# halismai/bpvo

Hardware: AMD Instinct MI355X
Metric: GN iterations/s (1241x376 bit-planes 8ch, 4 levels, Tukey; linearise + solve + update = 1, the reference's _num_fun_evals) (higher is better)
Workload: dtype f32 (+f64 projection/interpolation); 1 GPU; batch of 1024 independent 1241x376 stereo pairs (1024 per GPU), bitplanes descriptor, 4 pyramid levels, tukey loss, converge with AlgorithmParameters() tolerances; pairs_per_gpu=1024

## Files before the change

### __graft_entry__.py

```python
from __future__ import annotations

import os
import subprocess
import sys

ROOT = os.path.dirname(os.path.abspath(__file__))
CSRC = os.path.join(ROOT, "bpvo_amd", "csrc")
HIP_LIB = os.path.join(CSRC, "libbpvo_hip.so")
ORACLE_DIR = os.path.join(ROOT, "oracle")
ORACLE_LIB = os.path.join(ORACLE_DIR, "_build", "libbpvo_oracle.so")

MGPU_LIB = os.path.join(CSRC, "libbpvo_hip_mgpu.so")

HIP_SOURCES = ["context.hip", "frames.hip", "estimate.hip", "batch.hip", "vo.hip", "measure.hip", "kernels_frame.hip", "kernels_intensity_norm.hip", "kernels_planes.hip", "kernels_gn.hip", "kernels_gn_ref.hip", "kernels_gn_team.hip", "kernels_gn_rig.hip", "kernels_gn_cov.hip", "pose_cov.hip", "kernels_score.hip", "score.hip", "kernels_stereo.hip", "kernels_sgm.hip", "kernels_sgbm.hip", "kernels_rectify.hip", "rectify.hip", "stereo.hip", "kernels_disparity_fusion.hip", "disparity_fusion.hip", "kernels_disparity_variance.hip", "disparity_variance.hip", "kernels_motion_stereo.hip", "motion_stereo.hip"]
HIP_HEADERS = ["host_ctx.h", "device_owned.h", "vo_state.h", "gn_rounds.h", "frame_plan.h", "kernels.h", "types.h", "device_math.h", "gn_common.h", "gn_warp.h", "warp_rule.h", "gn_median.h", "gn_tscale.h", "tscale_math.h", "gn_irls.h", "gn_step.h", "rig_math.h", "pose_cov_math.h", "pose_score_math.h", "rectify_math.h", "intensity_norm_math.h", "disparity_fusion_math.h", "disparity_variance_math.h", "motion_stereo_math.h", "gn_cov.h", "frame_common.h", "latch_table.h", "sg_scanline.h",
               os.path.join("..", "..", "include", "bpvo_hip", "c_api.h")]
HIPCC_FLAGS = ["--offload-arch=gfx950", "-O3", "-std=c++17", "-ffp-contract=off", "-fPIC", "-Wall", "-Wno-unused-function"]
OBJ_DIR = os.path.join(CSRC, "obj")


def _newer(target, sources):
    if not os.path.exists(target):
        return True
    t = os.path.getmtime(target)
    return any(os.path.getmtime(s) > t for s in sources if os.path.exists(s))


def _hipcc():
    for cand in ("hipcc", "/opt/rocm/bin/hipcc"):
        try:
            subprocess.run([cand, "--version"], check=True, capture_output=True)
            return cand
        except Exception:
            continue
    raise RuntimeError("hipcc not found")


def build_hip(force: bool = False, extra_flags=(), out: str | None = None) -> str:
    from concurrent.futures import ThreadPoolExecutor
    out = out or HIP_LIB
    headers = [os.path.join(CSRC, h) for h in HIP_HEADERS]
    if not force and not _newer(out, [os.path.join(CSRC, s) for s in HIP_SOURCES] + headers):
        return out
    obj_dir = OBJ_DIR if out == HIP_LIB else OBJ_DIR + "_" + os.path.splitext(os.path.basename(out))[0]
    os.makedirs(obj_dir, exist_ok=True)
    hipcc = _hipcc()
    jobs = []
    for s in HIP_SOURCES:
        src = os.path.join(CSRC, s)
        obj = os.path.join(obj_dir, os.path.splitext(s)[0] + ".o")
        if force or _newer(obj, [src] + headers):
            jobs.append([hipcc, *HIPCC_FLAGS, *extra_flags, "-c", src, "-o", obj])

    def run(cmd):
        return subprocess.run(cmd, cwd=CSRC, capture_output=True, text=True)
    with ThreadPoolExecutor(max_workers=min(8, os.cpu_count() or 1)) as ex:
        for cmd, r in zip(jobs, ex.map(run, jobs)):
            if r.returncode != 0:
                raise RuntimeError("hipcc failed (%s):\n%s%s" % (cmd[-3], r.stdout, r.stderr))
    objs = [os.path.join(obj_dir, os.path.splitext(s)[0] + ".o") for s in HIP_SOURCES]
    if force or jobs or _newer(out, objs):
        r = subprocess.run([hipcc, "--offload-arch=gfx950", "-shared", "-fPIC", "-o", out, *objs], cwd=CSRC, capture_output=True, text=True)
        if r.returncode != 0:
            raise RuntimeError("hipcc link failed:\n" + r.stdout + r.stderr)
    return out


def build_mgpu(force: bool = False) -> str:
    src = os.path.join(CSRC, "multi_gpu.hip")
    deps = [src, HIP_LIB, os.path.join(ROOT, "include", "bpvo_hip", "multi_gpu.h"), os.path.join(ROOT, "include", "bpvo_hip", "c_api.h")]
    if force or _newer(MGPU_LIB, deps):
        rocm_lib = os.path.join(os.environ.get("ROCM_PATH", "/opt/rocm"), "lib")
        cmd = [_hipcc(), "--offload-arch=gfx950", "-O2", "-std=c++17", "-fPIC", "-shared", "-Wall", "-o", MGPU_LIB, src,
               "-L", CSRC, "-lbpvo_hip", "-L", rocm_lib, "-lrccl", "-lpthread", "-Wl,-rpath,$ORIGIN", f"-Wl,-rpath,{rocm_lib}"]
        r = subprocess.run(cmd, cwd=CSRC, capture_output=True, text=True)
        if r.returncode != 0:
            raise RuntimeError("hipcc (multi_gpu) failed:\n" + r.stdout + r.stderr)
    return MGPU_LIB


def build_oracle(force: bool = False) -> str:
    if force:
        subprocess.run(["make", "-C", ORACLE_DIR, "clean"], check=True, capture_output=True)
    r = subprocess.run(["make", "-C", ORACLE_DIR], capture_output=True, text=True)
    if r.returncode != 0:
        raise RuntimeError("oracle build failed:\n" + r.stdout + r.stderr)
    return ORACLE_LIB


def build_reference_pins() -> str | None:
    if not os.path.isdir("/root/reference/bpvo"):
        return None
    r = subprocess.run(["make", "-C", ORACLE_DIR, "ref"], capture_output=True, text=True)
    if r.returncode != 0:
        raise RuntimeError("oracle/_ref build failed:\n" + r.stdout + r.stderr)
    return os.path.join(ORACLE_DIR, "_ref", "libbpvo_ref.so")


# ... 65 lines not shown
```

### bpvo_amd/csrc/batch.hip

```cpp
#include "host_ctx.h"

using namespace bpvo_hip;
using namespace bpvo_hip_host;

namespace {

constexpr int kUploadChunkPairs = 16;
constexpr int kUploadGroup = 4;
struct UploadRun {
  bpvo_hip_ctx* c = nullptr;
  int n_pairs = 0;
  std::vector<std::pair<int, int>> chunks;
  std::vector<int> recorded;
  std::mutex mu;
  std::condition_variable cv;
  std::vector<std::thread> workers;
  std::string err;
  ~UploadRun() { for(auto& t : workers) if(t.joinable()) t.join(); }
};

int upload_prepare(bpvo_hip_ctx* c, int n_pairs)
{
  const size_t npix = c->geom[0].npix;
  c->up_slot_bytes = (size_t) kUploadChunkPairs * npix * (2 + 4);
// ... 107 lines not shown
      }
      FR_CK(c, fr_lane, hipStreamWaitEvent(fr_lane.stream, c->up_chunk_done[k], 0));
    }
    const int p0 = u.chunks[mine[i]].first;
    int np = 0;
    for(size_t q = i; q < i + take; ++q) np += u.chunks[mine[q]].second;
    FrameRun fr = fr_lane;
    fr.tab = 2 * p0;
    fr.selected_ev = nullptr; fr.on_selected = nullptr;
    int rc = frames_set_data_slots(c, strided_slots(2 * p0, 1, 2 * np).data(), 2 * np, c->up_d_img + (size_t) 2 * p0 * npix, c->up_d_disp + (size_t) p0 * npix, true, fr, 2);
    if(rc) return rc;
    i += take;
  }
  return BPVO_OK;
}

int batch_run_staggered(bpvo_hip_ctx* c, int n_pairs, int nl, const uint8_t* images, const float* disparities, bool on_device, float* poses,
                        bpvo_hip_stats* stats, UploadRun* pipe, const std::vector<std::pair<int, int>>* host_group_list)
{
  HIP_CK(c, hipStreamSynchronize(c->stream));
  c->frac_valid = false;
  const size_t npix = c->geom[0].npix;
  std::vector<int> rcs(nl, BPVO_OK);
  std::mutex mu;
  std::condition_variable cv;
  std::vector<int> selected(nl, 0);
  std::vector<std::pair<int, int>> groups;
  if(host_group_list) groups = *host_group_list;
  else host_groups(n_pairs, nl, 1, groups);
  const int nsub = (int) groups.size() / nl;
  auto run = [&](int k) {
    Lane* ln = &c->lanes[k];
    (void) hipSetDevice(c->device);
    auto release_next = [&mu, &cv, &selected, k] { { std::lock_guard<std::mutex> lk(mu); selected[k] = 1; } cv.notify_all(); };
    struct Release { std::function<void()> f; ~Release() { f(); } } always{release_next};
    if(k > 0 && !pipe) {
      { std::unique_lock<std::mutex> lk(mu); cv.wait(lk, [&] { return selected[k - 1] != 0; }); }
      if(hipStreamWaitEvent(ln->stream, c->lanes[k - 1].selected_ev, 0) != hipSuccess) { ln->err = "hipStreamWaitEvent"; rcs[k] = BPVO_ERR_DEVICE; return; }
    }
    for(int sub = 0; sub < nsub; ++sub) {
      const int lo = groups[(size_t) sub * nl + k].first, hi = groups[(size_t) sub * nl + k].second, n = hi - lo;
      if(n <= 0) continue;
      FrameRun fr{ln->stream, ln, 2 * lo, true, nullptr, nullptr};
      int rc = pipe ? upload_consume(c, *pipe, lo, hi, fr)
                    : frames_set_data_slots(c, strided_slots(2 * lo, 1, 2 * n).data(), 2 * n, images + (size_t) 2 * lo * npix, disparities + (size_t) 2 * lo * npix, on_device, fr,
                                            c->keep_current_disparity ? 0 : 1);
      if(rc) { rcs[k] = rc; return; }
      if(sub == 0) {
        fr.selected_ev = ln->selected_ev;
        fr.on_selected = release_next;
      }
      rc = frames_set_template_slots(c, strided_slots(2 * lo, 2, n).data(), n, fr);
      if(rc) { rcs[k] = rc; return; }
      std::vector<int> wss(n), refs(n), curs(n);
      for(int i = 0; i < n; ++i) { wss[i] = lo + i; refs[i] = 2 * (lo + i); curs[i] = 2 * (lo + i) + 1; }
      rc = estimate_group(c, ln, n, wss.data(), refs.data(), curs.data(), nullptr, poses ? poses + 16 * (size_t) lo : nullptr,
                          stats ? stats + (size_t) lo * c->L : nullptr, c->d_records + (size_t) kRecordFloats * lo, false);
      if(rc) { rcs[k] = rc; return; }
    }
  };
  {
    std::vector<std::thread> th;
    for(int k = 1; k < nl; ++k) th.emplace_back(run, k);
    run(0);
    for(auto& t : th) t.join();
  }
  for(int k = 0; k < nl; ++k)
    if(rcs[k]) { c->err = c->lanes[k].err; return rcs[k]; }
  resolve_events(c);
  for(int i = 0; i < n_pairs; ++i) {
    Workspace& w = c->ws[i];
    w.last_ref = 2 * i;
    w.last_cur = 2 * i + 1;
    w.last_level = c->params.maxTestLevel;
    w.has_estimate = true;
  }
  return BPVO_OK;
}

}

extern "C" {

int bpvo_hip_batch_run(bpvo_hip_ctx* c, int n_pairs, const uint8_t* images, const float* disparities, int on_device,
                       float* poses, bpvo_hip_stats* stats)
{
  CHECK_CTX(c);
  if(n_pairs < 0 || 2 * n_pairs > c->n_frames || n_pairs > c->n_pairs) return fail(c, BPVO_ERR_INVALID_ARG, "batch exceeds ctx capacity");
  for(int i = 0; i < 2 * n_pairs; ++i)
    if(c->frames[i].own_geom) return fail(c, BPVO_ERR_UNSUPPORTED, "pair batches run the context's camera: its slots carry per-sequence cameras (bpvo_hip_seq_set_camera)");
  (void) hipSetDevice(c->device);
  if(n_pairs > 0 && (!images || !disparities)) return fail(c, BPVO_ERR_INVALID_ARG, "nullptr image/disparity");
  const bool use_pipe = !on_device && c->up_workers > 0 && !c->keep_current_disparity && n_pairs >= 2 * kUploadChunkPairs;
  int nl = lanes_for(c, n_pairs, use_pipe ? 2 : 8);
  if(nl < 0) return nl;
  if(team_serves(c, n_pairs)) nl = 1;
  if(c->stagger && n_pairs >= c->stagger_min_pairs && nl > 1 && !c->profile_all) {
    if(!use_pipe) return batch_run_staggered(c, n_pairs, nl, images, disparities, on_device != 0, poses, stats, nullptr, nullptr);
    std::vector<std::pair<int, int>> groups;
    const int nsub = 1;
    const bool plan = nl == 2 && nsub == 1 && c->up_plan[0] > 0.0 && n_pairs >= 32 * kUploadChunkPairs;
    if(plan) host_groups_plan(c, n_pairs, groups);
    else host_groups(n_pairs, nl, nsub, groups);
    UploadRun pipe;
    int rcp = upload_start(c, pipe, n_pairs, groups, images, disparities);
    if(rcp) return rcp;
    c->ctl_by_kernel = true;
    rcp = batch_run_staggered(c, n_pairs, nl, images, disparities, false, poses, stats, &pipe, &groups);
    c->ctl_by_kernel = false;
    return rcp;
  }
  int rc;
  if(use_pipe) {
    UploadRun pipe;
    std::vector<std::pair<int, int>> groups;
    host_groups(n_pairs, 1, 1, groups);
    rc = upload_start(c, pipe, n_pairs, groups, images, disparities);
    if(rc) return rc;
    rc = upload_consume(c, pipe, 0, n_pairs, ctx_run(c));
  } else {
    rc = frames_set_data(c, 0, 1, 2 * n_pairs, images, disparities, on_device != 0, c->keep_current_disparity ? 0 : 1);
  }
  if(rc) return rc;
  FrameRun fr = ctx_run(c);
  fr.no_final_sync = !c->profiling;
  fr.defer_finest_nrm = !team_serves(c, n_pairs) || n_pairs <= c->team_split_max_pairs || templates_may_be_dense(c);
  rc = frames_set_template_slots(c, strided_slots(0, 2, n_pairs).data(), n_pairs, fr);
  if(rc == BPVO_OK) rc = bpvo_hip_batch_estimate(c, n_pairs, nullptr, poses, stats);
  if(c->nrm_pending) { (void) hipEventSynchronize(c->nrm_pending); c->nrm_pending = nullptr; }
  if(c->nrm_pending_finest) { (void) hipEventSynchronize(c->nrm_pending_finest); c->nrm_pending_finest = nullptr; }
  return rc;
}
int bpvo_hip_batch_result_records_device(bpvo_hip_ctx* c, const float** d_records, int* floats_per_pair)
{
  CHECK_CTX(c);
  *d_records = c->d_records;
  *floats_per_pair = kRecordFloats;
  return BPVO_OK;
}

int bpvo_hip_batch_copy_records_device(bpvo_hip_ctx* c, float* d_dst, int n_pairs)
{
  CHECK_CTX(c);
  if(!d_dst || n_pairs < 0 || n_pairs > c->n_pairs) return fail(c, BPVO_ERR_INVALID_ARG, "bad record copy");
  (void) hipSetDevice(c->device);
  HIP_CK(c, hipMemcpyAsync(d_dst, c->d_records, sizeof(float) * kRecordFloats * (size_t) n_pairs, hipMemcpyDeviceToDevice, c->stream));
  HIP_CK(c, hipStreamSynchronize(c->stream));
  return BPVO_OK;
}

}
```

### bpvo_amd/csrc/context.hip

```cpp
#include "host_ctx.h"

using namespace bpvo_hip;
using namespace bpvo_hip_host;

namespace bpvo_hip_host {

std::atomic<int> g_live_ctx[64];
thread_local std::string g_create_error;

int fail(bpvo_hip_ctx* c, int code, const char* msg)
{
  c->err = msg;
  return code;
}


void gaussian_kernel5(double sigma, float k[3])
{
  float kk[5];
  const double sigmaX = sigma > 0 ? sigma : ((5 - 1) * 0.5 - 1) * 0.3 + 0.8;
  const double scale2X = -0.5 / (sigmaX * sigmaX);
  double sum = 0;
  for(int i = 0; i < 5; ++i) {
    const double x = i - 2.0;
// ... 42 lines not shown
{
  Carver cv{base};
  for(int l = 0; l < c->L; ++l) {
    const LevelGeom& g = c->geom[l];
    f.sal[l] = cv.take<float>(g.npix);
    const size_t nwords = (size_t) g.rows * ((g.cols + 63) / 64);
    f.flag[l] = (uint8_t*) cv.take<unsigned long long>((std::max(g.npix, nwords * 8) + 7) / 8);
    f.blk_count[l] = cv.take<int>(std::max((size_t) g.nblk, nwords));
    f.pts[l] = cv.take<float4>(g.cap);
    f.ptc[l] = cv.take<float2>(g.cap);
    f.inds[l] = cv.take<int>(g.cap);
    f.pix[l] = cv.take<float>((size_t) g.cap * c->C);
    f.grad[l] = cv.take<float>((size_t) g.cap * c->C * 2);
  }
  f.nrm = cv.take<float>(4 * kMaxLevels);
  f.n_dev = cv.take<int>(kMaxLevels);
  f.sel_info = cv.take<int>(4 * kMaxLevels);
  if(total) *total = cv.off;
}

hipError_t ensure_template_storage(bpvo_hip_ctx* c, FrameSlot& f, hipStream_t stream)
{
  if(f.tmpl_slab) return hipSuccess;
  size_t total = 0;
  FrameSlot tmp;
  carve_frame_tmpl(c, tmp, nullptr, &total);
  if(hipError_t e = f.tmpl_slab.alloc(total)) return e;
  if(hipError_t e = hipMemsetAsync(f.tmpl_slab, 0, total, stream)) return e;
  carve_frame_tmpl(c, f, f.tmpl_slab, nullptr);
  return hipSuccess;
}

FrameJob make_frame_job(bpvo_hip_ctx* c, FrameSlot& f, int l)
{
  const LevelGeom& g = slot_geom(c, f, l);
  FrameJob j;
  std::memset(&j, 0, sizeof(j));
  j.img = f.img[l];
  j.cen = f.cen[l];
  j.ch0 = (f.ch0_valid && f.lazy[l] != 2) ? f.ch0[l] : nullptr;
  j.scratch = f.scratch;
  j.inorm = c->d_inorm ? c->d_inorm + ((size_t) (&f - c->frames.data()) * c->L + l) : nullptr;
  j.desc = f.desc[l];
  j.sal = f.sal_state[l] == FrameSlot::SAL_STORED ? f.sal[l] : nullptr;
  j.flag = f.flag[l];
  j.words = reinterpret_cast<unsigned long long*>(f.flag[l]);
  j.blk_count = f.blk_count[l];
  j.n_out = f.n_dev ? f.n_dev + l : nullptr;
  j.disp = f.disp;
  j.pts = f.pts[l];
  j.ptc = f.ptc[l];
  j.inds = f.inds[l];
  j.pix = f.pix[l];
  j.grad = f.grad[l];
  j.nrm = f.nrm ? f.nrm + 4 * l : nullptr;
  j.rows = g.rows; j.cols = g.cols; j.level = l; j.disp_cols = slot_geom(c, f, 0).cols;
  j.cap = g.cap;
  j.nms_radius = g.nms_radius;
  std::memcpy(j.K, g.K, sizeof(j.K));
  j.b = g.b;
  j.dspace = c->dspace;
  j.lazy = f.lazy[l];
  const bpvo_hip_params& sp = f.seq_params ? *f.seq_params : c->params;
  j.min_saliency = sp.minSaliency; j.min_disp = sp.minValidDisparity; j.max_disp = sp.maxValidDisparity;
  j.max_points = slot_budget(c, f, l);
  j.sel_info = f.sel_info ? f.sel_info + 4 * l : nullptr;
  return j;
}

PairJob make_pair_job(bpvo_hip_ctx* c, int ws, int ref, int cur, int l)
{
  FrameSlot& fr = c->frames[ref];
  FrameSlot& fc = c->frames[cur];
  const LevelGeom& g = slot_geom(c, fr, l);
  PairJob j;
  std::memset(&j, 0, sizeof(j));
  j.pts = fr.pts[l];
  j.ptc = fr.ptc[l];
  j.pix = fr.pix[l];
  j.grad = fr.grad[l];
  j.nrm = fr.nrm + 4 * l;
  j.n = fr.n_host[l];
  j.desc = fc.desc[l];
  j.rows = g.rows; j.cols = g.cols;
  std::memcpy(j.K, g.K, sizeof(j.K));
  j.b = g.b;
  j.f_inv[0] = 1.0f / g.K[0]; j.f_inv[1] = 1.0f / g.K[4];
  j.dspace = c->dspace;
  j.r = c->ws[ws].r;
  j.valid = c->ws[ws].valid;
  j.cand = c->ws[ws].cand;
  j.tapkey = c->ws[ws].tapkey;
  j.tapcache_on = c->ws[ws].tapkey != nullptr;
  j.tapcache = c->ws[ws].tapcache;
  j.med_blk = c->ws[ws].med_blk;
  j.partials = c->ws[ws].partials;
  j.st = c->d_states + ws;
  j.cnt = c->d_counters + kWsCounters * (size_t) ws;
  j.ticket = c->d_tickets + ws;
  if(ws == c->trace_ws) { j.trace = c->d_trace; j.trace_cap = (int) (c->d_trace.size() / kTraceFloats); }
  j.pitch = c->C;
  j.n_groups = c->G;
  j.med_tot = (int) med_totals_at(c);
  pair_job_set_params(j, c->params);
  return j;
}
void pair_job_set_params(PairJob& j, const bpvo_hip_params& p)
{
  j.prm = GNParams{p.maxIterations, kMaxFunEvals, p.parameterTolerance, p.functionTolerance, p.gradientTolerance};
  j.loss = p.lossFunction;
  j.good_thr = p.goodPointThreshold;
}

PairJob group_pair_job(const bpvo_hip_ctx* c, const PairJob& whole, int k)
{
  PairJob j = whole;
  const size_t off = (size_t) k * c->Cg;
  const size_t nblk = (size_t) ((whole.n + kChunkPoints - 1) / kChunkPoints);
  const size_t ntiles = (size_t) std::max(1, (whole.n + gn_pts_per_block(c->Cg) - 1) / gn_pts_per_block(c->Cg));
  j.desc = whole.desc.get() + off;
  j.pix = whole.pix.get() + off;
  j.grad = whole.grad.get() + off;
  j.r = whole.r.get() + off;
  j.cand = whole.cand.get() + (size_t) k * nblk * kChunkPoints * c->Cg;
  j.med_blk = whole.med_blk.get() + (size_t) k * nblk * 4;
  j.partials = whole.partials.get() + (size_t) k * ntiles * kPartialStride;
  j.n_groups = 1;
  return j;
}

Event take_event(Lane* ln)
{
  Event e;
  if(!ln->ev_pool.empty()) {
    e = std::move(ln->ev_pool.back());
    ln->ev_pool.pop_back();
  }
  else (void) e.create(0);
  return e;
}
void resolve_events(bpvo_hip_ctx* c)
{
  for(auto& ln : c->lanes) {
    for(auto& ep : ln.ev_pending) {
      float ms = 0.0f;
      if(hipEventElapsedTime(&ms, ep.a, ep.b) == hipSuccess) {
        c->kc_ms[ep.kc] += ms;
        c->kc_units[ep.kc] += ep.units;
        c->kc_launches[ep.kc] += 1;
      }
      ln.ev_pool.push_back(std::move(ep.a));
      ln.ev_pool.push_back(std::move(ep.b));
    }
    ln.ev_pending.clear();
  }
}

int lanes_for(bpvo_hip_ctx* c, int n, int cap)
{
  if(g_live_ctx[c->device & 63].load() > 1) return 1;
  const int want = std::max(1, std::min(std::min(c->max_lanes_now, cap), n / kMinPairsPerLane));
  if(want > (int) c->lanes.size()) {
    const int rc = ensure_lanes(c, want);
    if(rc) return rc;
  }
  return want;
// ... 21 lines not shown
    HIP_CK(c, ln.h_pk_ctl.alloc(kPkCtlWords * kMaxLevels));
    if(first) {
      HIP_CK(c, ln.d_team_ctl.alloc((size_t) gn_team_ctl_words(kMaxTeams)));
      HIP_CK(c, ln.h_team_ctl.alloc(64));
      std::memset(ln.h_team_ctl, 0, sizeof(unsigned) * 64);
    }
    HIP_CK(c, ln.h_states.alloc((size_t) n_pairs + n_pairs));
  }
  return BPVO_OK;
}

const std::vector<OptionDef>& option_table()
{
#define OPT_INT(key_, field_, lo_, hi_) OptionDef{key_, lo_, hi_, [](bpvo_hip_ctx* c) { return (double) c->field_; }, \
                                                  [](bpvo_hip_ctx* c, double v) { c->field_ = (decltype(c->field_)) v; return BPVO_OK; }}
  static const std::vector<OptionDef> t = {
    OptionDef{"lanes", 1, 8, [](bpvo_hip_ctx* c) { return (double) std::max(1, std::min(c->max_lanes_now, std::max(1, c->n_pairs / kMinPairsPerLane))); },
              [](bpvo_hip_ctx* c, double v) {
                const int n = std::max(1, std::min((int) v, std::max(1, c->n_pairs / kMinPairsPerLane)));
                const int rc = ensure_lanes(c, n);
                if(rc == BPVO_OK) c->max_lanes_now = (int) v;
                return rc;
              }},
    OptionDef{"persistent", 0, 1, [](bpvo_hip_ctx* c) { return (double) c->persistent; },
              [](bpvo_hip_ctx* c, double v) { c->persistent = (int) v; if(c->persistent) c->persistent_failed.store(false); return BPVO_OK; }},
    OPT_INT("persist_max_ws", persist_max_ws, 1, kPersistMaxWs),
    OPT_INT("persist_grid", persist_grid, 1, 128),
    OPT_INT("persist_max_points", persist_max_points, 0, 1 << 30),
    OPT_INT("dense_candidates_from", dense_candidates_from, 0, 1 << 30),
    OPT_INT("persist_timeout_ticks", persist_timeout, 1, 1e15),
    OPT_INT("team", team_mode, 0, 1),
    OPT_INT("team_max_pairs", team_max_pairs, 0, 1 << 20),
    OPT_INT("team_full_pairs", team_full_pairs, 0, 1 << 20),
    OPT_INT("team_size", team_size_env, 0, 256),
    OptionDef{"team_cus", 1, 1 << 16, [](bpvo_hip_ctx* c) { return (double) c->num_cus; },
              [](bpvo_hip_ctx* c, double v) {
                if(c->device_cus > 0 && (int) v > c->device_cus) { c->err = "option team_cus: more CUs than the device has"; return BPVO_ERR_INVALID_ARG; }
                c->num_cus = (int) v;
                return BPVO_OK;
              }},
    OPT_INT("team_local_barriers", team_local_barriers, 0, 1),
    OPT_INT("team_join", team_join, 0, 2),
    OptionDef{"team_joins_seen", 0, 0, [](bpvo_hip_ctx* c) { return (double) c->team_joins.load(); },
              [](bpvo_hip_ctx* c, double) { c->team_joins.store(0); return BPVO_OK; }},
    OPT_INT("team_join_from_pairs", team_join_from_pairs, 0, 1 << 20),
    OPT_INT("team_spares", team_spares, 0, 1),
    OPT_INT("vo_disparity_late", vo_disparity_late, 0, 1),
    OPT_INT("stereo_frames_per_launch", stereo_frames_per_launch, 0, 65535),
    OptionDef{"stereo_frames_per_launch_seen", 0, 0, [](bpvo_hip_ctx* c) { return (double) c->st_frames_per_launch_seen; }, [](bpvo_hip_ctx*, double) { return BPVO_OK; }},
    OptionDef{"stereo_free_mib_seen", 0, 0, [](bpvo_hip_ctx* c) { return (double) (c->st_free_seen >> 20); }, [](bpvo_hip_ctx*, double) { return BPVO_OK; }},
    OptionDef{"rectify_last_kernel_ms", 0, 0, [](bpvo_hip_ctx* c) {
                float ms = -1.0f;
                if(!c->rect.timed || hipEventSynchronize(c->rect.t1) != hipSuccess || hipEventElapsedTime(&ms, c->rect.t0, c->rect.t1) != hipSuccess) return -1.0;
                return (double) ms;
              }, [](bpvo_hip_ctx*, double) { return BPVO_OK; }},
    OptionDef{"fusion_last_splat_ms", 0, 0, [](bpvo_hip_ctx* c) { return fusion_last_ms(c, 0); }, [](bpvo_hip_ctx*, double) { return BPVO_OK; }},
    OptionDef{"fusion_last_update_ms", 0, 0, [](bpvo_hip_ctx* c) { return fusion_last_ms(c, 1); }, [](bpvo_hip_ctx*, double) { return BPVO_OK; }},
    OptionDef{"variance_last_kernel_ms", 0, 0, [](bpvo_hip_ctx* c) { return variance_last_ms(c); }, [](bpvo_hip_ctx*, double) { return BPVO_OK; }},
    OptionDef{"motion_stereo_last_kernel_ms", 0, 0, [](bpvo_hip_ctx* c) { return motion_stereo_last_ms(c); }, [](bpvo_hip_ctx*, double) { return BPVO_OK; }},
    OPT_INT("normalization_side_stream", nrm_side_stream, 0, 1),
    OPT_INT("normalization_form", nrm_dpp_asm, 0, 4),
    OPT_INT("small_batch_fused", small_batch_fused, 0, 1),
    OPT_INT("levels_in_one_launch_max_frames", merge_levels_max_frames, 0, 1 << 20),
    OPT_INT("normalization_deferred", nrm_defer, 0, 1),
    OPT_INT("team_split_max_pairs", team_split_max_pairs, 0, 1 << 20),
    OPT_INT("fuse_frozen", fuse_frozen, 0, 1),
    OPT_INT("reference_reduction", reference_reduction, 0, 1),
    OPT_INT("step_in_reduce_max_pairs", step_in_reduce_max, 0, 1 << 20),
    OPT_INT("stagger", stagger, 0, 1),
    OPT_INT("stagger_min_pairs", stagger_min_pairs, 0, 1 << 20),
    OPT_INT("upload_workers", up_workers, 0, 32),
    OPT_INT("keep_current_disparity", keep_current_disparity, 0, 1),
    OptionDef{"pose_covariance", 0, 1, [](bpvo_hip_ctx* c) { return (double) c->pose_covariance; },
              [](bpvo_hip_ctx* c, double v) -> int {
                if((int) v) {
                  const int rc = pose_cov_ensure_scratch(c);
                  if(rc) return rc;
                }
                c->pose_covariance = (int) v;
                return BPVO_OK;
              }},
    OPT_INT("lazy_template_descriptor", lazy_template, 0, 1),
    OPT_INT("lazy_template_saliency", lazy_saliency, 0, 1),
    OPT_INT("points_from_compact_stream", points_from_compact, 0, 1),
    OptionDef{"tapcache_max_density", 0.0, 1e9, [](bpvo_hip_ctx* c) { return c->tapcache_max_density; },
              [](bpvo_hip_ctx* c, double v) { c->tapcache_max_density = v; return BPVO_OK; }},
    OptionDef{"upload_plan_first", 0.0, 0.9, [](bpvo_hip_ctx* c) { return c->up_plan[0]; },
              [](bpvo_hip_ctx* c, double v) { if(v + c->up_plan[1] >= 1.0) return BPVO_ERR_INVALID_ARG; c->up_plan[0] = v; return BPVO_OK; }},
    OptionDef{"upload_plan_second", 0.01, 0.99, [](bpvo_hip_ctx* c) { return c->up_plan[1]; },
              [](bpvo_hip_ctx* c, double v) { if(v + c->up_plan[0] >= 1.0) return BPVO_ERR_INVALID_ARG; c->up_plan[1] = v; return BPVO_OK; }},
  };
#undef OPT_INT
  return t;
}
int set_option(bpvo_hip_ctx* c, const std::string& key, double v)
{
  for(const OptionDef& o : option_table())
    if(key == o.key) {
      if(!(v >= o.lo && v <= o.hi)) { c->err = "option " + key + ": value out of range"; return BPVO_ERR_INVALID_ARG; }
      const int rc = o.set(c, v);
      if(rc == BPVO_ERR_INVALID_ARG) c->err = "option " + key + ": invalid value";
      return rc;
    }
  c->err = "unknown option: " + key;
  return BPVO_ERR_INVALID_ARG;
}
int apply_options_string(bpvo_hip_ctx* c, const char* str)
{
  std::string s(str);
  size_t i = 0;
  while(i < s.size()) {
    size_t j = s.find(',', i);
    if(j == std::string::npos) j = s.size();
    const std::string kv = s.substr(i, j - i);
    i = j + 1;
    if(kv.empty()) continue;
    const size_t eq = kv.find('=');
    if(eq == std::string::npos) { c->err = "expected key=value: " + kv; return BPVO_ERR_INVALID_ARG; }
    char* end = nullptr;
    const double v = std::strtod(kv.c_str() + eq + 1, &end);
    if(end == kv.c_str() + eq + 1) { c->err = "not a number: " + kv; return BPVO_ERR_INVALID_ARG; }
    const int rc = set_option(c, kv.substr(0, eq), v);
    if(rc) return rc;
  }
  return BPVO_OK;
}

}

extern "C" {

void bpvo_hip_default_params(bpvo_hip_params* p)
{
  p->numPyramidLevels = -1;
  p->minImageDimensionForPyramid = 40;
  p->sigmaPriorToCensusTransform = -1.0f;
  p->sigmaBitPlanes = 0.5f;
  p->dfSigma1 = 0.75f;
  p->dfSigma2 = 1.75f;
  p->latchNumBytes = 1;
  p->latchRotationInvariance = 0;
  p->latchHalfSsdSize = 1;
  p->centralDifferenceRadius = 3;
  p->centralDifferenceSigmaBefore = 0.75f;
  p->centralDifferenceSigmaAfter = 1.75f;
  p->laplacianKernelSize = 1;
  p->maxIterations = 50;
  p->parameterTolerance = 1e-7f;
  p->functionTolerance = 1e-6f;
  p->gradientTolerance = 1e-8f;
  p->relaxTolerancesForCoarseLevels = 1;
  p->gradientEstimation = BPVO_GRAD_CD3;
  p->interp = BPVO_INTERP_LINEAR;
  p->lossFunction = BPVO_LOSS_TUKEY;
  p->descriptor = BPVO_DESC_INTENSITY;
  p->verbosity = BPVO_VERB_ITERATION;
  p->minTranslationMagToKeyFrame = 0.15f;
  p->minRotationMagToKeyFrame = 5.0f;
  p->maxFractionOfGoodPointsToKeyFrame = 0.6f;
  p->goodPointThreshold = 0.85f;
  p->minNumPixelsForNonMaximaSuppression = 320 * 240;
  p->nonMaxSuppRadius = 1;
  p->minNumPixelsToWork = 256;
  p->minSaliency = 0.1f;
  p->minValidDisparity = 0.001f;
  p->maxValidDisparity = 512.0f;
// ... 314 lines not shown
```

### bpvo_amd/csrc/estimate.hip

```cpp
#include "host_ctx.h"

using namespace bpvo_hip;
using namespace bpvo_hip_host;

namespace bpvo_hip_host {


struct TeamPlan { int team_size, n_teams, join_mode, spare_workgroups; };
static TeamPlan team_plan(const bpvo_hip_ctx* c, int n)
{
  TeamPlan t;
  const int slots = std::max(1, c->num_cus);
  int ts = c->team_size_env > 0 ? c->team_size_env : std::max(1, std::min(std::max(1, c->device_cus > 0 ? c->device_cus / 8 : 32), slots / std::max(1, n)));
  ts = std::max(1, std::min(ts, slots));
  t.team_size = ts;
  t.n_teams = std::max(1, std::min(std::min(n, slots / ts), kMaxTeams));
  t.join_mode = (t.team_size < gn_team_max_size() && t.n_teams > 1 && n >= c->team_join_from_pairs) ? c->team_join : 0;
  t.spare_workgroups = (t.join_mode && c->team_spares) ? std::max(0, slots - t.team_size * t.n_teams) : 0;
  return t;
}

bool team_serves(const bpvo_hip_ctx* c, int n)
{
  bool size_ok = n >= 2 && n > c->persist_max_ws && n <= c->team_max_pairs;
// ... 10 lines not shown
static bool templates_suit_teams(const bpvo_hip_ctx* c, int n, const int* refs)
{
  for(int i = 0; i < n; ++i)
    for(int l = c->params.maxTestLevel; l < c->L; ++l)
      if(c->frames[refs[i]].n_host[l] > c->persist_max_points) return false;
  return true;
}

template <class PrmOf>
static void fill_job_tables(bpvo_hip_ctx* c, Lane* ln, int first, int n, const int* wss, const int* refs, const int* curs, PrmOf&& prm_of, int* max_pts)
{
  const int NP = c->n_pairs;
  const size_t table = (size_t) c->L * NP;
  for(int l = 0; l < c->L; ++l)
    for(int i = 0; i < n; ++i) {
      PairJob& pj = ln->h_pjobs[(size_t) l * NP + first + i];
      pj = make_pair_job(c, wss[i], refs[i], curs[i], l);
      if(const bpvo_hip_params* prm = prm_of(i)) pair_job_set_params(pj, *prm);
      for(int k = 0; k < c->G && c->G > 1; ++k) ln->h_pjobs[(size_t) (1 + k) * table + (size_t) l * NP + first + i] = group_pair_job(c, pj, k);
      max_pts[l] = std::max(max_pts[l], pj.n);
    }
}
template <class LossOf, class Run>
static int for_each_loss(int n, LossOf&& loss_of, Run&& run)
{
  std::vector<char> done((size_t) n, 0);
  for(int i = 0; i < n; ++i) {
    if(done[i]) continue;
    std::vector<int> at;
    for(int k = i; k < n; ++k)
      if(!done[k] && loss_of(k) == loss_of(i)) { done[k] = 1; at.push_back(k); }
    if(int rc = run(at)) return rc;
  }
  return BPVO_OK;
}

void linearize_launches(bpvo_hip_ctx* c, Lane* ln, const GNLaunch& g, size_t stride, const LinearizeFlags& f)
{
  constexpr unsigned kProfileEvery = 5;
  const bool all = f.timers == TIMERS_ALWAYS || (f.timers != TIMERS_OFF && c->profile_all);
  if(f.warp) {
    const bool sampled = all || (f.timers == TIMERS_ESTIMATE && (c->profile_k6_all || (ln->k6_seq++ % kProfileEvery) == 0));
    ScopedTimer t(c, KC_WARP_RESIDUAL, 0.0, ln, sampled);
    for_each_group(c, g, stride, [&](const GNLaunch& gg) { launch_warp_residual(ln->stream, gg); });
  }
  { ScopedTimer t(c, KC_MEDIAN, 0.0, ln, all && f.median); if(f.median) launch_median(ln->stream, median_launch(c, g)); }
  if(f.reduce) {
    ScopedTimer t(c, KC_IRLS_REDUCE, 0.0, ln, all || (f.timers == TIMERS_ESTIMATE && c->profile_k6_all));
    if(g.reference_reduction) launch_irls_reduce(ln->stream, g);
    else for_each_group(c, g, stride, [&](const GNLaunch& gg) { launch_irls_reduce(ln->stream, gg); });
  }
  if(f.step && !g.step_in_reduce) {
    ScopedTimer t(c, KC_GN_STEP, 0.0, ln, all);
    launch_gn_step(ln->stream, g, f.step_mode);
  }
}

template <class QueueIterations, class QueueFlags, class Read>
static int lane_rounds(Lane* ln, int max_iterations, QueueIterations&& queue_iterations, QueueFlags&& queue_flags, Read&& read)
{
  return run_rounds(max_iterations, queue_iterations,
                    [&](int slot) -> int {
                      if(int rc = queue_flags(slot)) return rc;
                      LANE_CK(ln, hipEventRecord(ln->round_ev[slot], ln->stream));
                      return BPVO_OK;
                    },
                    [&](int slot) -> int {
                      LANE_CK(ln, hipEventSynchronize(ln->round_ev[slot]));
                      return BPVO_OK;
                    },
                    read);
}

struct GroupRun {
  bpvo_hip_ctx* c;
  Lane* ln;
  int n;
  const int* wss; const int* refs; const int* curs;
  const float* T_init;
  const bpvo_hip_params* const* prms;
  float* d_records_out;
  int loss, max_iterations;
  std::vector<int> max_pts;
  bool ref_mode;
  int fuse_frozen;
  bool allow_persistent;
  bool pk_group;
  bool small_ctx;
  bool l2_moot;
  bool team_ran, team_split, frac_queued;
};
static void group_modes(GroupRun& r, bool allow_persistent)
{
  const bpvo_hip_ctx* c = r.c;
  r.ref_mode = c->reference_reduction != 0;
  r.fuse_frozen = r.ref_mode ? 0 : c->fuse_frozen;
  r.allow_persistent = allow_persistent;
  r.pk_group = allow_persistent && c->persistent && !c->persistent_failed.load() && r.n <= c->persist_max_ws && !c->profile_all && !r.ref_mode &&
               !loss_is_chain_only(r.loss);
  r.small_ctx = (size_t) c->L * c->n_pairs <= 64 && r.n <= 8 && c->small_batch_fused && c->G == 1;
  r.l2_moot = r.loss == BPVO_LOSS_L2 && c->C == 8 && r.fuse_frozen && !c->fast_warp && c->params.interp == BPVO_INTERP_LINEAR;
  r.team_ran = r.team_split = r.frac_queued = false;
}

static int group_upload(GroupRun& r)
{
  bpvo_hip_ctx* c = r.c;
  Lane* ln = r.ln;
  const int n = r.n, NP = c->n_pairs;
  const int* refs = r.refs;
  const float* T_init = r.T_init;
  const bool persistent = r.pk_group;
  std::fill(r.max_pts.begin(), r.max_pts.end(), 0);
  const size_t table = (size_t) c->L * NP;
  fill_job_tables(c, ln, 0, n, r.wss, refs, r.curs, [&](int i) { return r.prms ? r.prms[i] : nullptr; }, r.max_pts.data());
  if((c->C == 8 || c->C == 1) && n > c->persist_max_ws)
    for(int l = 0; l < c->L; ++l)
      for(int i = 0; i < n; ++i) {
        PairJob& pj = ln->h_pjobs[(size_t) l * NP + i];
        if((double) pj.n > c->tapcache_max_density * (double) slot_geom(c, c->frames[refs[i]], l).npix) pj.tapcache_on = 0;
      }
  if(r.small_ctx) {
    if(T_init) std::memcpy(ln->h_T, T_init, sizeof(float) * 16 * n);
    launch_set_pose_upload(ln->stream, ln->d_pjobs, ln->h_pjobs, (size_t) c->L * NP, ln->h_pjobs + (size_t) (c->L - 1) * NP, T_init ? ln->h_T : nullptr, n,
                           persistent ? ln->d_pk_ctl : nullptr, persistent ? kPkCtlWords * kMaxLevels : 0);
  } else {
    const size_t table_bytes = sizeof(PairJob) * table * (size_t) job_tables(c);
    if(c->ctl_by_kernel.load()) launch_copy_rows(ln->stream, ln->d_pjobs, ln->h_pjobs, table_bytes, table_bytes, 1);
    else LANE_CK(ln, hipMemcpyAsync(ln->d_pjobs, ln->h_pjobs, table_bytes, hipMemcpyHostToDevice, ln->stream));
    const float* dT = nullptr;
    if(T_init) {
      std::memcpy(ln->h_T, T_init, sizeof(float) * 16 * n);
      if(c->ctl_by_kernel.load()) launch_copy_rows(ln->stream, ln->d_Tinit, ln->h_T, sizeof(float) * 16 * n, sizeof(float) * 16 * n, 1);
      else LANE_CK(ln, hipMemcpyAsync(ln->d_Tinit, ln->h_T, sizeof(float) * 16 * n, hipMemcpyHostToDevice, ln->stream));
      dT = ln->d_Tinit;
    }
    launch_set_pose(ln->stream, ln->d_pjobs + (size_t) (c->L - 1) * NP, dT, n, persistent ? ln->d_pk_ctl : nullptr, persistent ? kPkCtlWords * kMaxLevels : 0);
  }
  return BPVO_OK;
}

static int run_team(GroupRun& r)
{
  bpvo_hip_ctx* c = r.c;
  Lane* ln = r.ln;
  const bpvo_hip_params& p = c->params;
  const int n = r.n;
  r.team_split = (c->nrm_pending != nullptr || c->nrm_pending_finest != nullptr) && n <= c->team_split_max_pairs && c->L - 1 > p.maxTestLevel;
  if(!r.team_split) LANE_CK(ln, join_pending_normalization(c, ln->stream));
  GNTeamLaunch t;
  t.jobs_all = ln->d_pjobs; t.job_pitch = c->n_pairs; t.n_pairs = n; t.level_hi = c->L - 1; t.level_lo = p.maxTestLevel;
  t.C = c->C; t.loss = r.loss; t.fuse_frozen = c->fuse_frozen;
  t.scale_is_moot = (r.loss == BPVO_LOSS_L2 && c->C == 8 && c->fuse_frozen) ? 1 : 0;
  const TeamPlan plan = team_plan(c, n);
  t.team_size = plan.team_size;
  t.n_teams = plan.n_teams;
  t.ctl = ln->d_team_ctl;
  t.timeout_ticks = c->persist_timeout;
  t.local_barriers = c->team_local_barriers;
  t.join_mode = plan.join_mode;
  t.spare_workgroups = plan.spare_workgroups;
  LANE_CK(ln, hipMemsetAsync(ln->d_team_ctl, 0, sizeof(unsigned) * (size_t) gn_team_ctl_words(t.n_teams), ln->stream));
  hipError_t te;
  if(r.team_split) {
    t.level_lo = c->L - 1;
    te = launch_gn_team(ln->stream, t);
    if(te == hipSuccess) {
      LANE_CK(ln, hipMemcpyAsync(ln->h_team_ctl + 32, ln->d_team_ctl, sizeof(unsigned) * 32, hipMemcpyDeviceToHost, ln->stream));
      launch_team_ctl_reset_keep_abort(ln->stream, ln->d_team_ctl, t.n_teams);
    }
    LANE_CK(ln, join_pending_normalization(c, ln->stream));
    t.level_hi = c->L - 2; t.level_lo = p.maxTestLevel;
    if(te == hipSuccess) te = launch_gn_team(ln->stream, t);
  } else {
    te = launch_gn_team(ln->stream, t);
  }
  if(te == hipSuccess) {
    r.team_ran = true;
    c->team_launches.fetch_add(1);
    LANE_CK(ln, hipMemcpyAsync(ln->h_team_ctl, ln->d_team_ctl, sizeof(unsigned) * 32, hipMemcpyDeviceToHost, ln->stream));
  } else {
    (void) hipGetLastError();
    c->persistent_failed.store(true);
  }
  return BPVO_OK;
}

static GNLaunch group_level_launch(const GroupRun& r, int l)
{
  const bpvo_hip_ctx* c = r.c;
  GNLaunch g = level_launch(c, r.ln->d_pjobs + (size_t) l * c->n_pairs, r.n, r.max_pts[l], r.loss);
  g.fuse_frozen = r.fuse_frozen;
  g.step_in_reduce = (r.n <= c->step_in_reduce_max && !r.ref_mode && c->G == 1) ? 1 : 0;
  return g;
}
static bool persistent_serves_level(const GroupRun& r, int l)
{
  return r.max_pts[l] > 0 && gn_persistent_serves(group_level_launch(r, l)) && r.max_pts[l] <= r.c->persist_max_points;
}

struct PersistentLevel { bool served, began_next; };
static PersistentLevel run_level_persistent(GroupRun& r, GNLaunch g, int l, bool was_begun)
{
  bpvo_hip_ctx* c = r.c;
  Lane* ln = r.ln;
  const bool next_too = l - 1 >= c->params.maxTestLevel && persistent_serves_level(r, l - 1);
  g.begin_level = was_begun ? l : -1;
  g.begin_moot = r.l2_moot ? 1 : 0;
  g.next_jobs = next_too ? ln->d_pjobs + (size_t) (l - 1) * c->n_pairs : nullptr;
  const hipError_t pe = launch_gn_persistent(ln->stream, g, ln->d_pk_ctl + (size_t) l * kPkCtlWords, gn_persistent_grid(g, c->persist_grid), c->persist_timeout);
  if(pe == hipSuccess) {
    c->persistent_levels.fetch_add(1);
    return {true, next_too};
  }
  (void) hipGetLastError();
  c->persistent_failed.store(true);
  if(was_begun) launch_level_begin(ln->stream, g.jobs, r.n, g.max_points, l, r.l2_moot ? 1 : 0);
  return {false, false};
}

static int run_level_chain(GroupRun& r, GNLaunch g)
{
  bpvo_hip_ctx* c = r.c;
  Lane* ln = r.ln;
  const int NP = c->n_pairs;
  const size_t table = (size_t) c->L * NP;
  int* const lists[3] = {ln->d_list, ln->d_list + NP, ln->d_list + 2 * (size_t) NP};
  int n_cur = r.n;
  g.active.list = nullptr;
  const bool fused_path = c->C == 8 && r.fuse_frozen && !c->fast_warp && c->params.interp == BPVO_INTERP_LINEAR;
  bool none_moving = r.l2_moot;
  LinearizeFlags f;
  f.timers = TIMERS_ESTIMATE;
  return lane_rounds(ln, r.max_iterations,
                     [&](int) -> int {
                       g.npairs = n_cur;
                       f.median = !none_moving;
                       f.warp = !(none_moving && fused_path);
                       for(int k = 0; k < kItersPerSync; ++k) linearize_launches(c, ln, g, table, f);
                       return BPVO_OK;
                     },
                     [&](int slot) -> int {
                       launch_compact_active(ln->stream, g.jobs, g.active, n_cur, lists[slot], ln->d_active + 2 * slot);
                       LANE_CK(ln, hipMemcpyAsync(ln->h_active + 2 * slot, ln->d_active + 2 * slot, 2 * sizeof(int), hipMemcpyDeviceToHost, ln->stream));
                       return BPVO_OK;
                     },
                     [&](int slot) {
                       const int n_left = ln->h_active[2 * slot];
                       if(n_left <= 0) return false;
                       n_cur = n_left;
                       none_moving = none_moving || ln->h_active[2 * slot + 1] == 0;
                       g.active.list = lists[slot];
                       return true;
                     });
}

static int run_levels(GroupRun& r)
{
  bpvo_hip_ctx* c = r.c;
  Lane* ln = r.ln;
  bool persistent = r.pk_group;
  bool begun = false;
  for(int l = c->L - 1; l >= c->params.maxTestLevel; --l) {
    const GNLaunch g = group_level_launch(r, l);
    if(l < c->L - 1) LANE_CK(ln, join_pending_normalization(c, ln->stream, l));
    const bool was_begun = begun;
    begun = false;
    if(!was_begun) launch_level_begin(ln->stream, g.jobs, r.n, g.max_points, l, r.l2_moot ? 1 : 0);
    if(g.max_points <= 0) continue;
    if(persistent && persistent_serves_level(r, l)) {
      const PersistentLevel pk = run_level_persistent(r, g, l, was_begun);
      begun = pk.began_next;
      if(pk.served) continue;
    }
    persistent = false;
    if(int rc = run_level_chain(r, g)) return rc;
  }
  return BPVO_OK;
}

static int queue_fraction_good(GroupRun& r)
{
  bpvo_hip_ctx* c = r.c;
  Lane* ln = r.ln;
  const bpvo_hip_params& p = c->params;
  const int NP = c->n_pairs;
  const PairJob* coarsest = ln->d_pjobs + (size_t) (c->L - 1) * NP;
  const bool want_frac = r.n == 1 && c->prefetch_frac_thr >= 0.0f && ln == &c->lanes[0];
  if(r.small_ctx) launch_pack_records(ln->stream, coarsest, r.n, c->L, r.d_records_out, c->d_states, ln->h_states, r.pk_group ? ln->d_pk_ctl : nullptr,
                                      r.pk_group ? ln->h_pk_ctl : nullptr, kPkCtlWords * kMaxLevels, want_frac ? c->d_count : nullptr);
  else launch_pack_records(ln->stream, coarsest, r.n, c->L, r.d_records_out);
  const int npts = ln->h_pjobs[(size_t) p.maxTestLevel * NP].n;
  if(!want_frac || npts <= 0) return BPVO_OK;
  const PairJob* job = ln->d_pjobs + (size_t) p.maxTestLevel * NP;
  launch_refresh_residuals(ln->stream, level_launch(c, job, 1, npts, p.lossFunction));
  if(!r.small_ctx) LANE_CK(ln, hipMemsetAsync(c->d_count, 0, sizeof(unsigned int), ln->stream));
  launch_count_good(ln->stream, job, npts, c->C, p.lossFunction, c->prefetch_frac_thr, c->d_count);
  LANE_CK(ln, hipMemcpyAsync(c->h_ints, c->d_count, sizeof(unsigned int), hipMemcpyDeviceToHost, ln->stream));
  r.frac_queued = true;
  c->frac_n = npts;
  return BPVO_OK;
}

#ifdef BPVO_PK_TIMING
static void print_pk_timing(const GroupRun& r)
{
  const bpvo_hip_ctx* c = r.c;
  const Lane* ln = r.ln;
  static const char* names[6] = {"warp", "barrier1", "median", "irls", "barrier2", "step"};
  if(r.pk_group) {
    for(int l = c->L - 1; l >= 0; --l) {
      const unsigned* t = ln->h_pk_ctl + (size_t) l * kPkCtlWords;
      if(!t[15]) continue;
      std::fprintf(stderr, "pk level %d: %u iterations;", l, t[15]);
      for(int k = 0; k < 6; ++k) std::fprintf(stderr, " %s %.2f", names[k], 0.01 * t[8 + k] / t[15]);
      std::fprintf(stderr, " | step: sum_partials %.2f unpack %.2f solve %.2f pose %.2f tests %.2f", 0.01 * t[20] / t[15], 0.01 * t[16] / t[15], 0.01 * t[17] / t[15],
                   0.01 * t[18] / t[15], 0.01 * t[19] / t[15]);
      std::fprintf(stderr, " us per iteration\n");
    }
  }
  if(r.team_ran) {
    for(int l = c->L - 1; l >= 0 && l < 4; --l) {
      const unsigned* t = ln->h_team_ctl + 4 + 7 * l;
      if(!t[6]) continue;
      std::fprintf(stderr, "team level %d: %u iterations;", l, t[6]);
      for(int k = 0; k < 6; ++k) std::fprintf(stderr, " %s %.2f", names[k], 0.01 * t[k] / t[6]);
      std::fprintf(stderr, " us per iteration\n");
    }
  }
}
#endif

static int group_collect(GroupRun& r, bool* gave_up)
{
  bpvo_hip_ctx* c = r.c;
  Lane* ln = r.ln;
  int ws_lo = r.wss[0], ws_hi = r.wss[0];
  for(int i = 1; i < r.n; ++i) { ws_lo = std::min(ws_lo, r.wss[i]); ws_hi = std::max(ws_hi, r.wss[i]); }
  if(!r.small_ctx) {
    LANE_CK(ln, hipMemcpyAsync(ln->h_states + ws_lo, c->d_states + ws_lo, sizeof(GNState) * (size_t) (ws_hi - ws_lo + 1), hipMemcpyDeviceToHost, ln->stream));
    if(r.pk_group)
      LANE_CK(ln, hipMemcpyAsync(ln->h_pk_ctl, ln->d_pk_ctl, sizeof(unsigned) * kPkCtlWords * kMaxLevels, hipMemcpyDeviceToHost, ln->stream));
  }
  if(c->before_final_sync && ln == &c->lanes[0]) {
    const std::function<int()> f = std::move(c->before_final_sync);
    c->before_final_sync = nullptr;
    if(const int rcf = f()) return rcf;
  }
  LANE_CK(ln, hipStreamSynchronize(ln->stream));
  LANE_CK(ln, hipGetLastError());
  if(r.frac_queued) { c->frac_valid = true; c->frac_ws = r.wss[0]; c->frac_thr = c->prefetch_frac_thr; c->frac_cnt = (unsigned) c->h_ints[0]; }
#ifdef BPVO_PK_TIMING
  print_pk_timing(r);
#endif
  if(r.team_ran) {
    c->team_joins.fetch_add(ln->h_team_ctl[3] + (r.team_split ? ln->h_team_ctl[32 + 3] : 0u));
    *gave_up = ln->h_team_ctl[1] != 0 || (r.team_split && ln->h_team_ctl[32 + 1] != 0);
  }
  if(r.pk_group)
    for(int l = 0; l < c->L; ++l) *gave_up = *gave_up || ln->h_pk_ctl[(size_t) l * kPkCtlWords + 1] != 0;
  return BPVO_OK;
}

static void group_outputs(const GroupRun& r, float* poses, bpvo_hip_stats* stats)
{
  const int L = r.c->L;
  for(int i = 0; i < r.n; ++i) {
    const GNState& st = r.ln->h_states[r.wss[i]];
    if(poses) std::memcpy(poses + 16 * (size_t) i, st.T_out, 16 * sizeof(float));
    if(stats)
      for(int l = 0; l < L; ++l) stats[(size_t) i * L + l] = st.stats[l];
  }
}

int estimate_group(bpvo_hip_ctx* c, Lane* ln, int n, const int* wss, const int* refs, const int* curs, const float* T_init,
                   float* poses, bpvo_hip_stats* stats, float* d_records_out, bool allow_persistent, const bpvo_hip_params* const* prms)
{
  if(n <= 0) return BPVO_OK;
  (void) hipSetDevice(c->device);
  GroupRun r{c, ln, n, wss, refs, curs, T_init, prms, d_records_out};
  r.loss = prms ? prms[0]->lossFunction : c->params.lossFunction;
  r.max_iterations = c->params.maxIterations;
  if(prms) {
    r.max_iterations = prms[0]->maxIterations;
    for(int i = 1; i < n; ++i) r.max_iterations = std::max(r.max_iterations, prms[i]->maxIterations);
  }
  r.max_pts.assign((size_t) c->L, 0);
  for(const bool persistent_forms : {allow_persistent, false}) {
    group_modes(r, persistent_forms);
    if(int rc = group_upload(r)) return rc;
    if(persistent_forms && ln == &c->lanes[0] && !loss_is_chain_only(r.loss) && team_serves(c, n) && templates_suit_teams(c, n, refs))
      if(int rc = run_team(r)) return rc;
    if(!r.team_ran)
      if(int rc = run_levels(r)) return rc;
    if(int rc = queue_fraction_good(r)) return rc;
    bool gave_up = false;
    if(int rc = group_collect(r, &gave_up)) return rc;
    if(!gave_up) break;
    c->persistent_failed.store(true);
  }
  group_outputs(r, poses, stats);
  return BPVO_OK;
}

int check_pairs(bpvo_hip_ctx* c, int n, const int* wss, const int* refs, const int* curs, int level_lo, int level_hi)
{
  for(int i = 0; i < n; ++i) {
    CHECK_WS(c, wss[i]); CHECK_SLOT(c, refs[i]); CHECK_SLOT(c, curs[i]);
  }
  for(int i = 0; i < n; ++i) {
    if(!c->frames[refs[i]].has_template) return fail(c, BPVO_ERR_NO_TEMPLATE, "reference frame has no template");
    if(!c->frames[curs[i]].has_data) return fail(c, BPVO_ERR_NO_DATA, "no data in frame");
    for(int l = level_lo; l <= level_hi; ++l)
      if(c->frames[refs[i]].n_host[l] <= 0) return fail(c, BPVO_ERR_NO_TEMPLATE, "you should call setData before calling computeResiduals");
  }
  for(int i = 0; i < n; ++i)
    if(int rc = ensure_dense_descriptor(c, curs[i])) return rc;
  return BPVO_OK;
}

static int estimate_one_loss(bpvo_hip_ctx* c, int n, const int* wss, const int* refs, const int* curs, const float* T_init, float* poses, bpvo_hip_stats* stats,
                             const bpvo_hip_params* const* prms);
int estimate_batch(bpvo_hip_ctx* c, int n, const int* wss, const int* refs, const int* curs, const float* T_init, float* poses, bpvo_hip_stats* stats,
                   const bpvo_hip_params* const* prms)
{
  if(!prms) return estimate_one_loss(c, n, wss, refs, curs, T_init, poses, stats, prms);
  return for_each_loss(n, [&](int i) { return prms[i]->lossFunction; }, [&](const std::vector<int>& at) {
    const int m = (int) at.size();
    if(m == n) return estimate_one_loss(c, n, wss, refs, curs, T_init, poses, stats, prms);
    std::vector<int> w(m), r(m), cu(m);
    std::vector<const bpvo_hip_params*> pp(m);
    std::vector<float> Ti, To((size_t) m * 16);
    std::vector<bpvo_hip_stats> st((size_t) m * c->L);
    if(T_init) Ti.resize((size_t) m * 16);
    for(int k = 0; k < m; ++k) {
      w[k] = wss[at[k]]; r[k] = refs[at[k]]; cu[k] = curs[at[k]]; pp[k] = prms[at[k]];
      if(T_init) std::memcpy(&Ti[(size_t) k * 16], T_init + 16 * (size_t) at[k], 64);
    }
    const int rc = estimate_one_loss(c, m, w.data(), r.data(), cu.data(), T_init ? Ti.data() : nullptr, To.data(), st.data(), pp.data());
    if(rc) return rc;
    for(int k = 0; k < m; ++k) {
      if(poses) std::memcpy(poses + 16 * (size_t) at[k], &To[(size_t) k * 16], 64);
      if(stats) std::memcpy(stats + (size_t) at[k] * c->L, &st[(size_t) k * c->L], sizeof(bpvo_hip_stats) * (size_t) c->L);
    }
    return (int) BPVO_OK;
  });
}
static int estimate_one_loss(bpvo_hip_ctx* c, int n, const int* wss, const int* refs, const int* curs, const float* T_init, float* poses, bpvo_hip_stats* stats,
                             const bpvo_hip_params* const* prms)
{
  if(n <= 0) return BPVO_OK;
  if(n > c->n_pairs) return fail(c, BPVO_ERR_INVALID_ARG, "more pairs than workspaces");
  const bpvo_hip_params& p = c->params;
  if(int rc = check_pairs(c, n, wss, refs, curs, 0, -1)) return rc;
  int nl = lanes_for(c, n, 8);
  if(nl < 0) return nl;
  const int loss = prms ? prms[0]->lossFunction : p.lossFunction;
  if(!loss_is_chain_only(loss) && team_serves(c, n) && templates_suit_teams(c, n, refs)) nl = 1;
  if(nl > 1) {
    HIP_CK(c, join_pending_normalization(c, c->stream));
    HIP_CK(c, hipStreamSynchronize(c->stream));
  }
  std::vector<int> rcs(nl, BPVO_OK);
  c->frac_valid = false;
  auto run = [&](int k) {
    const int lo = (int) ((long long) n * k / nl), hi = (int) ((long long) n * (k + 1) / nl);
    rcs[k] = estimate_group(c, &c->lanes[k], hi - lo, wss + lo, refs + lo, curs + lo, T_init ? T_init + 16 * (size_t) lo : nullptr,
                            poses ? poses + 16 * (size_t) lo : nullptr, stats ? stats + (size_t) lo * c->L : nullptr,
                            c->d_records + (size_t) kRecordFloats * lo, nl == 1, prms ? prms + lo : nullptr);
  };
  if(nl == 1) {
    run(0);
  } else {
    std::vector<std::thread> th;
    for(int k = 1; k < nl; ++k) th.emplace_back(run, k);
    run(0);
    for(auto& t : th) t.join();
  }
  for(int k = 0; k < nl; ++k)
    if(rcs[k]) { c->err = c->lanes[k].err; return rcs[k]; }
  resolve_events(c);
  for(int i = 0; i < n; ++i) {
    Workspace& w = c->ws[wss[i]];
    w.last_ref = refs[i];
    w.last_cur = curs[i];
    w.last_level = p.maxTestLevel;
    w.has_estimate = true;
  }
  return BPVO_OK;
}

void detile_to_channel_major(const float* src, int n, int C, int E, int V, float* out)
{
  const int W = C * E, pieces = W / V;
  for(int i = 0; i < n; ++i)
    for(int w = 0; w < W; ++w) {
      const int piece = w / V, within = w - piece * V;
      const float v = src[(((size_t) (i / kTile) * pieces + piece) * kTile + (size_t) (i % kTile)) * V + within];
      const int ch = w / E, e = w - ch * E;
      out[((size_t) ch * n + i) * E + e] = v;
    }
}
size_t tiled_floats(int n, int floats_per_point) { return (size_t) ((n + kTile - 1) / kTile) * kTile * floats_per_point; }

int refresh_counters(bpvo_hip_ctx* c)
{
  std::vector<unsigned long long> all(kWsCounters * (size_t) c->n_pairs);
  HIP_CK(c, hipMemcpy(all.data(), c->d_counters, all.size() * sizeof(unsigned long long), hipMemcpyDeviceToHost));
  unsigned long long h[kWsCounters] = {};
  for(int w = 0; w < c->n_pairs; ++w)
    for(int k = 0; k < kWsCounters; ++k) h[k] += all[kWsCounters * (size_t) w + k];
  c->median_bracketed = h[2];
  c->median_full = h[3];
  c->tscale_passes = h[9]; c->tscale_stages = h[11];
  for(int k = 0; k < 4; ++k) c->tap_counts[k] = h[5 + k];
  c->total_lin = h[1];
  double all_k6 = 0;
  for(const auto& ln : c->lanes) all_k6 += ln.k6_seq;
  const bool sampled = c->profiling && !c->profile_all && !c->profile_k6_all && all_k6 > 0;
  c->kc_units[KC_WARP_RESIDUAL] = sampled ? (double) h[4] * (double) c->kc_launches[KC_WARP_RESIDUAL] / all_k6 : (double) h[4];
  c->points_fused = (double) h[10];
  c->kc_units[KC_IRLS_REDUCE] = (double) h[0];
  c->kc_units[KC_MEDIAN] = (double) h[0];
  c->kc_units[KC_GN_STEP] = (double) h[1];
  return BPVO_OK;
}

int upload_single_job(bpvo_hip_ctx* c, int ws, int ref, int cur, int level)
{
  PairJob* h = c->lanes[0].h_pjobs;
  h[0] = make_pair_job(c, ws, ref, cur, level);
  for(int k = 0; k < c->G && c->G > 1; ++k) h[1 + k] = group_pair_job(c, h[0], k);
  HIP_CK(c, hipMemcpyAsync(c->d_job1, h, sizeof(PairJob) * (size_t) job_tables(c), hipMemcpyHostToDevice, c->stream));
  HIP_CK(c, hipStreamSynchronize(c->stream));
  return BPVO_OK;
}

int ensure_residuals(bpvo_hip_ctx* c, int ws)
{
  Workspace& w = c->ws[ws];
  if(w.last_ref < 0 || c->C != 8) return BPVO_OK;
  int rc = upload_single_job(c, ws, w.last_ref, w.last_cur, w.last_level);
  if(rc) return rc;
  launch_refresh_residuals(c->stream, level_launch(c, c->d_job1, 1, c->frames[w.last_ref].n_host[w.last_level], c->params.lossFunction));
  return BPVO_OK;
}

int fraction_good(bpvo_hip_ctx* c, int ws, float thr, float* frac)
{
  Workspace& w = c->ws[ws];
  if(w.last_ref < 0) return fail(c, BPVO_ERR_NO_DATA, "no linearisation has run on this workspace");
  const int n = c->frames[w.last_ref].n_host[w.last_level];
  if(c->frac_valid && c->frac_ws == ws && c->frac_thr == thr && c->frac_n == n) {
    *frac = vo_fraction_good(c->frac_cnt, n, c->C);
    return BPVO_OK;
  }
  int rc = ensure_residuals(c, ws);
  if(rc) return rc;
  rc = upload_single_job(c, ws, w.last_ref, w.last_cur, w.last_level);
  if(rc) return rc;
  HIP_CK(c, hipMemsetAsync(c->d_count, 0, sizeof(unsigned int), c->stream));
  launch_count_good(c->stream, c->d_job1, n, c->C, c->params.lossFunction, thr, c->d_count);
  unsigned int cnt = 0;
  HIP_CK(c, hipMemcpyAsync(c->h_ints, c->d_count, sizeof(unsigned int), hipMemcpyDeviceToHost, c->stream));
  HIP_CK(c, hipStreamSynchronize(c->stream));
  cnt = (unsigned int) c->h_ints[0];
  *frac = vo_fraction_good(cnt, n, c->C);
  return BPVO_OK;
}

int get_weights_host(bpvo_hip_ctx* c, int ws, std::vector<float>& w_cm, int* n_out)
{
  Workspace& w = c->ws[ws];
  if(w.last_ref < 0) return fail(c, BPVO_ERR_NO_DATA, "no linearisation has run on this workspace");
  const int n = c->frames[w.last_ref].n_host[w.last_level];
  const int C = c->C;
  int rc = ensure_residuals(c, ws);
  if(rc) return rc;
  rc = upload_single_job(c, ws, w.last_ref, w.last_cur, w.last_level);
  if(rc) return rc;
  launch_weights(c->stream, c->d_job1, n, C, c->params.lossFunction, c->d_wtmp);
  std::vector<float> pm((size_t) n * C);
  HIP_CK(c, hipMemcpyAsync(pm.data(), c->d_wtmp, pm.size() * sizeof(float), hipMemcpyDeviceToHost, c->stream));
  HIP_CK(c, hipStreamSynchronize(c->stream));
  w_cm.resize(pm.size());
  for(int i = 0; i < n; ++i)
    for(int ch = 0; ch < C; ++ch) w_cm[(size_t) ch * n + i] = pm[(size_t) i * C + ch];
  *n_out = n;
  return BPVO_OK;
}

static int lane_error(bpvo_hip_ctx* c, const Lane* ln, int rc)
{
  if(rc) c->err = ln->err;
  return rc;
}
static int rig_check(bpvo_hip_ctx* c, int n, const int* wss, const int* refs, const int* curs, const float* X, int level_lo, int level_hi)
{
  if(n < 1 || n > c->n_pairs) return fail(c, BPVO_ERR_INVALID_ARG, "rig: n must be within 1 .. the context's workspaces");
  if(!wss || !refs || !curs || !X) return fail(c, BPVO_ERR_INVALID_ARG, "rig: nullptr members / extrinsics");
  if(c->dspace) return fail(c, BPVO_ERR_UNSUPPORTED, "rig mode does not serve BPVO_WARP_DISPARITY_SPACE_F32");
  for(int i = 0; i < n; ++i) {
    for(int k = 0; k < i; ++k)
      if(wss[k] == wss[i]) return fail(c, BPVO_ERR_INVALID_ARG, "rig: a workspace appears twice");
    if(!rig_extrinsic_ok(X + 16 * (size_t) i)) return fail(c, BPVO_ERR_INVALID_ARG, "rig: an extrinsic is not a rigid transform (finite, last row 0 0 0 1, R^T R = I within 1e-4)");
  }
  return check_pairs(c, n, wss, refs, curs, level_lo, level_hi);
}
static int rig_upload(bpvo_hip_ctx* c, Lane* ln, int n, const int* wss, const int* refs, const int* curs, const float* X, std::vector<int>& max_pts)
{
  const int NP = c->n_pairs;
  const size_t table = (size_t) c->L * NP;
// ... 392 lines not shown
```

### bpvo_amd/csrc/frame_common.h

```cpp
#pragma once
#include "kernels.h"

namespace bpvo_hip {

__device__ __forceinline__ int reflect101(int p, int len)
{
  if(p < 0) p = -p;
  if(p >= len) p = 2 * len - 2 - p;
  if(p < 0) p = 0;
  return p;
}

__device__ __forceinline__ int reflect101_wide(int p, int len)
{
  if(len == 1) return 0;
  while(p < 0 || p >= len) p = p < 0 ? -p : 2 * len - 2 - p;
  return p;
}

__device__ __forceinline__ uint2 spread_planes(unsigned c)
{
  unsigned lo = c & 0xFu, hi = (c >> 4) & 0xFu;
  lo = (lo | (lo << 14)) & 0x00030003u; lo = (lo | (lo << 7)) & 0x01010101u;
  hi = (hi | (hi << 14)) & 0x00030003u; hi = (hi | (hi << 7)) & 0x01010101u;
  return make_uint2(lo, hi);
}
__device__ __forceinline__ unsigned bp_row_index(unsigned cm2, unsigned cm1, unsigned c0, unsigned cp1, unsigned cp2)
{
  return (cm1 + cp1) + 3u * (cm2 + cp2) + 9u * c0;
}
__device__ __forceinline__ float bp_row_entry(int e, float k0, float k1, float k2)
{
  const float S0 = (float) (e / 9), A = (float) (e % 3), B = (float) ((e / 3) % 3);
  return S0 * k0 + A * k1 + B * k2;
}
__device__ __forceinline__ float bp_col(float Tm2, float Tm1, float T0, float Tp1, float Tp2, float k0, float k1, float k2)
{
  float o = k0 * T0;
  o += k1 * (Tp1 + Tm1);
  o += k2 * (Tp2 + Tm2);
  return o;
}
__device__ __forceinline__ int bp_census_coord(int p, int len) { return reflect101(min(p, len + 1), len); }

__host__ __device__ __forceinline__ bool bp_tile_column_is_lazy(int x0, int W)
{
  return x0 + 64 + 8 <= (W & ~3) && !(x0 == 0 && (W & 3) == 0);
}

static inline dim3 grid2d(int W, int R, int nz) { return dim3((W + 63) / 64, (R + 3) / 4, nz); }

}
```

### bpvo_amd/csrc/frames.hip

```cpp
#include "host_ctx.h"
#include "intensity_norm_math.h"

using namespace bpvo_hip;
using namespace bpvo_hip_host;

namespace bpvo_hip_host {

FrameRun ctx_run(bpvo_hip_ctx* c) { return FrameRun{c->stream, &c->lanes[0], 0, false, nullptr, nullptr}; }

int upload_frame_jobs(bpvo_hip_ctx* c, const int* slots, int count, const FrameRun& fr, int which, const FrameJob** tab)
{
  const size_t table = (size_t) which * c->L * c->n_frames;
  FR_CK(c, fr, hipEventSynchronize(fr.ln->staging_ev[which]));
  for(int l = 0; l < c->L; ++l) {
    FrameJob* row = c->h_fjobs + table + (size_t) l * c->n_frames + fr.tab;
    for(int i = 0; i < count; ++i) row[i] = make_frame_job(c, c->frames[slots[i]], l);
  }
  const size_t pitch = sizeof(FrameJob) * (size_t) c->n_frames;
  static_assert(sizeof(FrameJob) % 8 == 0 && sizeof(PairJob) % 8 == 0, "copy_rows_kernel moves 8-byte words");
  if(c->ctl_by_kernel.load() || count <= 512)
    launch_copy_rows(fr.stream, c->d_fjobs + table + fr.tab, c->h_fjobs + table + fr.tab, pitch, sizeof(FrameJob) * (size_t) count, c->L);
  else
    FR_CK(c, fr, hipMemcpy2DAsync(c->d_fjobs + table + fr.tab, pitch, c->h_fjobs + table + fr.tab, pitch, sizeof(FrameJob) * (size_t) count, (size_t) c->L,
                                  hipMemcpyHostToDevice, fr.stream));
  FR_CK(c, fr, hipEventRecord(fr.ln->staging_ev[which], fr.stream));
  *tab = c->d_fjobs + table + fr.tab;
  return BPVO_OK;
}
std::vector<int> strided_slots(int first, int stride, int count)
{
  std::vector<int> v((size_t) std::max(count, 0));
  for(int i = 0; i < count; ++i) v[i] = first + i * stride;
  return v;
}
static const LevelGeom* stage_geom(bpvo_hip_ctx* c, const int* slots, int count)
{
  const LevelGeom* geom = c->frames[slots[0]].own_geom ? c->frames[slots[0]].geom : c->geom;
  for(int i = 1; i < count; ++i)
    if(slot_geom(c, c->frames[slots[i]], 0).rows != geom[0].rows || slot_geom(c, c->frames[slots[i]], 0).cols != geom[0].cols) {
      fail(c, BPVO_ERR_INVALID_ARG, "frame stage over slots of different sizes");
      return nullptr;
    }
  return geom;
}

int frames_set_data_slots(bpvo_hip_ctx* c, const int* slots, int count, const uint8_t* images, const float* disps, bool on_device,
                          const FrameRun& fr, int skip_odd_disp, const size_t* offsets)
{
  if(count <= 0) return BPVO_OK;
  const LevelGeom* geom = stage_geom(c, slots, count);
  if(!geom) return BPVO_ERR_INVALID_ARG;
  const size_t npix = geom[0].npix;
  const bpvo_hip_params& p = c->params;
  const DescriptorForm form = descriptor_form(p, c->C, c->inorm_radius);
  hipStream_t s = fr.stream;
  if(!on_device) {
    for(int i = 0; i < count; ++i) {
      FrameSlot& f = c->frames[slots[i]];
      const size_t at = offsets ? offsets[i] : (size_t) i * npix;
      FR_CK(c, fr, hipMemcpyAsync(f.img[0], images + at, npix, hipMemcpyHostToDevice, s));
      if(!(skip_odd_disp && (i & 1)) && !fr.skip_disparity_upload)
        FR_CK(c, fr, hipMemcpyAsync(f.disp, disps + at, npix * sizeof(float), hipMemcpyHostToDevice, s));
    }
  }
  const bool lazy_ok = skip_odd_disp != 0 && c->lazy_template && form == DF_BITPLANES_FUSED && p.gradientEstimation == BPVO_GRAD_CD3;
  const bool census_only_ok = lazy_ok && c->lazy_saliency;
  bool census_only[kMaxLevels] = {};
  bool any_census_only = false;
  for(int l = p.maxTestLevel; l < c->L; ++l) any_census_only |= census_only[l] = census_only_ok && geom[l].nms_radius == 1;
  for(int i = 0; i < count; ++i) {
    FrameSlot& f = c->frames[slots[i]];
    f.ch0_valid = !(skip_odd_disp && (i & 1));
    for(int l = 0; l < c->L; ++l) {
      f.lazy[l] = (lazy_ok && !(i & 1) && geom[l].nms_radius > 0) ? (census_only[l] ? 2 : 1) : 0;
      if(f.sal_state[l] == FrameSlot::SAL_ON_DEMAND) f.sal_state[l] = FrameSlot::SAL_GONE;
    }
  }
  const FrameJob* tab = nullptr;
  int rc = upload_frame_jobs(c, slots, count, fr, 0, &tab);
  if(rc) return rc;
  const int NF = c->n_frames;
  if(on_device && offsets) {
    size_t* h_off = c->h_seq_off + fr.tab;
    for(int i = 0; i < count; ++i) h_off[i] = offsets[i];
    FR_CK(c, fr, hipMemcpyAsync(c->d_seq_off + fr.tab, h_off, sizeof(size_t) * (size_t) count, hipMemcpyHostToDevice, s));
    launch_ingest_at(s, tab, images, disps, c->d_seq_off + fr.tab, npix, count);
  } else if(on_device) {
    launch_ingest(s, tab, images, disps, npix, count, skip_odd_disp);
  }
  {
    double px = 0;
    for(int l = 1; l < c->L; ++l) px += (double) geom[l].npix * count;
    ScopedTimer t(c, KC_PYRAMID, px, fr.ln);
    bool grouped = count <= c->merge_levels_max_frames;
    for(int l = 0; l < c->L; ++l) grouped = grouped && geom[l].cols >= 8 && geom[l].rows >= 8;
    for(int l = 1; l < c->L;) {
      const int steps = grouped ? std::min(3, c->L - l) : 0;
      if(steps >= 2) {
        launch_pyramid_levels(s, tab + (size_t) (l - 1) * NF, NF, steps, geom[l + steps - 1].cols, geom[l + steps - 1].rows, count);
        l += steps;
      } else {
        launch_pyrdown(s, tab + (size_t) (l - 1) * NF, tab + (size_t) l * NF, geom[l].cols, geom[l].rows, count);
        l += 1;
      }
    }
  }
  {
    const int tested = c->L - p.maxTestLevel;
    double px = 0;
    for(int l = p.maxTestLevel; l < c->L; ++l) px += (double) geom[l].npix * count;
    ScopedTimer t(c, KC_DESCRIPTOR, px, fr.ln);
    for(const LevelSpan& sp : level_spans(c->L, p.maxTestLevel, merge_descriptor_levels(count, c->merge_levels_max_frames, tested, form))) {
      const FrameLaunch f = frame_launch(c, tab, geom, sp, count);
      switch(form) {
        case DF_BITPLANES_FUSED:
          if(sp.count > 1 ? any_census_only : census_only[sp.first]) launch_census_templates(s, f);
          if(sp.count == 1 && census_only[sp.first]) launch_bitplanes_pairs(s, f, c->gauss_k);
          else launch_bitplanes(s, f, p.sigmaBitPlanes, c->gauss_k, 1);
          break;
        case DF_BITPLANES_SMOOTHED_CENSUS:
        case DF_BITPLANES_UNSMOOTHED:
          launch_census(s, f, p.sigmaPriorToCensusTransform > 0.0f ? c->census_taps : nullptr);
          launch_bitplanes(s, f, p.sigmaBitPlanes, c->gauss_k, 0);
          break;
        case DF_INTENSITY: launch_intensity(s, f); break;
        case DF_INTENSITY_NORM: launch_intensity_norm(s, f, c->inorm_radius); break;
        case DF_LAPLACIAN: launch_laplacian(s, f.jobs, f.W, f.R, count, p.laplacianKernelSize); break;
        case DF_GRADIENT: launch_gradient_descriptor(s, f.jobs, f.W, f.R, count, c->grad_pre); break;
        case DF_FIELDS_1ST:
        case DF_FIELDS_2ND: launch_descriptor_fields(s, f.jobs, f.W, f.R, count, form == DF_FIELDS_2ND, c->df_g1, c->df_g2); break;
        case DF_CENTRAL_DIFFERENCE: launch_central_difference(s, f.jobs, f.W, f.R, count, p.centralDifferenceRadius, c->cd_before, c->cd_after); break;
        case DF_LATCH:
          launch_latch(s, f.jobs, f.W, f.R, count, p.latchNumBytes, p.latchHalfSsdSize, c->d_latch_off, c->latch_taps[0], c->latch_taps[1], c->latch_after);
          break;
      }
    }
  }
  FR_CK(c, fr, hipGetLastError());
  for(int i = 0; i < count; ++i) {
    FrameSlot& f = c->frames[slots[i]];
    f.has_data = true;
    f.has_disp = !(skip_odd_disp && (i & 1));
  }
  return BPVO_OK;
}
int upload_disparity(bpvo_hip_ctx* c, int slot, const float* disparity)
{
  if(!c->copy_stream) {
    HIP_CK(c, c->copy_stream.create());
    HIP_CK(c, c->copy_ev.create(hipEventDisableTiming));
  }
  HIP_CK(c, hipMemcpyAsync(c->frames[slot].disp, disparity, slot_geom(c, c->frames[slot], 0).npix * sizeof(float), hipMemcpyHostToDevice, c->copy_stream));
  HIP_CK(c, hipEventRecord(c->copy_ev, c->copy_stream));
  HIP_CK(c, hipStreamWaitEvent(c->stream, c->copy_ev, 0));
  return BPVO_OK;
}
int frames_set_data(bpvo_hip_ctx* c, int first, int stride, int count, const uint8_t* images, const float* disps, bool on_device, int skip_odd_disp)
{
  if(count <= 0) return BPVO_OK;
  if(first < 0 || stride < 1 || first + (count - 1) * stride >= c->n_frames) return fail(c, BPVO_ERR_INVALID_ARG, "bad frame slot range");
  if(!images || !disps) return fail(c, BPVO_ERR_INVALID_ARG, "nullptr image/disparity");
  return frames_set_data_slots(c, strided_slots(first, stride, count).data(), count, images, disps, on_device, ctx_run(c), skip_odd_disp);
}

int frames_set_template_slots(bpvo_hip_ctx* c, const int* slots, int count, const FrameRun& fr)
{
  if(count <= 0) return BPVO_OK;
  const LevelGeom* geom = stage_geom(c, slots, count);
  if(!geom) return BPVO_ERR_INVALID_ARG;
  hipStream_t s = fr.stream;
  for(int i = 0; i < count; ++i) FR_CK(c, fr, ensure_template_storage(c, c->frames[slots[i]], s));
  bool budget_at[kMaxLevels] = {};
  for(int i = 0; i < count; ++i) {
    FrameSlot& f = c->frames[slots[i]];
    f.min_saliency_used = (f.seq_params ? f.seq_params : &c->params)->minSaliency;
    for(int l = 0; l < c->L; ++l) {
      f.budget_used[l] = l >= c->params.maxTestLevel ? slot_budget(c, f, l) : 0;
      if(f.budget_used[l] > 0) budget_at[l] = true;
      f.sal_state[l] = (f.lazy[l] == 2 && slot_budget(c, f, l) <= 0) ? FrameSlot::SAL_ON_DEMAND : FrameSlot::SAL_STORED;
    }
  }
  const FrameJob* tab = nullptr;
  int rc = upload_frame_jobs(c, slots, count, fr, 1, &tab);
  if(rc) return rc;
  const int NF = c->n_frames;
  int* const h_ints = c->h_ints + (size_t) fr.tab * kMaxLevels;
  int* const d_ints = c->d_ints + (size_t) fr.tab * kMaxLevels;
  const bpvo_hip_params& p = c->params;
  const int border = std::max(p.nonMaxSuppRadius, 3);
  const int tested = c->L - p.maxTestLevel;
  bool tiled = true;
  for(int l = p.maxTestLevel; l < c->L; ++l) tiled = tiled && geom[l].nms_radius <= 1;
  hipEvent_t counts_ev = fr.ln ? fr.ln->round_ev[0] : nullptr;
  const bool side = c->nrm_side_stream && !fr.own_thread && fr.ln == &c->lanes[0] && counts_ev;
  if(side && !c->side_stream) {
    FR_CK(c, fr, c->side_stream.create());
    FR_CK(c, fr, c->side_stream2.create());
    for(auto& e : c->side_ev) FR_CK(c, fr, e.create(hipEventDisableTiming));
  }
  const int with_nrm = c->dspace ? 0 : p.withNormalization;
  const bool defer = fr.defer_finest_nrm && c->nrm_defer && !c->nrm_pending && !c->nrm_pending_finest;
// ... 3 lines not shown
    for(int k = 0; k < nrm.n; ++k) {
      const NrmPart& q = nrm.part[k];
      hipStream_t on = q.stream == NRM_INLINE ? s : (q.stream == NRM_SIDE ? c->side_stream : c->side_stream2);
      if(on != s && (k == 0 || q.stream != nrm.part[k - 1].stream)) FR_CK(c, fr, hipStreamWaitEvent(on, c->side_ev[0], 0));
      { ScopedTimer t(c, KC_NORMALIZATION, 0.0, fr.ln, true, on == s ? nullptr : on); launch_normalization(on, tab, NF, count, q.first_level, q.end_level, with_nrm, c->nrm_dpp_asm); }
      if(q.event >= 0) FR_CK(c, fr, hipEventRecord(c->side_ev[q.event], on));
    }
    if(nrm.pending_finest_event >= 0) c->nrm_pending_finest = c->side_ev[nrm.pending_finest_event];
    if(nrm.pending_event >= 0) c->nrm_pending = c->side_ev[nrm.pending_event];
    return BPVO_OK;
  };
  for(const LevelSpan& sp : level_spans(c->L, p.maxTestLevel, merge_selection_levels(count, c->merge_levels_max_frames, tested, tiled))) {
    const FrameLaunch f = frame_launch(c, tab, geom, sp, count);
    const int radius = geom[sp.first].nms_radius;
    double px = 0, budget_px = 0;
    for(int l = sp.first; l < sp.first + sp.count; ++l) {
      px += (double) geom[l].npix * count;
      if(budget_at[l]) budget_px += (double) geom[l].npix * count;
    }
    const bool budget = budget_px > 0;
    {
      ScopedTimer t(c, KC_SALIENCY_SELECT, px, fr.ln);
      launch_saliency_select(s, f, c->C, radius, border, c->gauss_k, budget ? SELECT_CANDIDATES : SELECT_ALL);
    }
    if(!budget) continue;
    {
      ScopedTimer t(c, KC_POINT_BUDGET, budget_px, fr.ln);
      launch_point_budget(s, f, radius);
    }
    ScopedTimer t(c, KC_SALIENCY_SELECT, 0.0, fr.ln);
    launch_saliency_select(s, f, c->C, radius, border, c->gauss_k, SELECT_COMPACT);
  }
  if(!nrm.behind_readback)
    if(int rcn = run_normalization()) return rcn;
  launch_gather_counts(s, tab, NF, count, p.maxTestLevel, c->L, d_ints);
  FR_CK(c, fr, hipMemcpyAsync(h_ints, d_ints, sizeof(int) * kMaxLevels * (size_t) count, hipMemcpyDeviceToHost, s));
  if(counts_ev) FR_CK(c, fr, hipEventRecord(counts_ev, s));
  if(fr.selected_ev) FR_CK(c, fr, hipEventRecord(fr.selected_ev, s));
  if(fr.on_selected) fr.on_selected();
  if(nrm.behind_readback)
    if(int rcn = run_normalization()) return rcn;
  if(counts_ev) FR_CK(c, fr, hipEventSynchronize(counts_ev));
  else FR_CK(c, fr, hipStreamSynchronize(s));
  int max_n[kMaxLevels] = {};
  double pts = 0;
  for(int i = 0; i < count; ++i) {
    FrameSlot& f = c->frames[slots[i]];
    for(int l = 0; l < c->L; ++l) {
      f.n_host[l] = (l >= p.maxTestLevel) ? h_ints[(size_t) i * kMaxLevels + l] : 0;
      max_n[l] = std::max(max_n[l], f.n_host[l]);
      pts += f.n_host[l];
    }
  }
  if(c->profiling) {
    std::lock_guard<std::mutex> lk(c->units_mu);
    c->kc_units[KC_TEMPLATE] += pts;
    c->kc_units[KC_NORMALIZATION] += pts;
  }
  for(const LevelSpan& sp : level_spans(c->L, p.maxTestLevel, merge_template_levels(count, c->merge_levels_max_frames, tested))) {
    ScopedTimer t(c, KC_TEMPLATE, 0.0, fr.ln);
    const int most = *std::max_element(max_n + sp.first, max_n + sp.first + sp.count);
    launch_template_build(s, frame_launch(c, tab, geom, sp, count), c->C, most, p.gradientEstimation == BPVO_GRAD_CD5, c->gauss_k);
  }
  if(nrm.join_event >= 0) FR_CK(c, fr, hipStreamWaitEvent(s, c->side_ev[nrm.join_event], 0));
  if(!fr.own_thread && !fr.no_final_sync) {
    FR_CK(c, fr, hipStreamSynchronize(s));
    FR_CK(c, fr, hipGetLastError());
    resolve_events(c);
  }
  for(int i = 0; i < count; ++i) c->frames[slots[i]].has_template = true;
  return BPVO_OK;
}
int frames_set_template(bpvo_hip_ctx* c, int first, int stride, int count)
{
  if(count <= 0) return BPVO_OK;
  if(first < 0 || stride < 1 || first + (count - 1) * stride >= c->n_frames) return fail(c, BPVO_ERR_INVALID_ARG, "bad frame slot range");
  for(int i = 0; i < count; ++i) {
    if(!c->frames[first + i * stride].has_data) return fail(c, BPVO_ERR_NO_DATA, "no data in frame");
    if(!c->frames[first + i * stride].has_disp) return fail(c, BPVO_ERR_NO_DATA, "no disparity in frame (the current frame of a pair batch)");
  }
  return frames_set_template_slots(c, strided_slots(first, stride, count).data(), count, ctx_run(c));
}

int ensure_dense_descriptor(bpvo_hip_ctx* c, int slot)
{
  FrameSlot& f = c->frames[slot];
  bool any = false;
  for(int l = 0; l < c->L; ++l) any = any || f.lazy[l];
  if(!any) return BPVO_OK;
  uint8_t was[kMaxLevels];
  for(int l = 0; l < c->L; ++l) { was[l] = f.lazy[l]; f.lazy[l] = 0; }
  auto restore = [&]() { for(int l = 0; l < c->L; ++l) f.lazy[l] = was[l]; };
  const FrameRun fr = ctx_run(c);
  const FrameJob* tab = nullptr;
  const int rc = upload_frame_jobs(c, &slot, 1, fr, 0, &tab);
  if(rc) { restore(); return rc; }
  for(const LevelSpan& sp : level_spans(c->L, c->params.maxTestLevel, false))
    launch_bitplanes(c->stream, frame_launch(c, tab, c->geom, sp, 1), c->params.sigmaBitPlanes, c->gauss_k, 1);
  if(hipGetLastError() != hipSuccess || hipStreamSynchronize(c->stream) != hipSuccess) {
    restore();
    return fail(c, BPVO_ERR_DEVICE, "ensure_dense_descriptor: descriptor kernels failed");
  }
  return BPVO_OK;
}


int ensure_saliency(bpvo_hip_ctx* c, int slot, int level)
{
  FrameSlot& f = c->frames[slot];
  if(f.sal_state[level] == FrameSlot::SAL_STORED) return BPVO_OK;
  if(f.sal_state[level] == FrameSlot::SAL_GONE)
    return fail(c, BPVO_ERR_NO_DATA, "the saliency map of a pair batch's template frame is formed on demand from the frame's data, which has been replaced");
  if(int rc = ensure_dense_descriptor(c, slot)) return rc;
  f.sal_state[level] = FrameSlot::SAL_STORED;
  const FrameRun fr = ctx_run(c);
  const FrameJob* tab = nullptr;
  int rc = upload_frame_jobs(c, &slot, 1, fr, 1, &tab);
  if(rc == BPVO_OK) {
    launch_saliency(c->stream, frame_launch(c, tab, &slot_geom(c, f, 0), LevelSpan{level, 1}, 1), c->C);
    if(hipGetLastError() != hipSuccess || hipStreamSynchronize(c->stream) != hipSuccess) rc = fail(c, BPVO_ERR_DEVICE, "ensure_saliency: saliency kernel failed");
  }
  if(rc) f.sal_state[level] = FrameSlot::SAL_ON_DEMAND;
  return rc;
}

int check_point_budget(bpvo_hip_ctx* c, const int* max_points, int n_levels)
{
  if(n_levels < 0 || n_levels > c->L) return fail(c, BPVO_ERR_INVALID_ARG, "point budget: more levels than the context has");
  if(n_levels > 0 && !max_points) return fail(c, BPVO_ERR_INVALID_ARG, "point budget: nullptr");
  for(int l = 0; l < n_levels; ++l) {
    if(max_points[l] < 0) return fail(c, BPVO_ERR_INVALID_ARG, "point budget: negative");
    if(max_points[l] > 0 && max_points[l] < 16) return fail(c, BPVO_ERR_INVALID_ARG, "point budget: 1 .. 15 points would always give an empty template (templates are cut to a multiple of 16)");
  }
  return BPVO_OK;
}

}

extern "C" {

int bpvo_hip_set_intensity_normalization(bpvo_hip_ctx* c, int radius)
{
  CHECK_CTX(c);
  if(descriptor_form(c->params, c->C) != DF_INTENSITY)
    return fail(c, BPVO_ERR_UNSUPPORTED, "intensity normalization: a mode of the Intensity descriptor, this context has another");
  if(radius < kInormOff || radius > kInormMaxRadius)
    return fail(c, BPVO_ERR_INVALID_ARG, "intensity normalization: radius -1 (off), 0 (whole image) or 1 .. 15 (local)");
  for(const FrameSlot& f : c->frames)
    if(f.has_data || f.has_template)
      return fail(c, BPVO_ERR_INVALID_ARG, "intensity normalization: a frame slot holds data; set it before the first frame or once every slot is cleared");
  (void) hipSetDevice(c->device);
  if(radius == 0 && !c->d_inorm) {
    const size_t n = (size_t) c->n_frames * c->L;
    HIP_CK(c, c->d_inorm.alloc(n));
    HIP_CK(c, hipMemsetAsync(c->d_inorm, 0, n * sizeof(InormScratch), c->stream));
    HIP_CK(c, hipStreamSynchronize(c->stream));
  } else if(radius != 0 && c->d_inorm) {
    HIP_CK(c, hipStreamSynchronize(c->stream));
    c->d_inorm.reset();
  }
  c->inorm_radius = radius;
  return BPVO_OK;
}
int bpvo_hip_get_intensity_normalization(const bpvo_hip_ctx* c, int* radius)
{
  if(!c || !radius) return BPVO_ERR_INVALID_ARG;
  *radius = c->inorm_radius;
  return BPVO_OK;
}

int bpvo_hip_set_point_budget(bpvo_hip_ctx* c, const int* max_points, int n_levels)
{
  CHECK_CTX(c);
  if(int rc = check_point_budget(c, max_points, n_levels)) return rc;
  for(int l = 0; l < kMaxLevels; ++l) c->point_budget[l] = l < n_levels ? max_points[l] : 0;
  return BPVO_OK;
}
int bpvo_hip_get_point_budget(const bpvo_hip_ctx* c, int* max_points)
{
  if(!c || !max_points) return BPVO_ERR_INVALID_ARG;
  for(int l = 0; l < kMaxLevels; ++l) max_points[l] = c->point_budget[l];
  return BPVO_OK;
}
int bpvo_hip_get_selection_info(bpvo_hip_ctx* c, int slot, int level, int* n_candidates, float* threshold, int* n_ties_kept)
{
// ... 190 lines not shown
```

### bpvo_amd/csrc/gn_warp.h

```cpp
#pragma once
#include "gn_common.h"
#include "warp_rule.h"

namespace bpvo_hip {

__device__ __forceinline__ void projection_matrix(const PairJob& j, const float* __restrict__ T, float (&P)[12])
{
#pragma unroll
  for(int r = 0; r < 3; ++r)
#pragma unroll
    for(int c = 0; c < 4; ++c) {
      float s = j.K[r * 3 + 0] * T[0 * 4 + c];
      s += j.K[r * 3 + 1] * T[1 * 4 + c];
      s += j.K[r * 3 + 2] * T[2 * 4 + c];
      P[r * 4 + c] = s;
    }
}

__device__ __forceinline__ void dspace_matrix(const PairJob& j, const float* __restrict__ T, float (&P)[12])
{
  const float fx = j.K[0], fy = j.K[4];
  M44 G, Gi, Tm;
  for(int i = 0; i < 16; ++i) { G.m[i] = 0.0f; Gi.m[i] = 0.0f; Tm.m[i] = T[i]; }
  G.m[0] = fx; G.m[5] = fy; G.m[11] = fx * j.b; G.m[14] = 1.0f;
  Gi.m[0] = (float) (1.0 / (double) fx); Gi.m[5] = (float) (1.0 / (double) fy); Gi.m[11] = 1.0f;
  Gi.m[14] = (float) (1.0 / (double) (fx * j.b));
  const M44 H = m44_mul(m44_mul(G, Tm), Gi);
#pragma unroll
  for(int c = 0; c < 4; ++c) { P[c] = H.m[c]; P[4 + c] = H.m[4 + c]; P[8 + c] = H.m[12 + c]; }
}

__device__ __forceinline__ float bilinear_res(float i00, float i01, float i10, float i11, float i0, double xf, double yf, double wx, double wy)
{
  const double Iw = wy * ((double) i00 * wx + (double) i01 * xf) + yf * ((double) i10 * wx + (double) i11 * xf);
  return (float) (Iw - (double) i0);
}
__device__ __forceinline__ float bilinear_res_f32(float i00, float i01, float i10, float i11, float i0, const float (&cf)[4])
{
  const float Iw = (cf[0] * i00 + cf[1] * i01) + (cf[2] * i10 + cf[3] * i11);
  return Iw - i0;
}

__device__ __forceinline__ unsigned tap_key(int xi, int yi) { return ((unsigned) yi << 16) | (unsigned) xi; }
__device__ __forceinline__ void taps8_gather(const PairJob& j, int xi, int yi, int W, float4 (&t)[8])
{
  const float4* q0 = reinterpret_cast<const float4*>(j.desc + ((size_t) yi * W + xi) * 8);
  const float4* q1 = q0 + (size_t) W * 2;
  t[0] = q0[0]; t[1] = q0[1]; t[2] = q0[2]; t[3] = q0[3];
  t[4] = q1[0]; t[5] = q1[1]; t[6] = q1[2]; t[7] = q1[3];
}
template <bool NT>
__device__ __forceinline__ void taps8_cache_store(const PairJob& j, int i, unsigned key, const float4 (&t)[8])
{
  float4* tc = reinterpret_cast<float4*>(j.tapcache.get());
#pragma unroll
  for(int k = 0; k < 8; ++k) store_v4<NT>(tc + tile_index<8>(i, k), t[k]);
  j.tapkey[i] = key;
}
__device__ __forceinline__ void taps8_unpack(const float4 (&t)[8], const float4 px0, const float4 px1, float (&i00)[8], float (&i01)[8],
                                             float (&i10)[8], float (&i11)[8], float (&i0)[8])
{
#pragma unroll
  for(int h = 0; h < 2; ++h) {
    i00[4 * h] = t[h].x; i00[4 * h + 1] = t[h].y; i00[4 * h + 2] = t[h].z; i00[4 * h + 3] = t[h].w;
    i01[4 * h] = t[2 + h].x; i01[4 * h + 1] = t[2 + h].y; i01[4 * h + 2] = t[2 + h].z; i01[4 * h + 3] = t[2 + h].w;
    i10[4 * h] = t[4 + h].x; i10[4 * h + 1] = t[4 + h].y; i10[4 * h + 2] = t[4 + h].z; i10[4 * h + 3] = t[4 + h].w;
    i11[4 * h] = t[6 + h].x; i11[4 * h + 1] = t[6 + h].y; i11[4 * h + 2] = t[6 + h].z; i11[4 * h + 3] = t[6 + h].w;
  }
  i0[0] = px0.x; i0[1] = px0.y; i0[2] = px0.z; i0[3] = px0.w; i0[4] = px1.x; i0[5] = px1.y; i0[6] = px1.z; i0[7] = px1.w;
}
__device__ __forceinline__ void taps8_residuals(const float4 (&t)[8], const float4 px0, const float4 px1, double xf, double yf, float (&res)[8])
{
  const double wx = 1.0 - xf, wy = 1.0 - yf;
  float i00[8], i01[8], i10[8], i11[8], i0[8];
  taps8_unpack(t, px0, px1, i00, i01, i10, i11, i0);
#pragma unroll
  for(int c = 0; c < 8; ++c) res[c] = bilinear_res(i00[c], i01[c], i10[c], i11[c], i0[c], xf, yf, wx, wy);
}

template <int C, bool FAST, bool HALF = false, bool NT = true>
__device__ __forceinline__ bool warp_point(const PairJob& j, const float (&P)[12], int i, bool in_block, float (&res)[C], bool& cache_hit,
                                           float4* X_out = nullptr)
{
  cache_hit = false;
  const int W = j.cols, R = j.rows;
  const float4 X = load_point<NT>(j, i);
  if(X_out) *X_out = X;
  unsigned spec_key = 0; float4 spec_taps = make_float4(0.0f, 0.0f, 0.0f, 0.0f); float spec_pix = 0.0f;
  if constexpr(C == 1) {
    if(j.tapcache_on) {
      spec_key = j.tapkey[i];
      spec_taps = load_v4<NT>(reinterpret_cast<const float4*>(j.tapcache.get()) + i);
    }
    spec_pix = j.pix[i];
  }
  int xi = 0, yi = 0;
  bool valid;
  double xf = 0.0, yf = 0.0;
  float cf[4] = {0, 0, 0, 0};
  if constexpr(!FAST) {
    const WarpFoot f = warp_foot(P, X.x, X.y, X.z, X.w, W, R);
    xi = f.xi; yi = f.yi; valid = f.valid; xf = f.xf; yf = f.yf;
  } else {
    const WarpFootF32 f = warp_foot_f32(P, X.x, X.y, X.z, X.w, j.dspace != 0, j.K[2], j.K[5], W, R);
    xi = f.xi; yi = f.yi; valid = f.valid;
#pragma unroll
    for(int k = 0; k < 4; ++k) cf[k] = f.cf[k];
  }

  if constexpr(HALF && C == 8 && !FAST) {
    if(valid) {
      const double wx = 1.0 - xf, wy = 1.0 - yf;
      const float4* q0 = reinterpret_cast<const float4*>(j.desc + ((size_t) yi * W + xi) * 8);
      const float4* q1 = q0 + (size_t) W * 2;
      const unsigned key = tap_key(xi, yi);
      const bool cached = j.tapcache_on != 0;
      const bool hit = cached && j.tapkey[i] == key;
      cache_hit = hit;
      float4* tc = reinterpret_cast<float4*>(j.tapcache.get());
      const float4* p0 = reinterpret_cast<const float4*>(j.pix.get());
#pragma unroll
      for(int h = 0; h < 2; ++h) {
        float4 a, b, c, d;
        if(hit) {
          a = load_v4<NT>(tc + tile_index<8>(i, h)); b = load_v4<NT>(tc + tile_index<8>(i, 2 + h));
          c = load_v4<NT>(tc + tile_index<8>(i, 4 + h)); d = load_v4<NT>(tc + tile_index<8>(i, 6 + h));
        } else {
          a = q0[h]; b = q0[2 + h]; c = q1[h]; d = q1[2 + h];
          if(in_block && cached) {
            store_v4<NT>(tc + tile_index<8>(i, h), a); store_v4<NT>(tc + tile_index<8>(i, 2 + h), b);
            store_v4<NT>(tc + tile_index<8>(i, 4 + h), c); store_v4<NT>(tc + tile_index<8>(i, 6 + h), d);
          }
        }
        const float4 t = load_v4<NT>(p0 + tile_index<2>(i, h));
        const float i00[4] = {a.x, a.y, a.z, a.w}, i01[4] = {b.x, b.y, b.z, b.w}, i10[4] = {c.x, c.y, c.z, c.w},
                    i11[4] = {d.x, d.y, d.z, d.w}, i0[4] = {t.x, t.y, t.z, t.w};
#pragma unroll
        for(int k = 0; k < 4; ++k) res[4 * h + k] = bilinear_res(i00[k], i01[k], i10[k], i11[k], i0[k], xf, yf, wx, wy);
        if(h == 0) __builtin_amdgcn_sched_barrier(0);
      }
      if(!hit && in_block && cached) j.tapkey[i] = key;
    } else {
#pragma unroll
      for(int c = 0; c < 8; ++c) res[c] = 0.0f;
    }
    return valid;
  }

  const int PT = (C == 8 || C == 1) ? C : j.pitch;
  if(valid) {
    const double wx = 1.0 - xf, wy = 1.0 - yf;
    const float* __restrict__ d0 = j.desc + ((size_t) yi * W + xi) * PT;
    const float* __restrict__ d1 = d0 + (size_t) W * PT;
    float I00[C], I01[C], I10[C], I11[C], I0[C];
    if constexpr(C == 8) {
      const unsigned key = tap_key(xi, yi);
      const bool cached = j.tapcache_on != 0;
      const bool hit = cached && j.tapkey[i] == key;
      cache_hit = hit;
      float4 t[8];
      if(hit) {
        const float4* tc = reinterpret_cast<const float4*>(j.tapcache.get());
#pragma unroll
        for(int k = 0; k < 8; ++k) t[k] = load_v4<NT>(tc + tile_index<8>(i, k));
      } else {
        taps8_gather(j, xi, yi, W, t);
        if(in_block && cached) taps8_cache_store<NT>(j, i, key, t);
      }
      const float4* p0 = reinterpret_cast<const float4*>(j.pix.get());
      const float4 t0 = load_v4<NT>(p0 + tile_index<2>(i, 0)), t1 = load_v4<NT>(p0 + tile_index<2>(i, 1));
      taps8_unpack(t, t0, t1, I00, I01, I10, I11, I0);
    } else if constexpr(C == 1) {
      const unsigned key = tap_key(xi, yi);
      float4* tc = reinterpret_cast<float4*>(j.tapcache.get());
      float4 t = spec_taps;
      const bool cached = j.tapcache_on != 0;
      cache_hit = cached && spec_key == key;
      if(!cache_hit) {
        t = make_float4(d0[0], d0[1], d1[0], d1[1]);
        if(in_block && cached) { store_v4<NT>(tc + i, t); j.tapkey[i] = key; }
      }
      I00[0] = t.x; I01[0] = t.y; I10[0] = t.z; I11[0] = t.w;
      I0[0] = spec_pix;
    } else {
#pragma unroll
      for(int c = 0; c < C; ++c) {
        I00[c] = d0[c]; I01[c] = d0[PT + c]; I10[c] = d1[c]; I11[c] = d1[PT + c];
        I0[c] = j.pix[(size_t) i * PT + c];
      }
    }
#pragma unroll
    for(int c = 0; c < C; ++c) {
      if constexpr(!FAST) {
        res[c] = bilinear_res(I00[c], I01[c], I10[c], I11[c], I0[c], xf, yf, wx, wy);
      } else {
        res[c] = bilinear_res_f32(I00[c], I01[c], I10[c], I11[c], I0[c], cf);
      }
    }
  } else {
    if constexpr(!FAST) {
#pragma unroll
      for(int c = 0; c < C; ++c) res[c] = 0.0f;
    } else {
      if constexpr(C == 8) {
        const float4* p0 = reinterpret_cast<const float4*>(j.pix.get());
        const float4 t0 = p0[tile_index<2>(i, 0)], t1 = p0[tile_index<2>(i, 1)];
        res[0] = 0.0f - t0.x; res[1] = 0.0f - t0.y; res[2] = 0.0f - t0.z; res[3] = 0.0f - t0.w;
        res[4] = 0.0f - t1.x; res[5] = 0.0f - t1.y; res[6] = 0.0f - t1.z; res[7] = 0.0f - t1.w;
      } else {
#pragma unroll
        for(int c = 0; c < C; ++c) res[c] = 0.0f - j.pix[(size_t) i * PT + c];
      }
    }
  }
  return valid;
}

template <int C, bool FAST>
__device__ __forceinline__ void warp_chunk(const PairJob& j, int mode, unsigned chunk, BracketLds& s, bool dense = false)
{
  const GNState* __restrict__ st = j.st;
  if(mode == 2) { if(!st->r_stale) return; }
  else {
    if(!st->active) return;
    if(mode == 1 && !(st->delta_scale > 1e-6f)) return;
  }
  const int n = j.n;
  if((int) (chunk * K6_BLOCK) >= n) return;

  if(mode != 2 && chunk == 0 && threadIdx.x == 0) j.cnt[4] += (unsigned long long) n;

  float P[12];
  if(FAST && j.dspace) dspace_matrix(j, mode == 2 ? st->T_lin : st->T, P);
  else projection_matrix(j, mode == 2 ? st->T_lin : st->T, P);

  const int i_raw = chunk * K6_BLOCK + threadIdx.x;
  const bool in_block = i_raw < n;
  const int i = in_block ? i_raw : n - 1;
  float res[C];
  bool hit;
  const bool valid = warp_point<C, FAST>(j, P, i, in_block, res, hit);
  if(in_block) j.valid[i] = valid ? 1 : 0;
  if(in_block) {
    if constexpr(C == 8) {
      float4* o = reinterpret_cast<float4*>(j.r.get());
      store_stream(o + tile_index<2>(i, 0), make_float4(res[0], res[1], res[2], res[3]));
      store_stream(o + tile_index<2>(i, 1), make_float4(res[4], res[5], res[6], res[7]));
    } else {
#pragma unroll
      for(int c = 0; c < C; ++c) j.r[(size_t) i * j.pitch + c] = res[c];
    }
  }
  if(mode != 2 && (st->delta_scale > 1e-6f) && st->median_valid) {
    if(dense) bracket_chunk<C, true>(j, st->lo_key, st->hi_key, valid && in_block, hit && valid && in_block, res, chunk, (int) (threadIdx.x >> 6), s, true);
    else bracket_chunk<C, false>(j, st->lo_key, st->hi_key, valid && in_block, hit && valid && in_block, res, chunk, (int) (threadIdx.x >> 6), s, true);
  }
}

}
```

### bpvo_amd/csrc/host_ctx.h

```cpp
#pragma once
#include <hip/hip_runtime.h>

#include <algorithm>
#include <atomic>
#include <chrono>
#include <cmath>
#include <cstdio>
#include <cstdlib>
#include <cstring>
#include <functional>
#include <condition_variable>
#include <memory>
#include <mutex>
#include <string>
#include <thread>
#include <vector>

#include "device_owned.h"
#include "frame_plan.h"
#include "gn_rounds.h"
#include "kernels.h"
#include "latch_table.h"
#include "rig_math.h"
#include "vo_state.h"

using namespace bpvo_hip;
#include "latch_table.h"

namespace bpvo_hip_host {

using namespace bpvo_hip;


extern std::atomic<int> g_live_ctx[64];
extern thread_local std::string g_create_error;

struct LevelGeom {
  int rows, cols;
  size_t npix;
  int nblk;
  int cap;
  int nms_radius;
  float K[9];
  float b;
};

struct FrameSlot {
  bool has_data = false, has_template = false;
  bool has_disp = false;
  DeviceBuf<unsigned char> data_slab, tmpl_slab;
  uint8_t* img[kMaxLevels] = {};
  uint8_t* cen[kMaxLevels] = {};
  float* ch0[kMaxLevels] = {};
  uint8_t lazy[kMaxLevels] = {};
  enum : uint8_t { SAL_STORED = 0, SAL_ON_DEMAND = 1, SAL_GONE = 2 };
  uint8_t sal_state[kMaxLevels] = {};
  bool ch0_valid = true;
  float* desc[kMaxLevels] = {};
  float* disp = nullptr;
  float* scratch = nullptr;
  float* sal[kMaxLevels] = {};
  uint8_t* flag[kMaxLevels] = {};
  int* blk_count[kMaxLevels] = {};
  float4* pts[kMaxLevels] = {};
  float2* ptc[kMaxLevels] = {};
  int* inds[kMaxLevels] = {};
  float* pix[kMaxLevels] = {};
  float* grad[kMaxLevels] = {};
  float* nrm = nullptr;
  int* n_dev = nullptr;
  int n_host[kMaxLevels] = {};
  bool own_geom = false;
  LevelGeom geom[kMaxLevels];
  const bpvo_hip_params* seq_params = nullptr;
  bool own_budget = false;
  int budget[kMaxLevels] = {};
  int budget_used[kMaxLevels] = {};
  float min_saliency_used = 0.0f;
  int* sel_info = nullptr;
};

struct Workspace {
  DeviceBuf<float> r;
  DeviceBuf<uint8_t> valid;
  DeviceBuf<uint32_t> cand, med_blk, tapkey;
  DeviceBuf<float> tapcache, partials;
  int last_ref = -1, last_cur = -1, last_level = -1;
  bool has_estimate = false;
};

struct CovScratch {
  int group = 0;
  DeviceBuf<unsigned char> d_slab;
  float* d_r = nullptr; size_t r_floats = 0;
  uint8_t* d_valid = nullptr; size_t valid_bytes = 0;
  float* d_partials = nullptr; size_t partial_floats = 0;
  unsigned long long* d_cnt = nullptr;
  GNState* d_states = nullptr;
  unsigned char* d_tables = nullptr;
  PinnedBuf<unsigned char> h_tables;
  size_t tables_bytes = 0, off_members = 0, off_T = 0, off_sigma = 0, off_X = 0;
  bpvo_hip_pose_covariance* d_out = nullptr;
  PinnedBuf<bpvo_hip_pose_covariance> h_out;
  float* d_sums = nullptr;
};

struct ScoreScratch {
  DeviceBuf<PairJob> d_jobs;
  DeviceBuf<float> d_T;
  DeviceBuf<ScorePartial> d_partials;
  DeviceBuf<bpvo_hip_pose_score> d_out;
};

struct RectMap {
  DeviceBuf<int2> d_map;
  int rows = 0, cols = 0;
  int raw_rows = 0, raw_cols = 0;
  uint64_t outside = 0;
};
struct RectState {
  RectMap own[2];
  std::vector<RectMap> seq;
  DeviceBuf<uint8_t> raw[2];
  DeviceBuf<uint8_t> out;
  PinnedBuf<RectifyFrame> h_tab; DeviceBuf<RectifyFrame> d_tab;
  Event tab_ev;
  uint64_t launches = 0, pixels = 0;
  Event t0, t1; bool timed = false;
};

struct FusionSeq {
  bpvo_hip_disparity_fusion prm = {0, 0.0f, 0.0f, 0.0f, 0.0f};
  bool own = false;
  DeviceBuf<unsigned char> slab;
  size_t npix = 0;
  float* Dc = nullptr; float* Vc = nullptr; unsigned long long* zbuf = nullptr;
  bool carried = false;
  bpvo_hip_disparity_fusion_info info = {};
};
// ... 135 lines not shown
  std::vector<SeqState> seqs;
  DeviceBuf<bpvo_hip_point_with_info> d_seq_cloud;
  PinnedBuf<PairJob> h_seq_jobs;
  DeviceBuf<PairJob> d_seq_jobs;
  PinnedBuf<CloudJob> h_cloud_jobs;
  DeviceBuf<CloudJob> d_cloud_jobs;
  PinnedBuf<unsigned> h_seq_cnt;
  DeviceBuf<unsigned> d_seq_cnt;
  PinnedBuf<size_t> h_seq_off;
  DeviceBuf<size_t> d_seq_off;
  std::vector<RigState> rigs;
  DeviceBuf<float> d_rig_X;
  DeviceBuf<char> d_rig_stage; PinnedBuf<char> h_rig_stage;
  DeviceBuf<int> d_rig_active; PinnedBuf<int> h_rig_active;
  int pose_covariance = 0;
  CovScratch cov;
  bpvo_hip_pose_covariance vo_cov;
  std::vector<bpvo_hip_pose_covariance> seq_cov;
  ScoreScratch score;
  double points_fused = 0;
  int fast_warp = 0;
  int dspace = 0;
  int fuse_frozen = 1;
  int G = 1, Cg = 0;
  int reference_reduction = 0;
  int step_in_reduce_max = 128;
  int persistent = 1, persist_max_ws = 1, persist_grid = 64;
  int persist_max_points = 32768;
  int dense_candidates_from = 32768;
  long long persist_timeout = 50000000ll;
  int team_mode = 1, team_max_pairs = 128, team_full_pairs = 80, team_size_env = 0, num_cus = 0, device_cus = 0;
  int team_join = 2;
  int merge_levels_max_frames = 8;
  int small_batch_fused = 1;
  int nrm_dpp_asm = 4;
  int nrm_side_stream = 1;
  int nrm_defer = 1;
  int team_split_max_pairs = 4;
  Stream side_stream, side_stream2;
  Stream copy_stream;
  Event copy_ev;
  std::function<int()> before_final_sync;
  int vo_disparity_late = 1;
  Event side_ev[4];
  hipEvent_t nrm_pending = nullptr;
  hipEvent_t nrm_pending_finest = nullptr;
  int team_spares = 1;
  int team_join_from_pairs = 48;
  int team_local_barriers = 1;
  std::atomic<uint64_t> team_launches{0};
  std::atomic<uint64_t> team_joins{0};
  std::atomic<bool> persistent_failed{false};
  std::atomic<uint64_t> persistent_levels{0};
  DeviceBuf<float> d_trace;
  int trace_ws = -1;
  int max_lanes_now = 1 << 30;
  DeviceBuf<uint8_t> st_left, st_right, st_left_pre, st_right_pre;
  DeviceBuf<float> st_disp;
  DeviceBuf<float> st_var;
  size_t st_pixels = 0;
  DeviceBuf<unsigned char> st_sgm;
  PinnedBuf<StereoFrame> h_st_frames; DeviceBuf<StereoFrame> d_st_frames;
  Event st_tab_ev;
  int stereo_frames_per_launch = 0;
  size_t st_sgm_budget = 0, st_free_seen = 0;
  int st_frames_per_launch_seen = 0;
  RectState rect;
  FusionState fusion;
  VarianceState variance;
  MotionStereoState motion_stereo;
  int up_workers = 6;
  std::atomic<bool> ctl_by_kernel{false};
  Stream up_stream;
  std::vector<PinnedBuf<uint8_t>> up_pinned;
  std::vector<Event> up_slot_free;
  std::vector<Event> up_chunk_done;
  size_t up_slot_bytes = 0;
  DeviceBuf<uint8_t> up_d_img;
  DeviceBuf<float> up_d_disp;
  double up_plan[2] = {0.19, 0.50};
  int points_from_compact = 0;
  int lazy_template = 1;
  int lazy_saliency = 1;
  int keep_current_disparity = 0;
  double up_last_seconds = 0.0;
  size_t up_last_bytes = 0;
  bool counted_live = false;
  float prefetch_frac_thr = -1.0f;
  bool frac_valid = false; int frac_ws = -1; float frac_thr = 0.0f; unsigned frac_cnt = 0; int frac_n = 0;
  double tapcache_max_density = 0.5;
  bool stagger = true;
  int stagger_min_pairs = 192;
  int census_taps[2] = {0, 0};
  bool profiling = false;
  bool profile_all = false;
  bool profile_k6_all = false;
  double kc_ms[KC_COUNT] = {};
  double kc_units[KC_COUNT] = {};
  uint64_t kc_launches[KC_COUNT] = {};
  uint64_t total_lin = 0, median_bracketed = 0, median_full = 0;
  uint64_t tscale_stages = 0, tscale_passes = 0;
  uint64_t tap_counts[4] = {};
  std::mutex units_mu;
  std::string err;
};

namespace bpvo_hip_host {

#define HIP_CK(ctx_, expr)                                                                  \
  do {                                                                                      \
    hipError_t e_ = (expr);                                                                 \
    if(e_ != hipSuccess) {                                                                  \
      (ctx_)->err = std::string(#expr) + ": " + hipGetErrorString(e_);                      \
      return BPVO_ERR_DEVICE;                                                               \
    }                                                                                       \
  } while(0)

#define LANE_CK(ln_, expr)                                                                  \
  do {                                                                                      \
    hipError_t e_ = (expr);                                                                 \
    if(e_ != hipSuccess) {                                                                  \
      (ln_)->err = std::string(#expr) + ": " + hipGetErrorString(e_);                       \
      (void) hipStreamSynchronize((ln_)->stream);                                           \
      return BPVO_ERR_DEVICE;                                                               \
    }                                                                                       \
  } while(0)

inline int auto_pyramid_levels(int rows, int cols, int minImageDimensionForPyramid)
{
  return 1 + (int) std::round(std::log2(std::min(rows, cols) / (double) minImageDimensionForPyramid));
}

Event take_event(Lane* ln);
struct ScopedTimer {
  Lane* ln;
  EventPair ep;
  bool on;
  hipStream_t st;
  ScopedTimer(bpvo_hip_ctx* c_, int kc, double units, Lane* lane = nullptr, bool sampled = true, hipStream_t stream = nullptr)
      : ln(lane ? lane : &c_->lanes[0]), on(c_->profiling && sampled), st(stream ? stream : (lane ? lane : &c_->lanes[0])->stream)
  {
    if(!on) return;
    ep.kc = kc; ep.units = units;
    ep.a = take_event(ln); ep.b = take_event(ln);
    (void) hipEventRecord(ep.a, st);
  }
  ~ScopedTimer()
  {
    if(!on) return;
    (void) hipEventRecord(ep.b, st);
    ln->ev_pending.push_back(std::move(ep));
  }
};

struct FrameRun {
  hipStream_t stream;
  Lane* ln;
  int tab;
  bool own_thread;
  hipEvent_t selected_ev;
  std::function<void()> on_selected;
  bool defer_finest_nrm = false;
  bool no_final_sync = false;
  bool skip_disparity_upload = false;
};
#define FR_CK(c_, fr_, expr)                                                                \
// ... 13 lines not shown
int check_point_budget(bpvo_hip_ctx* c, const int* max_points, int n_levels);

int fail(bpvo_hip_ctx* c, int code, const char* msg);
void gaussian_kernel5(double sigma, float k[3]);
void gaussian_taps(int n, double sigma, GaussTaps* g);
int imsmooth_taps(float sigma);
int auto_gauss_taps_f32(float sigma);
void carve_frame_data(bpvo_hip_ctx* c, FrameSlot& f, unsigned char* base, size_t* total);
void carve_frame_tmpl(bpvo_hip_ctx* c, FrameSlot& f, unsigned char* base, size_t* total);
hipError_t ensure_template_storage(bpvo_hip_ctx* c, FrameSlot& f, hipStream_t stream);
FrameJob make_frame_job(bpvo_hip_ctx* c, FrameSlot& f, int l);
PairJob make_pair_job(bpvo_hip_ctx* c, int ws, int ref, int cur, int l);
void pair_job_set_params(PairJob& j, const bpvo_hip_params& p);
void resolve_events(bpvo_hip_ctx* c);
FrameRun ctx_run(bpvo_hip_ctx* c);
std::vector<int> strided_slots(int first, int stride, int count);
int upload_frame_jobs(bpvo_hip_ctx* c, const int* slots, int count, const FrameRun& fr, int which, const FrameJob** tab);
inline bpvo_hip::FrameLaunch frame_launch(const bpvo_hip_ctx* c, const FrameJob* tab, const LevelGeom* geom, LevelSpan span, int count)
{
  return bpvo_hip::FrameLaunch{tab + (size_t) span.first * c->n_frames, geom[span.first].cols, geom[span.first].rows, count, span.count, c->n_frames};
}
int frames_set_data_slots(bpvo_hip_ctx* c, const int* slots, int count, const uint8_t* images, const float* disps, bool on_device, const FrameRun& fr,
                          int skip_odd_disp = 0, const size_t* offsets = nullptr);
int frames_set_template_slots(bpvo_hip_ctx* c, const int* slots, int count, const FrameRun& fr);
int frames_set_data(bpvo_hip_ctx* c, int first, int stride, int count, const uint8_t* images, const float* disps, bool on_device, int skip_odd_disp = 0);
int frames_set_template(bpvo_hip_ctx* c, int first, int stride, int count);
int upload_disparity(bpvo_hip_ctx* c, int slot, const float* disparity);
bool team_serves(const bpvo_hip_ctx* c, int n);
PairJob group_pair_job(const bpvo_hip_ctx* c, const PairJob& whole, int k);
inline int job_tables(const bpvo_hip_ctx* c) { return c->G > 1 ? 1 + c->G : 1; }
template <class F>
inline void for_each_group(const bpvo_hip_ctx* c, const bpvo_hip::GNLaunch& g, size_t stride, F&& f)
{
  if(c->G <= 1) { f(g); return; }
  for(int k = 0; k < c->G; ++k) {
    bpvo_hip::GNLaunch gg = g;
    gg.jobs = g.jobs + (size_t) (1 + k) * stride;
    gg.C = c->Cg;
    f(gg);
  }
}
inline size_t med_totals_at(const bpvo_hip_ctx* c) { return (((size_t) ((c->cap_max + bpvo_hip::kChunkPoints - 1) / bpvo_hip::kChunkPoints) * (size_t) c->G) + 7) / 8 * 8; }
inline hipError_t join_pending_normalization(bpvo_hip_ctx* c, hipStream_t s, int level = -1)
{
  hipError_t e = hipSuccess;
  if(c->nrm_pending) { e = hipStreamWaitEvent(s, c->nrm_pending, 0); c->nrm_pending = nullptr; }
  if(c->nrm_pending_finest && (level < 0 || level <= c->params.maxTestLevel)) {
    const hipError_t e2 = hipStreamWaitEvent(s, c->nrm_pending_finest, 0);
    c->nrm_pending_finest = nullptr;
    if(e == hipSuccess) e = e2;
  }
  return e;
}
inline bool templates_may_be_dense(const bpvo_hip_ctx* c)
{
  for(int l = c->params.maxTestLevel; l < c->L; ++l)
    if(c->geom[l].nms_radius <= 0 && c->geom[l].npix > (size_t) std::max(0, c->persist_max_points)) return true;
  return false;
}
inline bool loss_is_chain_only(int loss) { return loss == BPVO_LOSS_STUDENT_T; }
inline bool single_pair_is_queued_at_once(const bpvo_hip_ctx* c)
{
  return c->persistent && !c->persistent_failed.load() && !c->profile_all && !c->reference_reduction && !loss_is_chain_only(c->params.lossFunction) &&
         (c->C == 8 || c->C == 1) && c->params.interp == BPVO_INTERP_LINEAR && !c->fast_warp && !templates_may_be_dense(c);
}
inline int dense_candidates(const bpvo_hip_ctx* c, int max_points) { return (c->G == 1 && max_points >= c->dense_candidates_from) ? 1 : 0; }
inline bpvo_hip::GNLaunch median_launch(const bpvo_hip_ctx* c, bpvo_hip::GNLaunch g) { if(c->G > 1) g.C = c->Cg; return g; }
inline bpvo_hip::GNLaunch level_launch(const bpvo_hip_ctx* c, const bpvo_hip::PairJob* jobs, int npairs, int max_points, int loss)
{
  bpvo_hip::GNLaunch g;
  g.jobs = jobs; g.npairs = npairs; g.max_points = max_points; g.C = c->C; g.loss = loss;
  g.fast_warp = c->fast_warp; g.interp = c->params.interp;
  g.reference_reduction = c->reference_reduction ? 1 : 0;
  g.dense_candidates = dense_candidates(c, max_points);
  return g;
}
enum LinearizeTimers { TIMERS_OFF, TIMERS_ESTIMATE, TIMERS_LEVEL2, TIMERS_ALWAYS };
struct LinearizeFlags {
  bool warp = true, median = true, reduce = true, step = true;
  int step_mode = 0;
  LinearizeTimers timers = TIMERS_OFF;
};
void linearize_launches(bpvo_hip_ctx* c, Lane* ln, const bpvo_hip::GNLaunch& g, size_t stride, const LinearizeFlags& f);
int check_pairs(bpvo_hip_ctx* c, int n, const int* wss, const int* refs, const int* curs, int level_lo, int level_hi);
int estimate_group(bpvo_hip_ctx* c, Lane* ln, int n, const int* wss, const int* refs, const int* curs, const float* T_init, float* poses,
                   bpvo_hip_stats* stats, float* d_records_out, bool allow_persistent, const bpvo_hip_params* const* prms = nullptr);
int estimate_batch(bpvo_hip_ctx* c, int n, const int* wss, const int* refs, const int* curs, const float* T_init, float* poses, bpvo_hip_stats* stats,
                   const bpvo_hip_params* const* prms = nullptr);
int estimate_rig(bpvo_hip_ctx* c, int n, const int* wss, const int* refs, const int* curs, const float* X, const float* T_init, float* T_est, bpvo_hip_stats* stats);
struct RigProblem {
  int n;
  const int* wss; const int* refs; const int* curs;
  const float* X;
  const float* T_init;
  float* T_est;
  bpvo_hip_stats* stats;
  const bpvo_hip_params* prm;
};
int estimate_rigs(bpvo_hip_ctx* c, int R, const RigProblem* rigs);
inline size_t rig_stage_X_at(const bpvo_hip_ctx* c) { return (sizeof(bpvo_hip::RigEntry) * (size_t) c->n_pairs + 63) / 64 * 64; }
inline size_t rig_stage_bytes(const bpvo_hip_ctx* c) { return rig_stage_X_at(c) + 2 * sizeof(float) * 16 * (size_t) c->n_pairs; }
void detile_to_channel_major(const float* src, int n, int C, int E, int V, float* out);
size_t tiled_floats(int n, int floats_per_point);
int refresh_counters(bpvo_hip_ctx* c);
int upload_single_job(bpvo_hip_ctx* c, int ws, int ref, int cur, int level);
int ensure_residuals(bpvo_hip_ctx* c, int ws);
int fraction_good(bpvo_hip_ctx* c, int ws, float thr, float* frac);
int get_weights_host(bpvo_hip_ctx* c, int ws, std::vector<float>& w_cm, int* n_out);
int check_template_not_empty(bpvo_hip_ctx* c, int ref_slot);
int ensure_lanes(bpvo_hip_ctx* c, int n);
int lanes_for(bpvo_hip_ctx* c, int n, int cap);
int ensure_saliency(bpvo_hip_ctx* c, int slot, int level);
int ensure_dense_descriptor(bpvo_hip_ctx* c, int slot);
int pose_cov_pass(bpvo_hip_ctx* c, int n_records, int members, const int* wss, const int* refs, const int* curs, const float* X, int level,
                  const float* T, const float* sigma, const bpvo_hip_params* const* prms, bpvo_hip_pose_covariance* out);
int pose_cov_ensure_scratch(bpvo_hip_ctx* c);
void pose_cov_none(bpvo_hip_pose_covariance* r);
int pose_score_served(bpvo_hip_ctx* c);
int score_pairs(bpvo_hip_ctx* c, int n_pairs, const int* refs, const int* curs, int level, int n_poses, const float* T, float tau,
                bpvo_hip_pose_score* out);
inline int seq_capacity(const bpvo_hip_ctx* c) { return std::max(0, std::min(c->n_frames / 3, c->n_pairs)); }
const RectMap* rect_map_of(const bpvo_hip_ctx* c, int seq, int side);
struct RectSide { int side; const uint8_t* raw; uint8_t* dst; };
int rectify_queue(bpvo_hip_ctx* c, int n, const int* seq , int n_sides, const RectSide* sides, bool on_device);
int rect_clear(bpvo_hip_ctx* c, int seq);
struct FusionItem { int seq; int slot; const float* P; const float* R = nullptr; int view_slot = -1; const float* T_view = nullptr; };
bool fusion_on(const bpvo_hip_ctx* c, int seq);
int fusion_stage(bpvo_hip_ctx* c, int n, const FusionItem* items);
void fusion_seq_reset(bpvo_hip_ctx* c, int seq);
double fusion_last_ms(bpvo_hip_ctx* c, int which);
struct StereoSize;
int variance_front(bpvo_hip_ctx* c, int n, const StereoSize* sz, const int* ids, const uint8_t* d_left, const uint8_t* d_right);
const float* variance_map_of(const bpvo_hip_ctx* c, int seq);
inline void variance_call_done(bpvo_hip_ctx* c) { c->variance.live = false; }
void variance_seq_reset(bpvo_hip_ctx* c, int seq);
int variance_scratch_moved(bpvo_hip_ctx* c, size_t npix);
int stereo_reserve(bpvo_hip_ctx* c, size_t npix);
double variance_last_ms(bpvo_hip_ctx* c);
struct MotionStereoView { int seq; int slot; int view_slot; const float* T; unsigned long long* zbuf; };
bool motion_stereo_on(const bpvo_hip_ctx* c, int seq);
int motion_stereo_stage(bpvo_hip_ctx* c, int n, const MotionStereoView* views, bool* launched);
void motion_stereo_seq_reset(bpvo_hip_ctx* c, int seq);
double motion_stereo_last_ms(bpvo_hip_ctx* c);
int fuse_disparities_impl(bpvo_hip_ctx* c, int n, const int* seq, const float* disparities, const float* variances, int on_device, const float* poses);
struct StereoSize { int rows, cols; };
int stereo_front(bpvo_hip_ctx* c, int n, const StereoSize* sz, const int* ids, const uint8_t* left, const uint8_t* right, bool raw, bool on_device,
                 const bpvo_hip_stereo_params* sp, const uint8_t** d_left);
int seq_fail(bpvo_hip_ctx* c, int code, int seq, const char* what);
int camera_too_large(bpvo_hip_ctx* c, int seq, int rows, int cols);
int set_option(bpvo_hip_ctx* c, const std::string& key, double v);
int apply_options_string(bpvo_hip_ctx* c, const char* str);
struct OptionDef { const char* key; double lo, hi; std::function<double(bpvo_hip_ctx*)> get; std::function<int(bpvo_hip_ctx*, double)> set; };
const std::vector<OptionDef>& option_table();

}

#define CHECK_CTX(c) if(!(c)) return BPVO_ERR_INVALID_ARG
#define CHECK_SLOT(c, s) if((s) < 0 || (s) >= (c)->n_frames) return fail(c, BPVO_ERR_INVALID_ARG, "bad frame slot")
#define CHECK_WS(c, w) if((w) < 0 || (w) >= (c)->n_pairs) return fail(c, BPVO_ERR_INVALID_ARG, "bad workspace")
#define CHECK_LEVEL(c, l) if((l) < (c)->params.maxTestLevel || (l) >= (c)->L) return fail(c, BPVO_ERR_INVALID_ARG, "bad level")
```

### bpvo_amd/csrc/kernels.h

```cpp
#pragma once

#include <hip/hip_runtime.h>

#include "types.h"

#include <type_traits>

template <class F>
static inline void dispatch_channels(int C, F&& f)
{
  switch(C) {
    case 1: f(std::integral_constant<int, 1>()); break;
    case 3: f(std::integral_constant<int, 3>()); break;
    case 5: f(std::integral_constant<int, 5>()); break;
    case 10: f(std::integral_constant<int, 10>()); break;
    case 16: f(std::integral_constant<int, 16>()); break;
    case 32: f(std::integral_constant<int, 32>()); break;
    case 24: f(std::integral_constant<int, 24>()); break;
    case 48: f(std::integral_constant<int, 48>()); break;
    default: f(std::integral_constant<int, 8>()); break;
  }
}

template <class F>
static inline bool dispatch_wide_channels(int C, F&& f)
{
  switch(C) {
    case 64: f(std::integral_constant<int, 64>()); return true;
    case 80: f(std::integral_constant<int, 80>()); return true;
    case 120: f(std::integral_constant<int, 120>()); return true;
    case 128: f(std::integral_constant<int, 128>()); return true;
    case 168: f(std::integral_constant<int, 168>()); return true;
    case 224: f(std::integral_constant<int, 224>()); return true;
    case 256: f(std::integral_constant<int, 256>()); return true;
    case 288: f(std::integral_constant<int, 288>()); return true;
    case 360: f(std::integral_constant<int, 360>()); return true;
    case 512: f(std::integral_constant<int, 512>()); return true;
    default: return false;
  }
}

namespace bpvo_hip {

inline size_t align_up(size_t v, size_t a = 256) { return (v + a - 1) / a * a; }
struct Carver {
  unsigned char* base;
  size_t off = 0;
  template <typename T>
  T* take(size_t count)
  {
    T* p = base ? reinterpret_cast<T*>(base + off) : nullptr;
    off += align_up(count * sizeof(T));
    return p;
  }
};

constexpr int kMaxGaussTaps = 31;
struct GaussTaps { int n = 0; float k[kMaxGaussTaps] = {}; int ki[kMaxGaussTaps] = {}; };

void launch_ingest(hipStream_t s, const FrameJob* jobs_level0, const uint8_t* d_images, const float* d_disps, size_t npix, int nframes, int skip_odd_disp = 0);
void launch_ingest_at(hipStream_t s, const FrameJob* jobs_level0, const uint8_t* d_images, const float* d_disps, const size_t* d_offsets, size_t npix, int nframes);
void launch_pyrdown(hipStream_t s, const FrameJob* src, const FrameJob* dst, int dW, int dR, int nframes);
void launch_pyramid_levels(hipStream_t s, const FrameJob* src_row, int job_pitch, int steps, int dW, int dR, int nframes);
struct FrameLaunch { const FrameJob* jobs; int W, R, nframes, nlevels, job_pitch; };
void launch_intensity(hipStream_t s, const FrameLaunch& f);
void launch_intensity_norm(hipStream_t s, const FrameLaunch& f, int radius);
void launch_gradient_descriptor(hipStream_t s, const FrameJob* jobs, int W, int R, int nframes, const GaussTaps& pre);
void launch_descriptor_fields(hipStream_t s, const FrameJob* jobs, int W, int R, int nframes, int second_order, const GaussTaps& g1,
                              const GaussTaps& g2);
void launch_central_difference(hipStream_t s, const FrameJob* jobs, int W, int R, int nframes, int radius, const GaussTaps& before,
                               const GaussTaps& after);
void launch_latch(hipStream_t s, const FrameJob* jobs, int W, int R, int nframes, int bytes, int half_ssd, const signed char* d_offsets, int kc, int ks,
                  const GaussTaps& after);
void launch_laplacian(hipStream_t s, const FrameJob* jobs, int W, int R, int nframes, int ksize );
void launch_census(hipStream_t s, const FrameLaunch& f, const int* blur_taps );
void launch_bitplanes_pairs(hipStream_t s, const FrameLaunch& f, const float k[3]);
void launch_census_templates(hipStream_t s, const FrameLaunch& f);
void launch_bitplanes(hipStream_t s, const FrameLaunch& f, float sigma, const float k[3], int from_image);
enum { SELECT_ALL = 0, SELECT_CANDIDATES = 1, SELECT_COMPACT = 2 };
void launch_saliency_select(hipStream_t s, const FrameLaunch& f, int C, int nms_radius, int border, const float gauss_k[3], int part);
void launch_point_budget(hipStream_t s, const FrameLaunch& f, int nms_radius);
void launch_saliency(hipStream_t s, const FrameLaunch& f, int C);
void launch_copy_rows(hipStream_t s, void* dst, const void* src_host_pinned, size_t pitch_bytes, size_t width_bytes, int rows);
void launch_gather_counts(hipStream_t s, const FrameJob* jobs , int job_pitch, int nframes, int first_level, int num_levels,
                          int* out );
void launch_normalization(hipStream_t s, const FrameJob* jobs , int job_pitch, int nframes, int first_level,
                          int num_levels, int with_normalization, int form = 1);
void launch_export_jacobians(hipStream_t s, const FrameJob* job , int C, int n, float* out );
void launch_template_build(hipStream_t s, const FrameLaunch& f, int C, int max_points, int grad_cd5, const float gauss_k[3]);

struct StereoFrame { int rows, cols; size_t offset; };
struct StereoLaunch {
  const uint8_t* left_pre;
  const uint8_t* right_pre;
  float* disp;
  int rows, cols, nframes;
  const StereoFrame* frames = nullptr;
  size_t total_pixels = 0;
  int wsz, ndisp, mindisp, cap, texture_threshold, uniqueness_ratio;
};
void launch_stereo_prefilter(hipStream_t s, const uint8_t* src, uint8_t* dst, int rows, int cols, int cap, int nframes);
void launch_stereo_prefilter_frames(hipStream_t s, const uint8_t* src, uint8_t* dst, const StereoFrame* frames , int max_rows, int max_cols,
                                    int cap, int nframes);
bool launch_stereo_bm(hipStream_t s, const StereoLaunch& g);
struct RectifyFrame { int rows, cols, raw_rows, raw_cols; const int2* map; const uint8_t* src; uint8_t* dst; };
void launch_rectify_frames(hipStream_t s, const RectifyFrame* frames , int nframes, int max_rows, int max_cols);
struct FusionJob {
  int rows, cols, predict, pad_;
  float fx, fy, cx, cy, b, lo, hi;
  float r2, q2, gate, fill2;
  float P[12];
  float* slot;
  float* Dc;
  float* Vc;
  unsigned long long* zbuf;
  unsigned* counts;
  const float* R;
};
void launch_fusion_splat(hipStream_t s, const FusionJob* jobs , int njobs, size_t max_pixels);
void launch_fusion_update(hipStream_t s, const FusionJob* jobs , int njobs, size_t max_pixels);
struct VarianceJob {
  const uint8_t* L;
  const uint8_t* R;
  const float* M;
  float* out;
  unsigned* counts;
  int rows, cols, radius, pad_;
  float lo, hi, noise2, min2, max2;
};
constexpr int kVarianceCounters = 6 + 3;
void launch_disparity_variance(hipStream_t s, const VarianceJob* jobs , int njobs, int max_tiles);
int disparity_variance_tiles(int rows, int cols);
struct MotionStereoJob {
  const uint8_t* C;
  const uint8_t* K;
  unsigned long long* zbuf;
  const float* pd;
  const float* pv;
  float* out_d;
  float* out_v;
  uint8_t* out_c;
  unsigned* counts;
  double fx, fy, cx, cy, R[9], e[3];
  int rows, cols, radius, steps;
  float lo, hi, min_gain, noise2, min2, max2, gate, pad_;
};
constexpr int kMotionStereoCounters = 7 + 3;
void launch_motion_stereo(hipStream_t s, const MotionStereoJob* jobs , int njobs, int max_tiles);
int motion_stereo_tiles(int rows, int cols);

struct SgmLaunch {
  const uint8_t* left;
  const uint8_t* right;
  float* disp;
  void* scratch;
  int rows, cols, nframes;
  int frames_per_launch = 1;
  int ndisp, sobel_cap, census_radius, window_radius, P1, P2, consistency_threshold;
  double disparity_factor, census_weight;
};
// ... 153 lines not shown
```

### bpvo_amd/csrc/kernels_frame.hip

```cpp
#include <algorithm>
#include <cstdlib>

#include "frame_common.h"

namespace bpvo_hip {

__device__ __forceinline__ const FrameJob& level_job(const FrameJob* jobs, unsigned z, int nframes, int job_pitch, int job_step = 1)
{
  const unsigned lvl = z / (unsigned) nframes;
  return jobs[(size_t) lvl * job_pitch + (size_t) (z - lvl * (unsigned) nframes) * job_step];
}

template <bool AT>
__global__ __launch_bounds__(256) void ingest_kernel(const FrameJob* jobs, const uint8_t* images, const float* disps, size_t npix, int skip_odd_disp,
                                                     const size_t* __restrict__ offs)
{
  const FrameJob& j = jobs[blockIdx.z];
  const uint8_t* __restrict__ si = images + (AT ? offs[blockIdx.z] : (size_t) blockIdx.z * npix);
  const float* __restrict__ sd = disps + (AT ? offs[blockIdx.z] : (size_t) (skip_odd_disp == 2 ? blockIdx.z / 2 : blockIdx.z) * npix);
  uint8_t* __restrict__ di = const_cast<uint8_t*>(j.img.get());
  float* __restrict__ dd = const_cast<float*>(j.disp.get());
  const size_t t = (size_t) blockIdx.x * 256 + threadIdx.x, stride = (size_t) gridDim.x * 256;
  const bool w4 = (npix % 4 == 0) && (((uintptr_t) si | (uintptr_t) di) % 4 == 0);
  if(w4) {
// ... 153 lines not shown
      const int x2 = 2 * (xlo[k + 1] + c);
      const uint8_t* row = cur + r * pc - xlo[k];
      const unsigned a0 = row[reflect101(x2 - 2, W[k])], a1 = row[reflect101(x2 - 1, W[k])], a2 = row[x2], a3 = row[reflect101(x2 + 1, W[k])],
                     a4 = row[reflect101(x2 + 2, W[k])];
      s_h[r * E1 + c] = (uint16_t) (a0 + 4u * a1 + 6u * a2 + 4u * a3 + a4);
    }
    __syncthreads();
    const int sh = NL - (k + 1);
    const int ox0 = (blockIdx.x * PA_T) << sh, ox1 = min(((blockIdx.x + 1) * PA_T) << sh, W[k + 1]);
    const int oy0 = (blockIdx.y * PA_T) << sh, oy1 = min(((blockIdx.y + 1) * PA_T) << sh, H[k + 1]);
    uint8_t* __restrict__ dst = const_cast<uint8_t*>(jobs[(size_t) (k + 1) * job_pitch + blockIdx.z].img.get());
    for(int i = tid; i < dny * dnx; i += 256) {
      const int r = i / dnx, c = i - r * dnx;
      const int y = ylo[k + 1] + r, x = xlo[k + 1] + c, y2 = 2 * y;
      const uint16_t* col = s_h + c - ylo[k] * E1;
      const unsigned b0 = col[reflect101(y2 - 2, H[k]) * E1], b1 = col[reflect101(y2 - 1, H[k]) * E1], b2 = col[y2 * E1],
                     b3 = col[reflect101(y2 + 1, H[k]) * E1], b4 = col[reflect101(y2 + 2, H[k]) * E1];
      const uint8_t v = (uint8_t) ((b0 + 4u * b1 + 6u * b2 + 4u * b3 + b4 + 128u) >> 8);
      nxt[r * pn + c] = v;
      if(x >= ox0 && x < ox1 && y >= oy0 && y < oy1) dst[(size_t) y * W[k + 1] + x] = v;
    }
    __syncthreads();
    { uint8_t* t = cur; cur = nxt; nxt = t; }
    { const int t = pc; pc = pn; pn = t; }
  }
}
void launch_pyramid_levels(hipStream_t s, const FrameJob* src_row, int job_pitch, int steps, int dW, int dR, int nframes)
{
  const dim3 grid((dW + PA_T - 1) / PA_T, (dR + PA_T - 1) / PA_T, nframes);
  if(steps == 3) hipLaunchKernelGGL(pyramid_levels_kernel<3>, grid, dim3(256), 0, s, src_row, job_pitch);
  else if(steps == 2) hipLaunchKernelGGL(pyramid_levels_kernel<2>, grid, dim3(256), 0, s, src_row, job_pitch);
  else hipLaunchKernelGGL(pyramid_levels_kernel<1>, grid, dim3(256), 0, s, src_row, job_pitch);
}

__global__ __launch_bounds__(256) void intensity_kernel(const FrameJob* jobs, int nframes, int job_pitch)
{
  const FrameJob& j = level_job(jobs, blockIdx.z, nframes, job_pitch);
  const int n = j.rows * j.cols;
  const int i = (blockIdx.x * 256 + threadIdx.x) * 4;
  if(i >= n) return;
  if(i + 3 < n && ((uintptr_t) (j.img + i) & 3) == 0) {
    const uchar4 v = *reinterpret_cast<const uchar4*>(j.img + i);
    *reinterpret_cast<float4*>(j.desc + i) = make_float4((float) v.x, (float) v.y, (float) v.z, (float) v.w);
  } else {
    for(int k = i; k < n && k < i + 4; ++k) j.desc[k] = (float) j.img[k];
  }
}

constexpr int ROWS_PER_THREAD = 4;
constexpr int CENSUS_ROWS = 8;
__global__ __launch_bounds__(256) void census_kernel(const FrameJob* jobs)
{
  const FrameJob& j = jobs[blockIdx.z];
  const int x = blockIdx.x * 64 + (threadIdx.x & 63);
  const int y0 = (blockIdx.y * 4 + (threadIdx.x >> 6)) * CENSUS_ROWS;
  const int W = j.cols, R = j.rows;
  if(x >= W || y0 >= R) return;
  const bool xin = x > 0 && x < W - 1;
  const int xm = max(x - 1, 0), xp = min(x + 1, W - 1);
  uint8_t w[CENSUS_ROWS + 2][3];
#pragma unroll
  for(int k = 0; k < CENSUS_ROWS + 2; ++k) {
    const uint8_t* p = j.img + (size_t) min(max(y0 - 1 + k, 0), R - 1) * W;
    w[k][0] = p[xm]; w[k][1] = p[x]; w[k][2] = p[xp];
  }
#pragma unroll
  for(int k = 0; k < CENSUS_ROWS; ++k) {
    const int y = y0 + k;
    if(y < R) {
      uint8_t out = 0;
      if(xin && y > 0 && y < R - 1) {
        const uint8_t ctr = w[k + 1][1];
        out = (uint8_t) (((w[k][0] >= ctr) << 0) | ((w[k][1] >= ctr) << 1) | ((w[k][2] >= ctr) << 2) | ((w[k + 1][0] >= ctr) << 3) |
                         ((w[k + 1][2] >= ctr) << 4) | ((w[k + 2][0] >= ctr) << 5) | ((w[k + 2][1] >= ctr) << 6) | ((w[k + 2][2] >= ctr) << 7));
      }
      j.cen[(size_t) y * W + x] = out;
    }
  }
}

typedef unsigned int u32_unaligned __attribute__((aligned(1)));
typedef unsigned short u16_unaligned __attribute__((aligned(1)));
constexpr int CT_ROWS = 8, CT_PX = 4;
__global__ __launch_bounds__(256) void census_templates_kernel(const FrameJob* jobs, int nframes, int job_pitch)
{
  const FrameJob& j = level_job(jobs, blockIdx.z, nframes, job_pitch, 2);
  if(j.lazy != 2) return;
  const int W = j.cols, R = j.rows;
  const int x = (blockIdx.x * 64 + (threadIdx.x & 63)) * CT_PX;
  const int y0 = (blockIdx.y * 4 + (threadIdx.x >> 6)) * CT_ROWS;
  if(x >= W || y0 >= R) return;
  const uint8_t* __restrict__ img = j.img;
  uint8_t* __restrict__ cen = j.cen;
  const bool inner = x >= 1 && x + CT_PX < W;
  unsigned long long w[CT_ROWS + 2];
#pragma unroll
  for(int k = 0; k < CT_ROWS + 2; ++k) {
    const uint8_t* p = img + (size_t) min(max(y0 - 1 + k, 0), R - 1) * W;
    if(inner) {
      w[k] = (unsigned long long) *reinterpret_cast<const u32_unaligned*>(p + x - 1) |
             ((unsigned long long) *reinterpret_cast<const u16_unaligned*>(p + x + 3) << 32);
    } else {
      unsigned long long v = 0;
#pragma unroll
      for(int q = 0; q < CT_PX + 2; ++q) v |= (unsigned long long) p[min(max(x - 1 + q, 0), W - 1)] << (8 * q);
      w[k] = v;
    }
  }
#pragma unroll
  for(int k = 0; k < CT_ROWS; ++k) {
    const int y = y0 + k;
    if(y >= R) break;
    const bool yin = y > 0 && y < R - 1;
    unsigned out4 = 0;
#pragma unroll
    for(int q = 0; q < CT_PX; ++q) {
      const unsigned a = (unsigned) (w[k] >> (8 * q)), b = (unsigned) (w[k + 1] >> (8 * q)), c = (unsigned) (w[k + 2] >> (8 * q));
      const unsigned ctr = (b >> 8) & 0xffu;
      unsigned out = (((a & 0xffu) >= ctr) << 0) | ((((a >> 8) & 0xffu) >= ctr) << 1) | ((((a >> 16) & 0xffu) >= ctr) << 2) | (((b & 0xffu) >= ctr) << 3) |
                     ((((b >> 16) & 0xffu) >= ctr) << 4) | (((c & 0xffu) >= ctr) << 5) | ((((c >> 8) & 0xffu) >= ctr) << 6) | ((((c >> 16) & 0xffu) >= ctr) << 7);
      if(!(yin && x + q > 0 && x + q < W - 1)) out = 0;
      out4 |= out << (8 * q);
    }
    uint8_t* o = cen + (size_t) y * W + x;
    if(x + CT_PX <= W) *reinterpret_cast<u32_unaligned*>(o) = out4;
    else
      for(int q = 0; q < W - x; ++q) o[q] = (uint8_t) (out4 >> (8 * q));
  }
}

constexpr int CB_TW = 64, CB_TH = 4;
__global__ __launch_bounds__(256) void census_blur_kernel(const FrameJob* jobs, int kc, int ks, int nframes, int job_pitch)
{
  __shared__ uint8_t s_src[(CB_TH + 4) * (CB_TW + 4)];
  __shared__ int s_tmp[(CB_TH + 4) * (CB_TW + 2)];
  __shared__ uint8_t s_b[(CB_TH + 2) * (CB_TW + 2)];
  const FrameJob& j = level_job(jobs, blockIdx.z, nframes, job_pitch);
  const int W = j.cols, R = j.rows;
  const int x0 = blockIdx.x * CB_TW, y0 = blockIdx.y * CB_TH;
  if(x0 >= W || y0 >= R) return;
  const int tid = threadIdx.x;
  for(int i = tid; i < (CB_TH + 4) * (CB_TW + 4); i += 256) {
    const int ly = i / (CB_TW + 4), lx = i - ly * (CB_TW + 4);
    const int gy = reflect101(min(y0 + ly - 2, R + 1), R), gx = reflect101(min(x0 + lx - 2, W + 1), W);
    s_src[i] = j.img[(size_t) gy * W + gx];
  }
  __syncthreads();
  for(int i = tid; i < (CB_TH + 4) * (CB_TW + 2); i += 256) {
    const int ly = i / (CB_TW + 2), lx = i - ly * (CB_TW + 2);
    const uint8_t* p = s_src + ly * (CB_TW + 4) + lx + 1;
    s_tmp[i] = (int) p[0] * kc + ((int) p[-1] + (int) p[1]) * ks;
  }
  __syncthreads();
  for(int i = tid; i < (CB_TH + 2) * (CB_TW + 2); i += 256) {
    const int ly = i / (CB_TW + 2), lx = i - ly * (CB_TW + 2);
    const int* t = s_tmp + (ly + 1) * (CB_TW + 2) + lx;
    const int v = (t[0] * kc + (t[-(CB_TW + 2)] + t[CB_TW + 2]) * ks + (1 << 15)) >> 16;
    s_b[i] = (uint8_t) min(255, max(0, v));
  }
  __syncthreads();
  const int lx = tid & 63, ly = tid >> 6;
  const int x = x0 + lx, y = y0 + ly;
  if(x >= W || y >= R) return;
  uint8_t out = 0;
  if(x > 0 && x < W - 1 && y > 0 && y < R - 1) {
    constexpr int P = CB_TW + 2;
    const uint8_t* p = s_b + (ly + 1) * P + lx + 1;
    const uint8_t c = p[0];
    out = (uint8_t) (((p[-P - 1] >= c) << 0) | ((p[-P] >= c) << 1) | ((p[-P + 1] >= c) << 2) | ((p[-1] >= c) << 3) |
// ... 1341 lines not shown
__global__ void gather_counts_kernel(const FrameJob* jobs, int job_pitch, int nframes, int first_level, int num_levels, int* out )
{
  const int t = blockIdx.x * blockDim.x + threadIdx.x;
  if(t >= nframes * kMaxLevels) return;
  const int i = t / kMaxLevels, l = t - i * kMaxLevels;
  out[t] = (l >= first_level && l < num_levels) ? *jobs[(size_t) l * job_pitch + i].n_out : 0;
}

template <int C>
__global__ __launch_bounds__(256) void export_jacobians_kernel(const FrameJob* job, float* out)
{
  const FrameJob& j = *job;
  const int N = *j.n_out;
  const int i = blockIdx.x * 256 + threadIdx.x;
  if(i >= N) return;
  const float4 P = j.pts[i];
  const JacPoint jp = jac_point(P.x, P.y, P.z, j.nrm);
  float Ix[C], Iy[C];
  if constexpr(C == 8) {
    const float4* gv = reinterpret_cast<const float4*>(j.grad.get());
    const float4 a = gv[tile_index<4>(i, 0)], b = gv[tile_index<4>(i, 1)], c = gv[tile_index<4>(i, 2)], d = gv[tile_index<4>(i, 3)];
    Ix[0] = a.x; Ix[1] = a.y; Ix[2] = a.z; Ix[3] = a.w; Ix[4] = b.x; Ix[5] = b.y; Ix[6] = b.z; Ix[7] = b.w;
    Iy[0] = c.x; Iy[1] = c.y; Iy[2] = c.z; Iy[3] = c.w; Iy[4] = d.x; Iy[5] = d.y; Iy[6] = d.z; Iy[7] = d.w;
  } else {
#pragma unroll
    for(int c = 0; c < C; ++c) { Ix[c] = j.grad[((size_t) i * 2 + 0) * C + c]; Iy[c] = j.grad[((size_t) i * 2 + 1) * C + c]; }
  }
#pragma unroll
  for(int c = 0; c < C; ++c) {
    float J[6];
    if(j.dspace) dspace_jac_row(P.x, P.y, P.z, j.K[0], j.K[4], 1.0f / j.K[0], 1.0f / j.K[4], 1.0f / j.b, Ix[c], Iy[c], J);
    else jac_row(jp, Ix[c], Iy[c], J);
    float* o = out + ((size_t) c * N + i) * 6;
#pragma unroll
    for(int k = 0; k < 6; ++k) o[k] = J[k];
  }
}

__global__ __launch_bounds__(256) void export_jacobians_wide_kernel(const FrameJob* job, int C, float* out)
{
  const FrameJob& j = *job;
  const int N = *j.n_out;
  const size_t k = (size_t) blockIdx.x * 256 + threadIdx.x;
  if(k >= (size_t) N * C) return;
  const int c = (int) (k / N), i = (int) (k - (size_t) c * N);
  const float4 P = j.pts[i];
  const float Ix = j.grad[((size_t) i * 2 + 0) * C + c], Iy = j.grad[((size_t) i * 2 + 1) * C + c];
  float J[6];
  if(j.dspace) dspace_jac_row(P.x, P.y, P.z, j.K[0], j.K[4], 1.0f / j.K[0], 1.0f / j.K[4], 1.0f / j.b, Ix, Iy, J);
  else jac_row(jac_point(P.x, P.y, P.z, j.nrm), Ix, Iy, J);
  float* o = out + k * 6;
#pragma unroll
  for(int q = 0; q < 6; ++q) o[q] = J[q];
}

static inline dim3 grid2d_rows(int W, int R, int nz) { return dim3((W + 63) / 64, (R + 4 * ROWS_PER_THREAD - 1) / (4 * ROWS_PER_THREAD), nz); }

void launch_ingest(hipStream_t s, const FrameJob* jobs_level0, const uint8_t* d_images, const float* d_disps, size_t npix, int nframes, int skip_odd_disp)
{
  const int blocks = (int) std::min<size_t>(256, (npix / 4 + 255) / 256);
  hipLaunchKernelGGL(ingest_kernel<false>, dim3(blocks, 1, nframes), dim3(256), 0, s, jobs_level0, d_images, d_disps, npix, skip_odd_disp, nullptr);
}
void launch_ingest_at(hipStream_t s, const FrameJob* jobs_level0, const uint8_t* d_images, const float* d_disps, const size_t* d_offsets, size_t npix, int nframes)
{
  const int blocks = (int) std::min<size_t>(256, (npix / 4 + 255) / 256);
  hipLaunchKernelGGL(ingest_kernel<true>, dim3(blocks, 1, nframes), dim3(256), 0, s, jobs_level0, d_images, d_disps, npix, 0, d_offsets);
}
void launch_pyrdown(hipStream_t s, const FrameJob* src, const FrameJob* dst, int dW, int dR, int nframes)
{
  hipLaunchKernelGGL(pyrdown_u8_lds_kernel, dim3((dW + PDT_W - 1) / PDT_W, (dR + PDT_H * PD_STACK - 1) / (PDT_H * PD_STACK), nframes), dim3(256), 0, s, src, dst);
}
void launch_intensity(hipStream_t s, const FrameLaunch& f)
{
  hipLaunchKernelGGL(intensity_kernel, dim3((f.W * f.R + 1023) / 1024, 1, f.nframes * f.nlevels), dim3(256), 0, s, f.jobs, f.nframes, f.job_pitch);
}
void launch_census(hipStream_t s, const FrameLaunch& f, const int* blur_taps)
{
  if(blur_taps)
    hipLaunchKernelGGL(census_blur_kernel, dim3((f.W + CB_TW - 1) / CB_TW, (f.R + CB_TH - 1) / CB_TH, f.nframes * f.nlevels), dim3(256), 0, s,
                       f.jobs, blur_taps[0], blur_taps[1], f.nframes, f.job_pitch);
  else
    hipLaunchKernelGGL(census_kernel, dim3((f.W + 63) / 64, (f.R + 4 * CENSUS_ROWS - 1) / (4 * CENSUS_ROWS), f.nframes), dim3(256), 0, s, f.jobs);
}
void launch_census_templates(hipStream_t s, const FrameLaunch& f)
{
  const int na = (f.nframes + 1) / 2;
  hipLaunchKernelGGL(census_templates_kernel, dim3((f.W + 64 * CT_PX - 1) / (64 * CT_PX), (f.R + 4 * CT_ROWS - 1) / (4 * CT_ROWS), na * f.nlevels), dim3(256), 0, s,
                     f.jobs, na, f.job_pitch);
}
void launch_bitplanes(hipStream_t s, const FrameLaunch& f, float sigma, const float k[3], int from_image)
{
  const int stack = f.nframes >= 16 ? 8 : (f.nframes > 4 ? 4 : 1);
  const dim3 grid((f.W + BP_TW - 1) / BP_TW, (f.R + BP_TH * stack - 1) / (BP_TH * stack), f.nframes * f.nlevels);
  if(sigma > 0.0f && from_image)
    hipLaunchKernelGGL(bitplanes_blur_kernel<true>, grid, dim3(256), 0, s, f.jobs, k[0], k[1], k[2], stack, f.nframes, f.job_pitch, 1, 0);
  else if(sigma > 0.0f)
    hipLaunchKernelGGL(bitplanes_blur_kernel<false>, grid, dim3(256), 0, s, f.jobs, k[0], k[1], k[2], stack, f.nframes, f.job_pitch, 1, 0);
  else
    hipLaunchKernelGGL(bitplanes_noblur_kernel, dim3((f.W * f.R + 255) / 256, 1, f.nframes), dim3(256), 0, s, f.jobs);
}
void launch_bitplanes_pairs(hipStream_t s, const FrameLaunch& f, const float k[3])
{
  const int stack = f.nframes >= 16 ? 8 : (f.nframes > 4 ? 4 : 1);
  const int ncols = (f.W + BP_TW - 1) / BP_TW, nrows = (f.R + BP_TH * stack - 1) / (BP_TH * stack);
  int dense = 0;
  for(int cx = 0; cx < ncols; ++cx) dense += bp_tile_column_is_lazy(cx * BP_TW, f.W) ? 0 : 1;
  const int na = (f.nframes + 1) / 2, nb = f.nframes / 2;
  if(nb > 0) hipLaunchKernelGGL(bitplanes_blur_kernel<true>, dim3(ncols, nrows, nb), dim3(256), 0, s, f.jobs + 1, k[0], k[1], k[2], stack, nb, 0, 2, 0);
  if(dense > 0) hipLaunchKernelGGL(bitplanes_blur_kernel<true>, dim3(dense, nrows, na), dim3(256), 0, s, f.jobs, k[0], k[1], k[2], stack, na, 0, 2, 1);
}
void launch_saliency(hipStream_t s, const FrameLaunch& f, int C)
{
  auto plain = [&](auto c) { hipLaunchKernelGGL(saliency_kernel<decltype(c)::value>, grid2d_rows(f.W, f.R, f.nframes), dim3(256), 0, s, f.jobs); };
  if(C <= 48 || !dispatch_wide_channels(C, plain)) dispatch_channels(C, plain);
}
void launch_saliency_select(hipStream_t s, const FrameLaunch& f, int C, int nms_radius, int border, const float gauss_k[3], int part)
{
  const bool form = part != SELECT_COMPACT, compact = part != SELECT_CANDIDATES;
  if(nms_radius <= 1) {
    const int WPR = (f.W + 63) / 64, nw = f.R * WPR;
    auto tile = [&](auto c) {
      hipLaunchKernelGGL(saliency_select_tile_kernel<decltype(c)::value>, dim3(WPR, (f.R + ST_H - 1) / ST_H, f.nframes * f.nlevels), dim3(256), 0, s, f.jobs,
                         border, f.nframes, f.job_pitch, gauss_k[0], gauss_k[1], gauss_k[2]);
    };
    if(form && (C <= 48 || !dispatch_wide_channels(C, tile))) dispatch_channels(C, tile);
    if(!compact) return;
    hipLaunchKernelGGL(select_words_scan_kernel, dim3(f.nframes * f.nlevels), dim3(1024), 0, s, f.jobs, f.nframes, f.job_pitch);
    hipLaunchKernelGGL(select_words_write_kernel, dim3((nw + 4 * SW_WORDS - 1) / (4 * SW_WORDS), 1, f.nframes * f.nlevels), dim3(256), 0, s, f.jobs, f.nframes,
                       f.job_pitch);
    return;
  }
  const int nblk = (f.W * f.R + SEL_BLOCK_PX - 1) / SEL_BLOCK_PX;
  if(form) {
    launch_saliency(s, f, C);
    hipLaunchKernelGGL(select_flag_kernel, dim3(nblk, 1, f.nframes), dim3(256), 0, s, f.jobs, border);
  }
  if(!compact) return;
  hipLaunchKernelGGL(select_scan_kernel, dim3(f.nframes), dim3(1024), 0, s, f.jobs);
  hipLaunchKernelGGL(select_write_kernel, dim3(nblk, 1, f.nframes), dim3(256), 0, s, f.jobs);
}
void launch_point_budget(hipStream_t s, const FrameLaunch& f, int nms_radius)
{
  if(nms_radius <= 1) hipLaunchKernelGGL(point_budget_kernel<true>, dim3(f.nframes * f.nlevels), dim3(PB_THREADS), 0, s, f.jobs, f.nframes, f.job_pitch);
  else hipLaunchKernelGGL(point_budget_kernel<false>, dim3(f.nframes), dim3(PB_THREADS), 0, s, f.jobs, f.nframes, 0);
}
__global__ __launch_bounds__(256) void copy_rows_kernel(unsigned long long* __restrict__ dst, const unsigned long long* __restrict__ src, size_t pitch8,
                                                        size_t width8, int rows)
{
  const size_t n = width8 * (size_t) rows;
  for(size_t i = (size_t) blockIdx.x * 256 + threadIdx.x; i < n; i += (size_t) gridDim.x * 256) {
    const size_t r = i / width8, k = i - r * width8;
    dst[r * pitch8 + k] = src[r * pitch8 + k];
  }
}
void launch_copy_rows(hipStream_t s, void* dst, const void* src_host_pinned, size_t pitch_bytes, size_t width_bytes, int rows)
{
  const size_t n = width_bytes / 8 * (size_t) rows;
  if(n == 0) return;
  hipLaunchKernelGGL(copy_rows_kernel, dim3((unsigned) std::min<size_t>(64, (n + 255) / 256)), dim3(256), 0, s, (unsigned long long*) dst,
                     (const unsigned long long*) src_host_pinned, pitch_bytes / 8, width_bytes / 8, rows);
}
void launch_normalization(hipStream_t s, const FrameJob* jobs, int job_pitch, int nframes, int first_level, int num_levels,
                          int with_normalization, int form)
{
  const dim3 grid(nframes, num_levels - first_level);
  if(form == 4) form = (nframes * (num_levels - first_level) <= 1024) ? 3 : 1;
  if(form == 3) hipLaunchKernelGGL(normalization_kernel<3>, grid, dim3(NRM_THREADS), 0, s, jobs, job_pitch, first_level, with_normalization);
  else if(form == 2) hipLaunchKernelGGL(normalization_kernel<2>, grid, dim3(NRM_THREADS), 0, s, jobs, job_pitch, first_level, with_normalization);
  else if(form == 1) hipLaunchKernelGGL(normalization_kernel<1>, grid, dim3(NRM_THREADS), 0, s, jobs, job_pitch, first_level, with_normalization);
  else hipLaunchKernelGGL(normalization_kernel<0>, grid, dim3(NRM_THREADS), 0, s, jobs, job_pitch, first_level, with_normalization);
}
void launch_gather_counts(hipStream_t s, const FrameJob* jobs, int job_pitch, int nframes, int first_level, int num_levels, int* out)
{
  hipLaunchKernelGGL(gather_counts_kernel, dim3((nframes * kMaxLevels + 255) / 256), dim3(256), 0, s, jobs, job_pitch, nframes, first_level,
                     num_levels, out);
}
void launch_template_build(hipStream_t s, const FrameLaunch& f, int C, int max_points, int grad_cd5, const float gauss_k[3])
{
  if(max_points <= 0) return;
  const dim3 g((max_points + 255) / 256, 1, f.nframes * f.nlevels);
  if(C > 48) { hipLaunchKernelGGL(template_build_wide_kernel, g, dim3(256), 0, s, f.jobs, C, grad_cd5, f.nframes, f.job_pitch); return; }
  dispatch_channels(C, [&](auto c) {
    hipLaunchKernelGGL(template_build_kernel<decltype(c)::value>, g, dim3(256), 0, s, f.jobs, grad_cd5, gauss_k[0], gauss_k[1], gauss_k[2], f.nframes, f.job_pitch);
  });
}

void launch_export_jacobians(hipStream_t s, const FrameJob* job, int C, int n, float* out)
{
  if(n <= 0) return;
  const dim3 g((n + 255) / 256);
  if(C > 48) { hipLaunchKernelGGL(export_jacobians_wide_kernel, dim3((unsigned) (((size_t) n * C + 255) / 256)), dim3(256), 0, s, job, C, out); return; }
// ... 5 lines not shown
```

### bpvo_amd/csrc/kernels_gn.hip

```cpp
#include <float.h>

#include <algorithm>
#include <cstdlib>

#include <mutex>

#include "kernels.h"

#include "gn_common.h"
#include "gn_warp.h"
#include "gn_median.h"
#include "gn_tscale.h"
#include "gn_irls.h"
#include "gn_step.h"

namespace bpvo_hip {

template <int C, bool FAST>
__global__ __launch_bounds__(K6_BLOCK) void warp_residual_kernel(const PairJob* __restrict__ jobs, ActiveSet act, int mode, int dense)
{
  __shared__ BracketLds s;
  warp_chunk<C, FAST>(jobs[active_workspace(act, blockIdx.y)], mode, blockIdx.x, s, dense != 0);
}

__global__ void clear_stale_kernel(const PairJob* jobs, int n)
{
  const int p = blockIdx.x * blockDim.x + threadIdx.x;
  if(p < n) jobs[p].st->r_stale = 0;
}

__device__ __forceinline__ void interp_cosine(float x, float (&c)[2])
{
  const double m = (1.0 - cos((double) x * 3.14159265358979323846)) / 2.0;
  c[0] = (float) (1.0 - m);
  c[1] = (float) m;
}
__device__ __forceinline__ void interp_cubic(float x, float (&c)[4])
{
  const float A = -0.5f;
  c[0] = ((A * (x + 1.0f) - 5.0f * A) * (x + 1.0f) + 8.0f * A) * (x + 1.0f) - 4.0f * A;
  c[1] = ((A + 2.0f) * x - (A + 3.0f)) * x * x + 1.0f;
  c[2] = ((A + 2.0f) * (1.0f - x) - (A + 3.0f)) * (1.0f - x) * (1.0f - x) + 1.0f;
  c[3] = 1.0f - c[0] - c[1] - c[2];
}
__device__ __forceinline__ float interp_hermite(float y0, float y1, float y2, float y3, float mu)
{
  const float mu2 = mu * mu;
  const float mu3 = mu * mu2;
  const float m0 = (float) (((double) (y1 - y0) / 2.0) + ((double) (y2 - y1) / 2.0));
  const float m1 = (float) (((double) (y2 - y1) / 2.0) + ((double) (y3 - y2) / 2.0));
  const float a0 = 2 * mu3 - 3 * mu2 + 1;
  const float a1 = mu3 - 2 * mu2 + mu;
  const float a2 = mu3 - mu2;
  const float a3 = -2 * mu3 + 3 * mu2;
  return a0 * y1 + a1 * m0 + a2 * m1 + a3 * y2;
}
__device__ __forceinline__ float dot4(float a0, float a1, float a2, float a3, const float (&b)[4])
{
  return (a0 * b[0] + a1 * b[1]) + (a2 * b[2] + a3 * b[3]);
}

template <int C> struct InterpGroup { static constexpr int G = (C % 8 == 0) ? 8 : (C % 4 == 0) ? 4 : (C % 2 == 0) ? 2 : 1; };
template <int G>
__device__ __forceinline__ void load_group(const float* __restrict__ p, float (&v)[G])
{
  if constexpr(G == 8) {
    const float4 a = reinterpret_cast<const float4*>(p)[0], b = reinterpret_cast<const float4*>(p)[1];
    v[0] = a.x; v[1] = a.y; v[2] = a.z; v[3] = a.w; v[4] = b.x; v[5] = b.y; v[6] = b.z; v[7] = b.w;
  } else if constexpr(G == 4) { const float4 t = *reinterpret_cast<const float4*>(p); v[0] = t.x; v[1] = t.y; v[2] = t.z; v[3] = t.w; }
  else if constexpr(G == 2) { const float2 t = *reinterpret_cast<const float2*>(p); v[0] = t.x; v[1] = t.y; }
  else v[0] = p[0];
}

#ifndef ROW_BARRIER_AT
#define ROW_BARRIER_AT 1
#endif
template <int C, int INTERP>
__global__ __launch_bounds__(K6_BLOCK) void warp_residual_interp_kernel(const PairJob* __restrict__ jobs, ActiveSet act, int dense)
{
  constexpr int interp = INTERP;
  const PairJob& j = jobs[active_workspace(act, blockIdx.y)];
  const GNState* __restrict__ st = j.st;
  if(!st->active) return;
  const int n = j.n;
  if((int) (blockIdx.x * K6_BLOCK) >= n) return;
  if(blockIdx.x == 0 && threadIdx.x == 0) j.cnt[4] += (unsigned long long) n;

  float P[12];
  projection_matrix(j, st->T, P);

  const int i_raw = blockIdx.x * K6_BLOCK + threadIdx.x;
  const bool in_block = i_raw < n;
  const int i = in_block ? i_raw : n - 1;
  const int W = j.cols, R = j.rows;
  const float4 X = load_point<false>(j, i);
  constexpr bool two_tap = interp == BPVO_INTERP_COSINE;
  constexpr int border_lo = two_tap ? 0 : 1, border_hi = two_tap ? 1 : 3;
  const WarpFoot ft = warp_foot<border_lo, border_hi>(P, X.x, X.y, X.z, X.w, W, R);
  const int xi = ft.xi, yi = ft.yi;
  const bool valid = ft.valid;
  const float xf = (float) ft.xf, yf = (float) ft.yf;
  if(in_block) j.valid[i] = valid ? 1 : 0;

  constexpr int G = InterpGroup<C>::G;
  const size_t PT = (C == 8 || C == 1) ? (size_t) C : (size_t) j.pitch;
// ... 700 lines not shown
```

### bpvo_amd/csrc/types.h

```cpp
#pragma once

#include <stdint.h>

#include "../../include/bpvo_hip/c_api.h"
#include "device_math.h"

namespace bpvo_hip {

constexpr int kMaxLevels = BPVO_HIP_MAX_LEVELS;
constexpr int kHistBins1 = 2048;
constexpr int kReduceVals = 28;
constexpr int kPartialStride = 32;
constexpr int kWsCounters = 12;
constexpr int kRecordFloats = 32;
constexpr int kTraceFloats = BPVO_HIP_TRACE_FLOATS;
constexpr int kMaxGroups = 16;

#ifndef BPVO_TILE_VALUE
#define BPVO_TILE_VALUE 2048
#endif
constexpr int kTile = BPVO_TILE_VALUE;
template <int PIECES>
__host__ __device__ inline size_t tile_index(int i, int piece)
{
// ... 57 lines not shown
  float T_out[16];
  float T_lin[16];
  int   r_stale;
  int   trace_n;
  GNParams prm;
};

#if defined(__HIPCC__)
typedef float bpvo_v4f __attribute__((ext_vector_type(4)));
__device__ __forceinline__ float4 load_stream(const float4* p)
{
  const bpvo_v4f v = __builtin_nontemporal_load(reinterpret_cast<const bpvo_v4f*>(p));
  return make_float4(v.x, v.y, v.z, v.w);
}
__device__ __forceinline__ void store_stream(float4* p, const float4& a)
{
  bpvo_v4f v; v.x = a.x; v.y = a.y; v.z = a.z; v.w = a.w;
  __builtin_nontemporal_store(v, reinterpret_cast<bpvo_v4f*>(p));
}
__device__ __forceinline__ float2 compact_point(float z, int x, int y) { return make_float2(z, __uint_as_float((unsigned) x | ((unsigned) y << 16))); }
typedef float bpvo_v2f __attribute__((ext_vector_type(2)));
template <bool NT>
__device__ __forceinline__ float2 load_v2(const float2* p)
{
  if constexpr(NT) {
    const bpvo_v2f v = __builtin_nontemporal_load(reinterpret_cast<const bpvo_v2f*>(p));
    return make_float2(v.x, v.y);
  } else return *p;
}
template <bool NT>
__device__ __forceinline__ float4 load_v4(const float4* p) { if constexpr(NT) return load_stream(p); else return *p; }
template <bool NT>
__device__ __forceinline__ void store_v4(float4* p, const float4& a) { if constexpr(NT) store_stream(p, a); else *p = a; }
#endif

template <class T>
struct GPtr {
#if defined(__HIP_DEVICE_COMPILE__)
  typedef T __attribute__((address_space(1)))* raw_t;
#else
  typedef T* raw_t;
#endif
  raw_t p;
  __host__ __device__ operator T*() const { return (T*) p; }
  __host__ __device__ T* get() const { return (T*) p; }
  __host__ __device__ T* operator->() const { return (T*) p; }
  __host__ __device__ GPtr& operator=(T* q) { p = (raw_t) q; return *this; }
};

static_assert(sizeof(GPtr<float>) == sizeof(float*) && alignof(GPtr<float>) == alignof(float*), "GPtr must be layout-compatible with a plain pointer: the host fills the tables the device reads");

struct PairJob {
  GPtr<const float4> pts;
  GPtr<const float2> ptc;
  GPtr<const float> pix;
  GPtr<const float> grad;
  GPtr<const float> nrm;
  int           n;
  GPtr<const float> desc;
  int           rows, cols;
  float         K[9];
  float         b;
  float         f_inv[2];
  int           dspace;
  GPtr<float> r;
  GPtr<uint8_t> valid;
  GPtr<uint32_t> tapkey;
  int           tapcache_on;
  GPtr<float> tapcache;
  GPtr<uint32_t> cand;
  GPtr<uint32_t> med_blk;
  GPtr<float> partials;
  GPtr<unsigned long long> cnt;
  GPtr<GNState> st;
  GPtr<unsigned> ticket;
  GPtr<float> trace;
  int           trace_cap;
  int           pitch;
  int           n_groups;
  int           med_tot;
  GNParams      prm;
  int           loss;
  float         good_thr;
};

struct InormScratch { uint32_t bins[256]; float table[256]; uint32_t ticket; uint32_t pad[31]; };

constexpr int kDfPlanes = 7;
struct FrameJob {
  GPtr<const uint8_t> img;
  GPtr<uint8_t> cen;
  GPtr<float> desc;
  GPtr<float> ch0;
  GPtr<float> scratch;
  GPtr<InormScratch> inorm;
  GPtr<float> sal;
  GPtr<uint8_t> flag;
  GPtr<unsigned long long> words;
  GPtr<int> blk_count;
  GPtr<int> n_out;
  GPtr<const float> disp;
  GPtr<float4> pts;
  GPtr<float2> ptc;
  GPtr<int> inds;
  GPtr<float> pix;
  GPtr<float> grad;
  GPtr<float> nrm;
  int            rows, cols, level, disp_cols;
  int            cap;
  int            nms_radius;
  float          K[9];
  float          b;
  int            dspace;
  float          min_saliency, min_disp, max_disp;
  int            max_points;
  GPtr<int> sel_info;
  int            lazy;
};

}
```

Before: 1.357 million GN iterations/s.

## Compute current-frame bitplane descriptors lazily from census during warp

Current frames at pyramid levels whose descriptor is otherwise fully materialised now keep only the census bytes. The GN warp kernel rebuilds the needed 8-channel bit-plane taps on demand into the tap cache, and also prefills that cache for frozen pairs. This is meant to avoid the dense blurred-bitplane pass and its memory writes for current frames. In exchange, the warp gains extra census decode and blur arithmetic on tap-cache misses. Paths that cannot read census fall back to building the dense descriptor.

New measurement: 1.336 million GN iterations/s. 1.5% lower.

```diff
diff --git a/__graft_entry__.py b/__graft_entry__.py
--- a/__graft_entry__.py
+++ b/__graft_entry__.py
@@ -13,7 +13,7 @@
 MGPU_LIB = os.path.join(CSRC, "libbpvo_hip_mgpu.so")
 
 HIP_SOURCES = ["context.hip", "frames.hip", "estimate.hip", "batch.hip", "vo.hip", "measure.hip", "kernels_frame.hip", "kernels_intensity_norm.hip", "kernels_planes.hip", "kernels_gn.hip", "kernels_gn_ref.hip", "kernels_gn_team.hip", "kernels_gn_rig.hip", "kernels_gn_cov.hip", "pose_cov.hip", "kernels_score.hip", "score.hip", "kernels_stereo.hip", "kernels_sgm.hip", "kernels_sgbm.hip", "kernels_rectify.hip", "rectify.hip", "stereo.hip", "kernels_disparity_fusion.hip", "disparity_fusion.hip", "kernels_disparity_variance.hip", "disparity_variance.hip", "kernels_motion_stereo.hip", "motion_stereo.hip"]
-HIP_HEADERS = ["host_ctx.h", "device_owned.h", "vo_state.h", "gn_rounds.h", "frame_plan.h", "kernels.h", "types.h", "device_math.h", "gn_common.h", "gn_warp.h", "warp_rule.h", "gn_median.h", "gn_tscale.h", "tscale_math.h", "gn_irls.h", "gn_step.h", "rig_math.h", "pose_cov_math.h", "pose_score_math.h", "rectify_math.h", "intensity_norm_math.h", "disparity_fusion_math.h", "disparity_variance_math.h", "motion_stereo_math.h", "gn_cov.h", "frame_common.h", "latch_table.h", "sg_scanline.h",
+HIP_HEADERS = ["host_ctx.h", "device_owned.h", "vo_state.h", "gn_rounds.h", "frame_plan.h", "kernels.h", "types.h", "device_math.h", "gn_common.h", "gn_warp.h", "gn_census_taps.h", "warp_rule.h", "gn_median.h", "gn_tscale.h", "tscale_math.h", "gn_irls.h", "gn_step.h", "rig_math.h", "pose_cov_math.h", "pose_score_math.h", "rectify_math.h", "intensity_norm_math.h", "disparity_fusion_math.h", "disparity_variance_math.h", "motion_stereo_math.h", "gn_cov.h", "frame_common.h", "latch_table.h", "sg_scanline.h",
                os.path.join("..", "..", "include", "bpvo_hip", "c_api.h")]
 HIPCC_FLAGS = ["--offload-arch=gfx950", "-O3", "-std=c++17", "-ffp-contract=off", "-fPIC", "-Wall", "-Wno-unused-function"]
 OBJ_DIR = os.path.join(CSRC, "obj")
diff --git a/bpvo_amd/csrc/batch.hip b/bpvo_amd/csrc/batch.hip
--- a/bpvo_amd/csrc/batch.hip
+++ b/bpvo_amd/csrc/batch.hip
@@ -213,10 +213,19 @@
 
 extern "C" {
 
+static int batch_run(bpvo_hip_ctx* c, int n_pairs, const uint8_t* images, const float* disparities, int on_device, float* poses, bpvo_hip_stats* stats);
 int bpvo_hip_batch_run(bpvo_hip_ctx* c, int n_pairs, const uint8_t* images, const float* disparities, int on_device,
                        float* poses, bpvo_hip_stats* stats)
 {
   CHECK_CTX(c);
+  c->lazy_current_call = (c->lazy_current == 2 || (c->lazy_current == 1 && n_pairs > c->team_max_pairs)) && c->C == 8 &&
+                         c->params.interp == BPVO_INTERP_LINEAR && !c->fast_warp && !c->reference_reduction;
+  const int rc = batch_run(c, n_pairs, images, disparities, on_device, poses, stats);
+  c->lazy_current_call = false;
+  return rc;
+}
+static int batch_run(bpvo_hip_ctx* c, int n_pairs, const uint8_t* images, const float* disparities, int on_device, float* poses, bpvo_hip_stats* stats)
+{
   if(n_pairs < 0 || 2 * n_pairs > c->n_frames || n_pairs > c->n_pairs) return fail(c, BPVO_ERR_INVALID_ARG, "batch exceeds ctx capacity");
   for(int i = 0; i < 2 * n_pairs; ++i)
     if(c->frames[i].own_geom) return fail(c, BPVO_ERR_UNSUPPORTED, "pair batches run the context's camera: its slots carry per-sequence cameras (bpvo_hip_seq_set_camera)");
diff --git a/bpvo_amd/csrc/context.hip b/bpvo_amd/csrc/context.hip
--- a/bpvo_amd/csrc/context.hip
+++ b/bpvo_amd/csrc/context.hip
@@ -148,6 +148,11 @@
   j.nrm = fr.nrm + 4 * l;
   j.n = fr.n_host[l];
   j.desc = fc.desc[l];
+  if(fc.census_current && fc.lazy[l] == 2) {
+    j.desc = nullptr;
+    j.cen = fc.cen[l];
+    j.bk[0] = c->gauss_k[0]; j.bk[1] = c->gauss_k[1]; j.bk[2] = c->gauss_k[2];
+  }
   j.rows = g.rows; j.cols = g.cols;
   std::memcpy(j.K, g.K, sizeof(j.K));
   j.b = g.b;
@@ -335,6 +340,7 @@
               }},
     OPT_INT("lazy_template_descriptor", lazy_template, 0, 1),
     OPT_INT("lazy_template_saliency", lazy_saliency, 0, 1),
+    OPT_INT("lazy_current_descriptor", lazy_current, 0, 2),
     OPT_INT("points_from_compact_stream", points_from_compact, 0, 1),
     OptionDef{"tapcache_max_density", 0.0, 1e9, [](bpvo_hip_ctx* c) { return c->tapcache_max_density; },
               [](bpvo_hip_ctx* c, double v) { c->tapcache_max_density = v; return BPVO_OK; }},
diff --git a/bpvo_amd/csrc/estimate.hip b/bpvo_amd/csrc/estimate.hip
--- a/bpvo_amd/csrc/estimate.hip
+++ b/bpvo_amd/csrc/estimate.hip
@@ -116,6 +116,7 @@
   float* d_records_out;
   int loss, max_iterations;
   std::vector<int> max_pts;
+  std::vector<char> census_level;
   bool ref_mode;
   int fuse_frozen;
   bool allow_persistent;
@@ -135,6 +136,30 @@
   r.small_ctx = (size_t) c->L * c->n_pairs <= 64 && r.n <= 8 && c->small_batch_fused && c->G == 1;
   r.l2_moot = r.loss == BPVO_LOSS_L2 && c->C == 8 && r.fuse_frozen && !c->fast_warp && c->params.interp == BPVO_INTERP_LINEAR;
   r.team_ran = r.team_split = r.frac_queued = false;
+}
+
+static int settle_current_slots(GroupRun& r, bool team)
+{
+  bpvo_hip_ctx* c = r.c;
+  std::fill(r.census_level.begin(), r.census_level.end(), 0);
+  const bool kernels_read_census = !team && !r.pk_group && !r.ref_mode && c->C == 8 && c->G == 1 && c->params.interp == BPVO_INTERP_LINEAR && !c->fast_warp;
+  for(int i = 0; i < r.n; ++i) {
+    FrameSlot& fc = c->frames[r.curs[i]];
+    if(!fc.census_current) continue;
+    bool ok = kernels_read_census && c->ws[r.wss[i]].tapkey != nullptr;
+    for(int l = 0; l < c->L && ok; ++l)
+      if(fc.lazy[l] == 2 && r.n > c->persist_max_ws &&
+         (double) c->frames[r.refs[i]].n_host[l] > c->tapcache_max_density * (double) slot_geom(c, c->frames[r.refs[i]], l).npix)
+        ok = false;
+    if(ok) {
+      for(int l = 0; l < c->L; ++l)
+        if(fc.lazy[l] == 2) r.census_level[l] = 1;
+      continue;
+    }
+    const FrameRun fr{r.ln->stream, r.ln, r.curs[i], true, nullptr, nullptr};
+    if(int rc = ensure_dense_descriptor(c, r.curs[i], &fr)) return rc;
+  }
+  return BPVO_OK;
 }
 
 static int group_upload(GroupRun& r)
@@ -253,7 +278,7 @@
   return {false, false};
 }
 
-static int run_level_chain(GroupRun& r, GNLaunch g)
+static int run_level_chain(GroupRun& r, GNLaunch g, int l)
 {
   bpvo_hip_ctx* c = r.c;
   Lane* ln = r.ln;
@@ -263,6 +288,7 @@
   int n_cur = r.n;
   g.active.list = nullptr;
   const bool fused_path = c->C == 8 && r.fuse_frozen && !c->fast_warp && c->params.interp == BPVO_INTERP_LINEAR;
+  const bool warp_fills_caches = r.census_level[l] != 0;
   bool none_moving = r.l2_moot;
   LinearizeFlags f;
   f.timers = TIMERS_ESTIMATE;
@@ -270,7 +296,7 @@
                      [&](int) -> int {
                        g.npairs = n_cur;
                        f.median = !none_moving;
-                       f.warp = !(none_moving && fused_path);
+                       f.warp = !(none_moving && fused_path) || warp_fills_caches;
                        for(int k = 0; k < kItersPerSync; ++k) linearize_launches(c, ln, g, table, f);
                        return BPVO_OK;
                      },
@@ -308,7 +334,7 @@
       if(pk.served) continue;
     }
     persistent = false;
-    if(int rc = run_level_chain(r, g)) return rc;
+    if(int rc = run_level_chain(r, g, l)) return rc;
   }
   return BPVO_OK;
 }
@@ -420,10 +446,13 @@
     for(int i = 1; i < n; ++i) r.max_iterations = std::max(r.max_iterations, prms[i]->maxIterations);
   }
   r.max_pts.assign((size_t) c->L, 0);
+  r.census_level.assign((size_t) c->L, 0);
   for(const bool persistent_forms : {allow_persistent, false}) {
     group_modes(r, persistent_forms);
+    const bool team = persistent_forms && ln == &c->lanes[0] && !loss_is_chain_only(r.loss) && team_serves(c, n) && templates_suit_teams(c, n, refs);
+    if(int rc = settle_current_slots(r, team)) return rc;
     if(int rc = group_upload(r)) return rc;
-    if(persistent_forms && ln == &c->lanes[0] && !loss_is_chain_only(r.loss) && team_serves(c, n) && templates_suit_teams(c, n, refs))
+    if(team)
       if(int rc = run_team(r)) return rc;
     if(!r.team_ran)
       if(int rc = run_levels(r)) return rc;
@@ -437,7 +466,7 @@
   return BPVO_OK;
 }
 
-int check_pairs(bpvo_hip_ctx* c, int n, const int* wss, const int* refs, const int* curs, int level_lo, int level_hi)
+int check_pairs(bpvo_hip_ctx* c, int n, const int* wss, const int* refs, const int* curs, int level_lo, int level_hi, bool keep_census)
 {
   for(int i = 0; i < n; ++i) {
     CHECK_WS(c, wss[i]); CHECK_SLOT(c, refs[i]); CHECK_SLOT(c, curs[i]);
@@ -448,8 +477,10 @@
     for(int l = level_lo; l <= level_hi; ++l)
       if(c->frames[refs[i]].n_host[l] <= 0) return fail(c, BPVO_ERR_NO_TEMPLATE, "you should call setData before calling computeResiduals");
   }
-  for(int i = 0; i < n; ++i)
+  for(int i = 0; i < n; ++i) {
+    if(keep_census && c->frames[curs[i]].census_current) continue;
     if(int rc = ensure_dense_descriptor(c, curs[i])) return rc;
+  }
   return BPVO_OK;
 }
 
@@ -486,7 +517,7 @@
   if(n <= 0) return BPVO_OK;
   if(n > c->n_pairs) return fail(c, BPVO_ERR_INVALID_ARG, "more pairs than workspaces");
   const bpvo_hip_params& p = c->params;
-  if(int rc = check_pairs(c, n, wss, refs, curs, 0, -1)) return rc;
+  if(int rc = check_pairs(c, n, wss, refs, curs, 0, -1, true)) return rc;
   int nl = lanes_for(c, n, 8);
   if(nl < 0) return nl;
   const int loss = prms ? prms[0]->lossFunction : p.lossFunction;
@@ -562,6 +593,7 @@
 
 int upload_single_job(bpvo_hip_ctx* c, int ws, int ref, int cur, int level)
 {
+  if(int rc = ensure_dense_descriptor(c, cur)) return rc;
   PairJob* h = c->lanes[0].h_pjobs;
   h[0] = make_pair_job(c, ws, ref, cur, level);
   for(int k = 0; k < c->G && c->G > 1; ++k) h[1 + k] = group_pair_job(c, h[0], k);
diff --git a/bpvo_amd/csrc/frame_common.h b/bpvo_amd/csrc/frame_common.h
--- a/bpvo_amd/csrc/frame_common.h
+++ b/bpvo_amd/csrc/frame_common.h
@@ -34,6 +34,10 @@
   const float S0 = (float) (e / 9), A = (float) (e % 3), B = (float) ((e / 3) % 3);
   return S0 * k0 + A * k1 + B * k2;
 }
+__device__ __forceinline__ float bp_row_value(unsigned S0, unsigned a, unsigned b, float k0, float k1, float k2)
+{
+  return (float) S0 * k0 + (float) a * k1 + (float) b * k2;
+}
 __device__ __forceinline__ float bp_col(float Tm2, float Tm1, float T0, float Tp1, float Tp2, float k0, float k1, float k2)
 {
   float o = k0 * T0;
diff --git a/bpvo_amd/csrc/frames.hip b/bpvo_amd/csrc/frames.hip
--- a/bpvo_amd/csrc/frames.hip
+++ b/bpvo_amd/csrc/frames.hip
@@ -68,11 +68,16 @@
   bool census_only[kMaxLevels] = {};
   bool any_census_only = false;
   for(int l = p.maxTestLevel; l < c->L; ++l) any_census_only |= census_only[l] = census_only_ok && geom[l].nms_radius == 1;
+  const bool cur_census_ok = skip_odd_disp != 0 && c->lazy_current_call && form == DF_BITPLANES_FUSED;
+  bool cur_census[kMaxLevels] = {};
+  bool any_cur_census = false;
+  for(int l = p.maxTestLevel; l < c->L; ++l) any_cur_census |= cur_census[l] = cur_census_ok && geom[l].nms_radius > 0;
   for(int i = 0; i < count; ++i) {
     FrameSlot& f = c->frames[slots[i]];
     f.ch0_valid = !(skip_odd_disp && (i & 1));
+    f.census_current = (i & 1) && any_cur_census;
     for(int l = 0; l < c->L; ++l) {
-      f.lazy[l] = (lazy_ok && !(i & 1) && geom[l].nms_radius > 0) ? (census_only[l] ? 2 : 1) : 0;
+      f.lazy[l] = (lazy_ok && !(i & 1) && geom[l].nms_radius > 0) ? (census_only[l] ? 2 : 1) : ((i & 1) && cur_census[l]) ? 2 : 0;
       if(f.sal_state[l] == FrameSlot::SAL_ON_DEMAND) f.sal_state[l] = FrameSlot::SAL_GONE;
     }
   }
@@ -108,15 +113,19 @@
   {
     const int tested = c->L - p.maxTestLevel;
     double px = 0;
-    for(int l = p.maxTestLevel; l < c->L; ++l) px += (double) geom[l].npix * count;
+    for(int l = p.maxTestLevel; l < c->L; ++l) px += (double) geom[l].npix * (cur_census[l] ? count - count / 2 : count);
     ScopedTimer t(c, KC_DESCRIPTOR, px, fr.ln);
     for(const LevelSpan& sp : level_spans(c->L, p.maxTestLevel, merge_descriptor_levels(count, c->merge_levels_max_frames, tested, form))) {
       const FrameLaunch f = frame_launch(c, tab, geom, sp, count);
       switch(form) {
         case DF_BITPLANES_FUSED:
-          if(sp.count > 1 ? any_census_only : census_only[sp.first]) launch_census_templates(s, f);
-          if(sp.count == 1 && census_only[sp.first]) launch_bitplanes_pairs(s, f, c->gauss_k);
-          else launch_bitplanes(s, f, p.sigmaBitPlanes, c->gauss_k, 1);
+          {
+            const bool census_a = sp.count > 1 ? any_census_only : census_only[sp.first];
+            const bool census_b = sp.count > 1 ? any_cur_census : cur_census[sp.first];
+            if(census_a || census_b) launch_census_templates(s, f, census_b);
+            if(sp.count == 1 && census_only[sp.first]) launch_bitplanes_pairs(s, f, c->gauss_k, !census_b);
+            else launch_bitplanes(s, f, p.sigmaBitPlanes, c->gauss_k, 1);
+          }
           break;
         case DF_BITPLANES_SMOOTHED_CENSUS:
         case DF_BITPLANES_UNSMOOTHED:
@@ -286,7 +295,7 @@
   return frames_set_template_slots(c, strided_slots(first, stride, count).data(), count, ctx_run(c));
 }
 
-int ensure_dense_descriptor(bpvo_hip_ctx* c, int slot)
+int ensure_dense_descriptor(bpvo_hip_ctx* c, int slot, const FrameRun* run)
 {
   FrameSlot& f = c->frames[slot];
   bool any = false;
@@ -295,16 +304,18 @@
   uint8_t was[kMaxLevels];
   for(int l = 0; l < c->L; ++l) { was[l] = f.lazy[l]; f.lazy[l] = 0; }
   auto restore = [&]() { for(int l = 0; l < c->L; ++l) f.lazy[l] = was[l]; };
-  const FrameRun fr = ctx_run(c);
+  const FrameRun fr = run ? *run : ctx_run(c);
   const FrameJob* tab = nullptr;
   const int rc = upload_frame_jobs(c, &slot, 1, fr, 0, &tab);
   if(rc) { restore(); return rc; }
   for(const LevelSpan& sp : level_spans(c->L, c->params.maxTestLevel, false))
-    launch_bitplanes(c->stream, frame_launch(c, tab, c->geom, sp, 1), c->params.sigmaBitPlanes, c->gauss_k, 1);
-  if(hipGetLastError() != hipSuccess || hipStreamSynchronize(c->stream) != hipSuccess) {
+    launch_bitplanes(fr.stream, frame_launch(c, tab, c->geom, sp, 1), c->params.sigmaBitPlanes, c->gauss_k, 1);
+  if(hipGetLastError() != hipSuccess || hipStreamSynchronize(fr.stream) != hipSuccess) {
     restore();
+    if(fr.own_thread) { fr.ln->err = "ensure_dense_descriptor: descriptor kernels failed"; return BPVO_ERR_DEVICE; }
     return fail(c, BPVO_ERR_DEVICE, "ensure_dense_descriptor: descriptor kernels failed");
   }
+  f.census_current = false;
   return BPVO_OK;
 }
 
diff --git a/bpvo_amd/csrc/gn_census_taps.h b/bpvo_amd/csrc/gn_census_taps.h
--- /dev/null
+++ b/bpvo_amd/csrc/gn_census_taps.h
@@ -0,0 +1,69 @@
+#pragma once
+#include "frame_common.h"
+#include "gn_common.h"
+
+namespace bpvo_hip {
+
+__device__ __forceinline__ unsigned tap_key(int xi, int yi) { return ((unsigned) yi << 16) | (unsigned) xi; }
+
+__device__ __forceinline__ float4 census_half_record(const uint8_t* __restrict__ cen, int W, int R, int px, int py, int half, float k0, float k1, float k2)
+{
+  int cx[5];
+#pragma unroll
+  for(int d = 0; d < 5; ++d) cx[d] = bp_census_coord(px - 2 + d, W);
+  const int sh = 4 * half;
+  unsigned idx[5];
+#pragma unroll
+  for(int r = 0; r < 5; ++r) {
+    const uint8_t* __restrict__ row = cen + (size_t) bp_census_coord(py - 2 + r, R) * W;
+    const unsigned cm2 = spread_planes((unsigned) row[cx[0]] >> sh).x, cm1 = spread_planes((unsigned) row[cx[1]] >> sh).x,
+                   c0 = spread_planes((unsigned) row[cx[2]] >> sh).x, cp1 = spread_planes((unsigned) row[cx[3]] >> sh).x,
+                   cp2 = spread_planes((unsigned) row[cx[4]] >> sh).x;
+    idx[r] = bp_row_index(cm2, cm1, c0, cp1, cp2);
+    __builtin_amdgcn_sched_barrier(0);
+  }
+  float o[4];
+#pragma unroll
+  for(int c = 0; c < 4; ++c) {
+    float T[5];
+#pragma unroll
+    for(int r = 0; r < 5; ++r) T[r] = bp_row_entry((int) ((idx[r] >> (8 * c)) & 0xffu), k0, k1, k2);
+    o[c] = bp_col(T[0], T[1], T[2], T[3], T[4], k0, k1, k2);
+  }
+  return make_float4(o[0], o[1], o[2], o[3]);
+}
+
+template <bool NT>
+__device__ __forceinline__ void census_taps_fill_wave(const PairJob& j, int i, int xi, int yi, bool miss)
+{
+  unsigned long long m = __ballot(miss);
+  if(m == 0) return;
+  const int lane = (int) __lane_id();
+  do {
+    int q = lane >> 3, pos = 0;
+    unsigned long long mm = m;
+#pragma unroll
+    for(int s = 32; s >= 1; s >>= 1) {
+      const unsigned long long low = mm & ((1ull << s) - 1ull);
+      const int cl = __popcll(low);
+      const bool up = q >= cl;
+      q -= up ? cl : 0;
+      pos += up ? s : 0;
+      mm = up ? (mm >> s) : low;
+    }
+    const bool work = (lane >> 3) < __popcll(m);
+    const int si = __shfl(i, pos), sx = __shfl(xi, pos), sy = __shfl(yi, pos);
+    if(work) {
+      const int t = lane & 3, half = (lane >> 2) & 1;
+      const float4 v = census_half_record(j.cen, j.cols, j.rows, sx + (t & 1), sy + (t >> 1), half, j.bk[0], j.bk[1], j.bk[2]);
+      store_v4<NT>(reinterpret_cast<float4*>(j.tapcache.get()) + tile_index<8>(si, 2 * t + half), v);
+      if((lane & 7) == 0) j.tapkey[si] = tap_key(sx, sy);
+    }
+#pragma unroll 1
+    for(int k = 0; k < 8 && m; ++k) m &= m - 1;
+  } while(m);
+  __builtin_amdgcn_fence(__ATOMIC_RELEASE, "workgroup");
+  __builtin_amdgcn_fence(__ATOMIC_ACQUIRE, "workgroup");
+}
+
+}
diff --git a/bpvo_amd/csrc/gn_warp.h b/bpvo_amd/csrc/gn_warp.h
--- a/bpvo_amd/csrc/gn_warp.h
+++ b/bpvo_amd/csrc/gn_warp.h
@@ -1,6 +1,7 @@
 #pragma once
 #include "gn_common.h"
 #include "warp_rule.h"
+#include "gn_census_taps.h"
 
 namespace bpvo_hip {
 
@@ -41,7 +42,6 @@
   return Iw - i0;
 }
 
-__device__ __forceinline__ unsigned tap_key(int xi, int yi) { return ((unsigned) yi << 16) | (unsigned) xi; }
 __device__ __forceinline__ void taps8_gather(const PairJob& j, int xi, int yi, int W, float4 (&t)[8])
 {
   const float4* q0 = reinterpret_cast<const float4*>(j.desc + ((size_t) yi * W + xi) * 8);
@@ -78,10 +78,11 @@
   for(int c = 0; c < 8; ++c) res[c] = bilinear_res(i00[c], i01[c], i10[c], i11[c], i0[c], xf, yf, wx, wy);
 }
 
-template <int C, bool FAST, bool HALF = false, bool NT = true>
+template <int C, bool FAST, bool HALF = false, bool NT = true, bool CEN = false>
 __device__ __forceinline__ bool warp_point(const PairJob& j, const float (&P)[12], int i, bool in_block, float (&res)[C], bool& cache_hit,
                                            float4* X_out = nullptr)
 {
+  static_assert(!CEN || (C == 8 && !FAST && !HALF), "census-only levels: bit-planes, the f64 formulation, the warp kernel");
   cache_hit = false;
   const int W = j.cols, R = j.rows;
   const float4 X = load_point<NT>(j, i);
@@ -148,6 +149,16 @@
   }
 
   const int PT = (C == 8 || C == 1) ? C : j.pitch;
+  bool census_level = false, census_hit = false;
+  if constexpr(CEN && !HALF) {
+    if(j.cen) {
+      census_level = true;
+      const unsigned key = tap_key(xi, yi);
+      const bool look = valid && in_block;
+      census_hit = look && j.tapkey[i] == key;
+      census_taps_fill_wave<NT>(j, i, xi, yi, look && !census_hit);
+    }
+  }
   if(valid) {
     const double wx = 1.0 - xf, wy = 1.0 - yf;
     const float* __restrict__ d0 = j.desc + ((size_t) yi * W + xi) * PT;
@@ -156,10 +167,10 @@
     if constexpr(C == 8) {
       const unsigned key = tap_key(xi, yi);
       const bool cached = j.tapcache_on != 0;
-      const bool hit = cached && j.tapkey[i] == key;
+      const bool hit = census_level ? census_hit : (cached && j.tapkey[i] == key);
       cache_hit = hit;
       float4 t[8];
-      if(hit) {
+      if(hit || census_level) {
         const float4* tc = reinterpret_cast<const float4*>(j.tapcache.get());
 #pragma unroll
         for(int k = 0; k < 8; ++k) t[k] = load_v4<NT>(tc + tile_index<8>(i, k));
@@ -216,14 +227,36 @@
   return valid;
 }
 
-template <int C, bool FAST>
+__device__ __forceinline__ void census_prefill_chunk(const PairJob& j, unsigned chunk)
+{
+  if(!j.cen) return;
+  const int n = j.n;
+  if((int) (chunk * K6_BLOCK) >= n) return;
+  float P[12];
+  projection_matrix(j, j.st->T, P);
+  const int i_raw = chunk * K6_BLOCK + threadIdx.x;
+  const bool in_block = i_raw < n;
+  const int i = in_block ? i_raw : n - 1;
+  const float4 X = load_point<true>(j, i);
+  const WarpFoot f = warp_foot(P, X.x, X.y, X.z, X.w, j.cols, j.rows);
+  const unsigned key = tap_key(f.xi, f.yi);
+  const bool miss = f.valid && in_block && j.tapkey[i] != key;
+  const unsigned long long m = __ballot(miss);
+  census_taps_fill_wave<true>(j, i, f.xi, f.yi, miss);
+  if(m && (threadIdx.x & 63) == 0) atomicAdd(j.cnt.get() + 5, 0ull - (unsigned long long) __popcll(m));
+}
+
+template <int C, bool FAST, bool CEN = false>
 __device__ __forceinline__ void warp_chunk(const PairJob& j, int mode, unsigned chunk, BracketLds& s, bool dense = false)
 {
   const GNState* __restrict__ st = j.st;
   if(mode == 2) { if(!st->r_stale) return; }
   else {
     if(!st->active) return;
-    if(mode == 1 && !(st->delta_scale > 1e-6f)) return;
+    if(mode == 1 && !(st->delta_scale > 1e-6f)) {
+      if constexpr(CEN) census_prefill_chunk(j, chunk);
+      return;
+    }
   }
   const int n = j.n;
   if((int) (chunk * K6_BLOCK) >= n) return;
@@ -239,7 +272,7 @@
   const int i = in_block ? i_raw : n - 1;
   float res[C];
   bool hit;
-  const bool valid = warp_point<C, FAST>(j, P, i, in_block, res, hit);
+  const bool valid = warp_point<C, FAST, false, true, CEN>(j, P, i, in_block, res, hit);
   if(in_block) j.valid[i] = valid ? 1 : 0;
   if(in_block) {
     if constexpr(C == 8) {
diff --git a/bpvo_amd/csrc/host_ctx.h b/bpvo_amd/csrc/host_ctx.h
--- a/bpvo_amd/csrc/host_ctx.h
+++ b/bpvo_amd/csrc/host_ctx.h
@@ -55,6 +55,7 @@
   uint8_t lazy[kMaxLevels] = {};
   enum : uint8_t { SAL_STORED = 0, SAL_ON_DEMAND = 1, SAL_GONE = 2 };
   uint8_t sal_state[kMaxLevels] = {};
+  bool census_current = false;
   bool ch0_valid = true;
   float* desc[kMaxLevels] = {};
   float* disp = nullptr;
@@ -356,6 +357,8 @@
   int points_from_compact = 0;
   int lazy_template = 1;
   int lazy_saliency = 1;
+  int lazy_current = 1;
+  bool lazy_current_call = false;
   int keep_current_disparity = 0;
   double up_last_seconds = 0.0;
   size_t up_last_bytes = 0;
@@ -535,7 +538,7 @@
   LinearizeTimers timers = TIMERS_OFF;
 };
 void linearize_launches(bpvo_hip_ctx* c, Lane* ln, const bpvo_hip::GNLaunch& g, size_t stride, const LinearizeFlags& f);
-int check_pairs(bpvo_hip_ctx* c, int n, const int* wss, const int* refs, const int* curs, int level_lo, int level_hi);
+int check_pairs(bpvo_hip_ctx* c, int n, const int* wss, const int* refs, const int* curs, int level_lo, int level_hi, bool keep_census = false);
 int estimate_group(bpvo_hip_ctx* c, Lane* ln, int n, const int* wss, const int* refs, const int* curs, const float* T_init, float* poses,
                    bpvo_hip_stats* stats, float* d_records_out, bool allow_persistent, const bpvo_hip_params* const* prms = nullptr);
 int estimate_batch(bpvo_hip_ctx* c, int n, const int* wss, const int* refs, const int* curs, const float* T_init, float* poses, bpvo_hip_stats* stats,
@@ -564,7 +567,7 @@
 int ensure_lanes(bpvo_hip_ctx* c, int n);
 int lanes_for(bpvo_hip_ctx* c, int n, int cap);
 int ensure_saliency(bpvo_hip_ctx* c, int slot, int level);
-int ensure_dense_descriptor(bpvo_hip_ctx* c, int slot);
+int ensure_dense_descriptor(bpvo_hip_ctx* c, int slot, const FrameRun* fr = nullptr);
 int pose_cov_pass(bpvo_hip_ctx* c, int n_records, int members, const int* wss, const int* refs, const int* curs, const float* X, int level,
                   const float* T, const float* sigma, const bpvo_hip_params* const* prms, bpvo_hip_pose_covariance* out);
 int pose_cov_ensure_scratch(bpvo_hip_ctx* c);
diff --git a/bpvo_amd/csrc/kernels.h b/bpvo_amd/csrc/kernels.h
--- a/bpvo_amd/csrc/kernels.h
+++ b/bpvo_amd/csrc/kernels.h
@@ -74,8 +74,8 @@
                   const GaussTaps& after);
 void launch_laplacian(hipStream_t s, const FrameJob* jobs, int W, int R, int nframes, int ksize );
 void launch_census(hipStream_t s, const FrameLaunch& f, const int* blur_taps );
-void launch_bitplanes_pairs(hipStream_t s, const FrameLaunch& f, const float k[3]);
-void launch_census_templates(hipStream_t s, const FrameLaunch& f);
+void launch_bitplanes_pairs(hipStream_t s, const FrameLaunch& f, const float k[3], bool current = true);
+void launch_census_templates(hipStream_t s, const FrameLaunch& f, bool current = false);
 void launch_bitplanes(hipStream_t s, const FrameLaunch& f, float sigma, const float k[3], int from_image);
 enum { SELECT_ALL = 0, SELECT_CANDIDATES = 1, SELECT_COMPACT = 2 };
 void launch_saliency_select(hipStream_t s, const FrameLaunch& f, int C, int nms_radius, int border, const float gauss_k[3], int part);
diff --git a/bpvo_amd/csrc/kernels_frame.hip b/bpvo_amd/csrc/kernels_frame.hip
--- a/bpvo_amd/csrc/kernels_frame.hip
+++ b/bpvo_amd/csrc/kernels_frame.hip
@@ -259,9 +259,9 @@
 typedef unsigned int u32_unaligned __attribute__((aligned(1)));
 typedef unsigned short u16_unaligned __attribute__((aligned(1)));
 constexpr int CT_ROWS = 8, CT_PX = 4;
-__global__ __launch_bounds__(256) void census_templates_kernel(const FrameJob* jobs, int nframes, int job_pitch)
-{
-  const FrameJob& j = level_job(jobs, blockIdx.z, nframes, job_pitch, 2);
+__global__ __launch_bounds__(256) void census_templates_kernel(const FrameJob* jobs, int nframes, int job_pitch, int job_step)
+{
+  const FrameJob& j = level_job(jobs, blockIdx.z, nframes, job_pitch, job_step);
   if(j.lazy != 2) return;
   const int W = j.cols, R = j.rows;
   const int x = (blockIdx.x * 64 + (threadIdx.x & 63)) * CT_PX;
@@ -1769,11 +1769,11 @@
   else
     hipLaunchKernelGGL(census_kernel, dim3((f.W + 63) / 64, (f.R + 4 * CENSUS_ROWS - 1) / (4 * CENSUS_ROWS), f.nframes), dim3(256), 0, s, f.jobs);
 }
-void launch_census_templates(hipStream_t s, const FrameLaunch& f)
-{
-  const int na = (f.nframes + 1) / 2;
+void launch_census_templates(hipStream_t s, const FrameLaunch& f, bool current)
+{
+  const int na = current ? f.nframes : (f.nframes + 1) / 2;
   hipLaunchKernelGGL(census_templates_kernel, dim3((f.W + 64 * CT_PX - 1) / (64 * CT_PX), (f.R + 4 * CT_ROWS - 1) / (4 * CT_ROWS), na * f.nlevels), dim3(256), 0, s,
-                     f.jobs, na, f.job_pitch);
+                     f.jobs, na, f.job_pitch, current ? 1 : 2);
 }
 void launch_bitplanes(hipStream_t s, const FrameLaunch& f, float sigma, const float k[3], int from_image)
 {
@@ -1786,14 +1786,14 @@
   else
     hipLaunchKernelGGL(bitplanes_noblur_kernel, dim3((f.W * f.R + 255) / 256, 1, f.nframes), dim3(256), 0, s, f.jobs);
 }
-void launch_bitplanes_pairs(hipStream_t s, const FrameLaunch& f, const float k[3])
+void launch_bitplanes_pairs(hipStream_t s, const FrameLaunch& f, const float k[3], bool current)
 {
   const int stack = f.nframes >= 16 ? 8 : (f.nframes > 4 ? 4 : 1);
   const int ncols = (f.W + BP_TW - 1) / BP_TW, nrows = (f.R + BP_TH * stack - 1) / (BP_TH * stack);
   int dense = 0;
   for(int cx = 0; cx < ncols; ++cx) dense += bp_tile_column_is_lazy(cx * BP_TW, f.W) ? 0 : 1;
   const int na = (f.nframes + 1) / 2, nb = f.nframes / 2;
-  if(nb > 0) hipLaunchKernelGGL(bitplanes_blur_kernel<true>, dim3(ncols, nrows, nb), dim3(256), 0, s, f.jobs + 1, k[0], k[1], k[2], stack, nb, 0, 2, 0);
+  if(nb > 0 && current) hipLaunchKernelGGL(bitplanes_blur_kernel<true>, dim3(ncols, nrows, nb), dim3(256), 0, s, f.jobs + 1, k[0], k[1], k[2], stack, nb, 0, 2, 0);
   if(dense > 0) hipLaunchKernelGGL(bitplanes_blur_kernel<true>, dim3(dense, nrows, na), dim3(256), 0, s, f.jobs, k[0], k[1], k[2], stack, na, 0, 2, 1);
 }
 void launch_saliency(hipStream_t s, const FrameLaunch& f, int C)
diff --git a/bpvo_amd/csrc/kernels_gn.hip b/bpvo_amd/csrc/kernels_gn.hip
--- a/bpvo_amd/csrc/kernels_gn.hip
+++ b/bpvo_amd/csrc/kernels_gn.hip
@@ -20,7 +20,7 @@
 __global__ __launch_bounds__(K6_BLOCK) void warp_residual_kernel(const PairJob* __restrict__ jobs, ActiveSet act, int mode, int dense)
 {
   __shared__ BracketLds s;
-  warp_chunk<C, FAST>(jobs[active_workspace(act, blockIdx.y)], mode, blockIdx.x, s, dense != 0);
+  warp_chunk<C, FAST, C == 8 && !FAST>(jobs[active_workspace(act, blockIdx.y)], mode, blockIdx.x, s, dense != 0);
 }
 
 __global__ void clear_stale_kernel(const PairJob* jobs, int n)
diff --git a/bpvo_amd/csrc/types.h b/bpvo_amd/csrc/types.h
--- a/bpvo_amd/csrc/types.h
+++ b/bpvo_amd/csrc/types.h
@@ -163,6 +163,8 @@
   GNParams      prm;
   int           loss;
   float         good_thr;
+  GPtr<const uint8_t> cen;
+  float         bk[4];
 };
 
 struct InormScratch { uint32_t bins[256]; float table[256]; uint32_t ticket; uint32_t pad[31]; };
```
